# salesforce/ALPRO

Hardware: AMD Instinct MI355X
Metric: video-text pairs/sec (8f x 224^2, 40-tok) (higher is better)
Workload: dtype fp16

## Files before the change

alpro_amd/amp.py:

```python
import contextlib

import torch

from alpro_amd import config as rt


class LossScaler:

    def __init__(self, init_scale=2.0 ** 16, dynamic=True, growth=2.0, backoff=0.5, window=2000, min_scale=1.0, max_scale=2.0 ** 24, device=None):
        self.dynamic, self.growth, self.backoff, self.window = dynamic, growth, backoff, window
        self.min_scale, self.max_scale = min_scale, max_scale
        self._init = float(init_scale)
        self.state = None
        if device is not None:
            self.to(device)

    def to(self, device):
        if self.state is None or self.state.device != torch.device(device):
            prev = self.state.tolist() if self.state is not None else (getattr(self, "_pending", None) or [self._init, 0.0, 0.0, 0.0])
            self.state = torch.tensor(prev, dtype=torch.float32, device=device)
        return self

    @property
    def scale(self):
        return self.state[0:1]

    def loss_scale(self):
        return float(self.state[0].item())

    def state_dict(self):
        s = self.state.tolist() if self.state is not None else (getattr(self, "_pending", None) or [self._init, 0.0, 0.0, 0.0])
        return {"loss_scale": s[0], "unskipped": int(s[1]), "applied_steps": int(s[2]), "skipped_steps": int(s[3])}

    def load_state_dict(self, sd):
        vals = [float(sd["loss_scale"]), float(sd.get("unskipped", 0)), float(sd.get("applied_steps", 0)), float(sd.get("skipped_steps", 0))]
        if self.state is None:
            self._init = vals[0]
            self._pending = vals
        else:
            self.state.copy_(torch.tensor(vals, dtype=torch.float32))


_SCALERS = []


def needs_loss_scaling(dtype=None):
    return (dtype or rt.compute_dtype()) == torch.float16


def scaler_for(optimizer, create=True, **kw):
    inner = getattr(optimizer, "_opt", optimizer)
    sc = getattr(inner, "scaler", None)
    if sc is None and create:
        sc = LossScaler(**kw)
        inner.scaler = sc
        _SCALERS.append(sc)
        rt.set_armed_loss_scaler(sc)
    return sc


def initialize(models, optimizers=None, enabled=True, opt_level="O1", loss_scale="dynamic", **unused):
    if optimizers is not None and needs_loss_scaling():
        for opt in (optimizers if isinstance(optimizers, (list, tuple)) else [optimizers]):
            if loss_scale == "dynamic" or loss_scale is None:
                scaler_for(opt)
            else:
                scaler_for(opt, init_scale=float(loss_scale), dynamic=False)
    return models if optimizers is None else (models, optimizers)


def _grads_of(optimizer):
    from alpro_amd.optim import real_grad
    return [p.grad for g in optimizer.param_groups for p in g["params"] if real_grad(p) is not None]


def unscale_(optimizer, scaler):
    inner = getattr(optimizer, "_opt", optimizer)
    inv = torch.reciprocal(scaler.scale).reshape(())
    flat = getattr(inner, "flat", None)
    if flat is not None:
        if getattr(inner, "_inflight", None):
            inner._finish_exchange()
            inner._note_synced("sum")
        flat["g"].mul_(inv)
    else:
        grads = _grads_of(inner)
        if grads:
            torch._foreach_mul_(grads, inv)
    inner._grads_scaled = False


@contextlib.contextmanager
def scale_loss(loss, optimizers, delay_unscale=False, **unused):
    if not needs_loss_scaling():
        yield loss
        return
    opts = optimizers if isinstance(optimizers, (list, tuple)) else [optimizers]
    scaler = scaler_for(opts[0]).to(loss.device)
    for o in opts[1:]:
        getattr(o, "_opt", o).scaler = scaler
    for o in opts:
        getattr(o, "_opt", o)._grads_scaled = True
        if hasattr(getattr(o, "_opt", o), "_g_clean"):
            getattr(o, "_opt", o)._mark_dirty()
    with rt.loss_scaling(scaler):
        yield loss * scaler.scale.reshape(())
    if not delay_unscale:
        for o in opts:
            unscale_(o, scaler)
            _install_foreign_step_guard(getattr(o, "_opt", o), scaler)


def _install_foreign_step_guard(opt, scaler):
    if hasattr(opt, "flat") or getattr(opt, "_alpro_guarded", False):
        return
    real = opt.step

    def step(*a, **k):
        grads = _grads_of(opt)
        norms = torch._foreach_norm(grads) if grads else []
        finite = bool(torch.isfinite(torch.stack(norms)).all()) if norms else True
        st = scaler.state
        if not finite:
            st[0] = max(float(st[0]) * scaler.backoff, scaler.min_scale) if scaler.dynamic else st[0]
            st[1] = 0.0
            st[3] += 1.0
            return None
        out = real(*a, **k)
        st[2] += 1.0
        st[1] += 1.0
# ... 29 lines not shown
```

alpro_amd/config.py:

```python
import os

import torch

_DTYPES = {"bf16": torch.bfloat16, "bfloat16": torch.bfloat16, "f16": torch.float16, "fp16": torch.float16,
           "float16": torch.float16, "f32": torch.float32, "fp32": torch.float32, "float32": torch.float32}

_compute_dtype = _DTYPES[os.environ.get("ALPRO_COMPUTE_DTYPE", "bf16").lower()]


def compute_dtype():
    return _compute_dtype


def set_compute_dtype(dt):
    global _compute_dtype
    _compute_dtype = _DTYPES[dt.lower()] if isinstance(dt, str) else dt
    return _compute_dtype


class use_compute_dtype:

    def __init__(self, dt):
        self.dt = dt

# ... 71 lines not shown
_WGRAD_SIDE = {}


def _several_ranks():
    try:
        import torch.distributed as td
        return td.is_available() and td.is_initialized() and td.get_world_size() > 1
    except Exception:
        return False


def set_wgrad_stream(v):
    _wgrad_stream[0] = bool(v)


def wgrad_stream_enabled():
    return _wgrad_stream[0]


def wgrad_scope(enter):
    _wgrad_active[0] += 1 if enter else -1


def wgrad_side_stream(device):
    if not (_wgrad_stream[0] and _wgrad_active[0] > 0 and device.type == "cuda") or (_several_ranks() and os.environ.get("ALPRO_WGRAD_STREAM") != "force"):
        return None
    import torch
    cur = torch.cuda.current_stream(device)
    if any(s.cuda_stream == cur.cuda_stream for s in _TEXT_SIDE.values()):
        return None
    key = (device.index if device.index is not None else torch.cuda.current_device(), cur.cuda_stream)
    ent = _WGRAD_SIDE.get(key)
    if ent is None:
        ent = _WGRAD_SIDE[key] = [torch.cuda.Stream(device), False]
    ent[1] = True
    return ent[0]


def side_streams_of_current(device):
    if not (_wgrad_stream[0] and device.type == "cuda") or (_several_ranks() and os.environ.get("ALPRO_WGRAD_STREAM") != "force"):
        return []
    import torch
    key = (device.index if device.index is not None else torch.cuda.current_device(), torch.cuda.current_stream(device).cuda_stream)
    ent = _WGRAD_SIDE.get(key)
    if ent is None:
        ent = _WGRAD_SIDE[key] = [torch.cuda.Stream(device), False]
    return [ent[0].cuda_stream]


def join_wgrad():
    if not _WGRAD_SIDE:
        return
    import torch
    for (idx, handle), ent in _WGRAD_SIDE.items():
        if ent[1]:
            cur = torch.cuda.current_stream(idx)
            if cur.cuda_stream == handle:
                cur.wait_stream(ent[0])
                ent[1] = False


_text_stream = [os.environ.get("ALPRO_TEXT_STREAM", "1") != "0"]
_TEXT_SIDE = {}


def set_text_stream(v):
    _text_stream[0] = bool(v)


def text_stream_enabled():
    return _text_stream[0]


def text_side_stream(device):
    if not (_text_stream[0] and device.type == "cuda"):
        return None
    import torch
    key = (device.index if device.index is not None else torch.cuda.current_device(), torch.cuda.current_stream(device).cuda_stream)
    s = _TEXT_SIDE.get(key)
    if s is None:
        s = _TEXT_SIDE[key] = torch.cuda.Stream(device)
    return s


def is_text_side_stream(stream):
    return any(s.cuda_stream == stream.cuda_stream for s in _TEXT_SIDE.values())


def join_text_streams():
    if not _TEXT_SIDE:
        return
    import torch
    for (idx, handle), s in _TEXT_SIDE.items():
        cur = torch.cuda.current_stream(idx)
        if cur.cuda_stream == handle:
            cur.wait_stream(s)


_prompter_stream = [os.environ.get("ALPRO_PROMPTER_STREAM", "1") != "0"]
_PROMPTER_SIDE = {}


def set_prompter_stream(v):
    _prompter_stream[0] = bool(v)


def prompter_stream_enabled():
    return _prompter_stream[0]


def prompter_side_stream(device):
    if not (_prompter_stream[0] and device.type == "cuda") or (_several_ranks() and os.environ.get("ALPRO_PROMPTER_STREAM") != "force"):
        return None
    import torch
    key = (device.index if device.index is not None else torch.cuda.current_device(), torch.cuda.current_stream(device).cuda_stream)
    s = _PROMPTER_SIDE.get(key)
    if s is None:
        s = _PROMPTER_SIDE[key] = torch.cuda.Stream(device)
    return s


_defer_tadd = [os.environ.get("ALPRO_DEFER_TEMPORAL_ADD", "1") != "0"]


def defer_temporal_add():
    return _defer_tadd[0]


def set_defer_temporal_add(v):
    _defer_tadd[0] = bool(v)


def _recompute_from_env():
    v = os.environ.get("ALPRO_RECOMPUTE", "0").strip()
    if v not in ("0", "1"):
        raise ValueError("ALPRO_RECOMPUTE=%r: expected 0 (keep every ViT block activation, the default) or 1 (recompute them in backward)" % v)
    return v == "1"


_recompute = [_recompute_from_env()]


def recompute_blocks():
    return _recompute[0]


def set_recompute(flag):
    _recompute[0] = bool(flag)

# ... 113 lines not shown
```

alpro_amd/csrc/backward.hip:

```cpp
#include "common.hpp"
#include "row768.hpp"
#include <algorithm>

namespace alpro {
namespace {

template <typename Tin, typename Tout>
__device__ __forceinline__ void transpose_tile(float (&tile)[64][65], const Tin* __restrict__ in, int64_t ld_in, Tout* __restrict__ out,
                                               int64_t ld_out, int R, int C, int Rpad, float* __restrict__ colsum, int bx, int by) {
  const int r0 = by * 64, c0 = bx * 64;
  const int tx = threadIdx.x & 63, ty = threadIdx.x >> 6;
#pragma unroll 4
  for (int i = ty; i < 64; i += 4) {
    const int r = r0 + i, c = c0 + tx;
    tile[i][tx] = (r < R && c < C) ? to_f32(in[(int64_t)r * ld_in + c]) : 0.f;
  }
  __syncthreads();
  if (colsum && ty == 0 && c0 + tx < C) {
    float s = 0.f;
#pragma unroll 8
    for (int i = 0; i < 64; ++i) s += tile[i][tx];
    atomicAdd(colsum + c0 + tx, s);
  }
#pragma unroll 4
  for (int i = ty; i < 64; i += 4) {
    const int c = c0 + i, r = r0 + tx;
    if (c < C && r < Rpad) out[(int64_t)c * ld_out + r] = from_f32<Tout>(tile[tx][i]);
  }
}

template <typename Tin, typename Tout>
__global__ __launch_bounds__(256) void transpose_kernel(const Tin* __restrict__ in, int64_t ld_in, Tout* __restrict__ out, int64_t ld_out,
                                                        int R, int C, int Rpad, float* __restrict__ colsum) {
  __shared__ float tile[64][65];
  transpose_tile<Tin, Tout>(tile, in, ld_in, out, ld_out, R, C, Rpad, colsum, blockIdx.x, blockIdx.y);
}

template <typename Tout>
__global__ __launch_bounds__(256) void transpose_batch_kernel(const alpro_transpose_job_t* __restrict__ jobs, int njobs) {
  __shared__ float tile[64][65];
  int lo = 0, hi = njobs - 1;
  while (lo < hi) {
    const int mid = (lo + hi + 1) >> 1;
    if (jobs[mid].tile0 <= (int)blockIdx.x) lo = mid;
    else hi = mid - 1;
  }
  const alpro_transpose_job_t jb = jobs[lo];
  const int t = blockIdx.x - jb.tile0, tcx = (jb.C + 63) / 64;
  transpose_tile<float, Tout>(tile, jb.in, jb.ld_in, (Tout*)jb.out, jb.ld_out, jb.R, jb.C, jb.Rpad, nullptr, t % tcx, t / tcx);
}

constexpr int LN_PART_BYTES = 3 * LN_D * (int)sizeof(float);

struct EmitArgs {
// ... 4 lines not shown
  float drop_p;
  uint32_t drop_seed;
  float* colsum_pre;
  int extra_cls;
};

template <typename T, bool CP = true>
__device__ __forceinline__ void emit_row(const EmitArgs& e, int64_t r, int lane, float (&v)[12], float (&cp)[12]) {
  T* out = (T*)e.out;
  if (e.mode == ALPRO_EMIT_ROWS) {
    if (e.drop_seed) {
      const uint32_t th = drop_thresh24(e.drop_p);
      const float ks = 1.0f / (1.0f - e.drop_p);
#pragma unroll
      for (int i = 0; i < 12; ++i) v[i] = row_drop_keep(e.drop_seed, r, lane, i, th) ? v[i] * ks : 0.f;
    }
    ln_store_scaled<T>(out + r * LN_D, lane, v, e.scale ? e.scale[r / e.group] : 1.0f);
    return;
  }
  const int Tn = e.p0, N = e.p1;
  const int64_t S = 1 + (int64_t)N * Tn;
  const int64_t b = r / S, k = r - b * S;
  if (e.mode == ALPRO_EMIT_FRAME) {
    if (k == 0) {
      const float inv = 1.0f / (float)Tn;
      for (int t = 0; t < Tn; ++t) ln_store_scaled<T>(out + ((b * Tn + t) * (N + 1)) * LN_D, lane, v, (e.scale ? e.scale[b * Tn + t] : 1.0f) * inv);
    } else {
      const int64_t n = (k - 1) / Tn;
      const int t = (int)((k - 1) - n * Tn);
      ln_store_scaled<T>(out + ((b * Tn + t) * (N + 1) + 1 + n) * LN_D, lane, v, e.scale ? e.scale[b * Tn + t] : 1.0f);
    }
  } else {
    if (k == 0) return;
    const int64_t o = r - b - 1;
    if constexpr (CP) {
#pragma unroll
      for (int i = 0; i < 12; ++i) cp[i] += v[i];
    }
    ln_store_scaled<T>(out + o * LN_D, lane, v, e.scale ? e.scale[o / e.group] : 1.0f);
  }
}

#define ALPRO_LN_DATA 0
#include "layernorm_bwd_kernel.hpp"
#undef ALPRO_LN_DATA
#define ALPRO_LN_DATA 1
#include "layernorm_bwd_kernel.hpp"
#undef ALPRO_LN_DATA

__global__ __launch_bounds__(1024) void colsum_reduce_kernel(const float* __restrict__ part, int nparts, int nslots, float* __restrict__ d0,
                                                             float* __restrict__ d1, float* __restrict__ d2) {
  __shared__ float4 red[128][8];
  __shared__ float4 red2[8][8];
  const int k = blockIdx.y, c4 = threadIdx.x & 7, sl = threadIdx.x >> 3;
  float* dst = k == 0 ? d0 : (k == 1 ? d1 : d2);
  if (!dst) return;
  const int col = blockIdx.x * 32 + c4 * 4;
  float4 s = make_float4(0.f, 0.f, 0.f, 0.f);
#pragma unroll 4
  for (int p = sl; p < nparts; p += 128) {
    const float4 v = *(const float4*)(part + ((int64_t)p * nslots + k) * LN_D + col);
    s.x += v.x; s.y += v.y; s.z += v.z; s.w += v.w;
  }
  red[sl][c4] = s;
  __syncthreads();
  if (sl < 8) {
    float4 t = red[sl * 16][c4];
#pragma unroll
    for (int i = 1; i < 16; ++i) { const float4 v = red[sl * 16 + i][c4]; t.x += v.x; t.y += v.y; t.z += v.z; t.w += v.w; }
    red2[sl][c4] = t;
  }
  __syncthreads();
  if (sl == 0) {
    float4 t = red2[0][c4];
#pragma unroll
    for (int i = 1; i < 8; ++i) { const float4 v = red2[i][c4]; t.x += v.x; t.y += v.y; t.z += v.z; t.w += v.w; }
    float4* o = (float4*)(dst + col);
    const float4 c = *o;
    *o = make_float4(c.x + t.x, c.y + t.y, c.z + t.z, c.w + t.w);
  }
}

__global__ __launch_bounds__(192) void cls_rows_reduce_kernel(const float* __restrict__ cls_ws, float* __restrict__ dx, int64_t ld_dx, int T, int N) {
  const int b = blockIdx.x, c = threadIdx.x * 4;
  float4 s = make_float4(0.f, 0.f, 0.f, 0.f);
  for (int t = 0; t < T; ++t) {
    const float4 v = *(const float4*)(cls_ws + ((int64_t)b * T + t) * LN_D + c);
    s.x += v.x; s.y += v.y; s.z += v.z; s.w += v.w;
  }
  float4* o = (float4*)(dx + (int64_t)b * (1 + (int64_t)N * T) * ld_dx + c);
  const float4 cur = *o;
  *o = make_float4(cur.x + s.x, cur.y + s.y, cur.z + s.z, cur.w + s.w);
}

template <typename TE, int MODE>
__global__ __launch_bounds__(256) void vit_final_pool_bwd_kernel(const float* __restrict__ dout, const float* __restrict__ x, const float* __restrict__ gamma,
                                                                 float eps, float* __restrict__ dx, float* __restrict__ dgamma, float* __restrict__ dbeta,
                                                                 int64_t rows, int Tn, int N, const EmitArgs em, float* __restrict__ part) {
  __shared__ float red[2][4][LN_D];
  const int lane = threadIdx.x & 63, w = threadIdx.x >> 6;
  const int64_t nwaves = (int64_t)gridDim.x * 4;
  const int64_t S = 1 + (int64_t)N * Tn;
  float g[12], ag[12], ab[12], cp[12];
  ln_load(gamma, lane, g);
#pragma unroll
  for (int i = 0; i < 12; ++i) ag[i] = ab[i] = cp[i] = 0.f;
  for (int64_t r = (int64_t)blockIdx.x * 4 + w; r < rows; r += nwaves) {
    const int64_t b = r / S, k = r - b * S;
    const int64_t n = k ? (k - 1) / Tn : 0;
    const int t = k ? (int)((k - 1) - n * Tn) : 0;
    int64_t src;
    float sc = 1.0f;
    if constexpr (MODE == ALPRO_POOL_TEMPORAL) {
      src = b * (N + 1) + (k ? 1 + n : 0);
      if (k) sc = 1.0f / (float)Tn;
    } else if constexpr (MODE == ALPRO_POOL_SPATIAL) {
      src = b * (Tn + 1) + (k ? 1 + t : 0);
      if (k) sc = 1.0f / (float)N;
    } else {
      src = (b * Tn + t) * (N + 1) + (k ? 1 + n : 0);
    }
    float xv[12], d[12];
    ln_load_nt(x + r * LN_D, lane, xv);
    ln_load(dout + src * LN_D, lane, d);
    if (MODE == ALPRO_POOL_NONE && k == 0) {
      for (int f = 1; f < Tn; ++f) {
        float d2[12];
        ln_load(dout + (src + (int64_t)f * (N + 1)) * LN_D, lane, d2);
#pragma unroll
        for (int i = 0; i < 12; ++i) d[i] += d2[i];
      }
    }
    float mean, rstd;
// ... 345 lines not shown
  ALPRO_DISPATCH_DTYPE(out_dtype, T, hipLaunchKernelGGL(transpose_batch_kernel<T>, dim3((unsigned)total_tiles), dim3(256), 0, (hipStream_t)stream, jobs, njobs));
  return check_launch("alpro_transpose_batch");
}

extern "C" int alpro_layernorm_bwd_emit(const void* dy, int dy_dtype, int64_t ld_dy, const float* dy2, const float* x, int64_t ldx,
                                        const float* gamma, float eps, float* dx, int64_t ld_dx, int accumulate, float* dgamma, float* dbeta,
                                        int rows, int D, int map_mode, int map_p0, int map_p1, float drop_p, uint32_t drop_seed, void* emit_out,
                                        int emit_dtype, int emit_mode, int emit_p0, int emit_p1, const float* emit_scale, int emit_scale_group, float emit_drop_p,
                                        uint32_t emit_drop_seed, float* emit_colsum_pre, int emit_extra_cls, void* workspace, size_t workspace_bytes,
                                        void* stream) {
  ALPRO_CHECK(dy && x && gamma && dx && rows > 0, "alpro_layernorm_bwd: bad args");
  ALPRO_CHECK((dgamma != nullptr) == (dbeta != nullptr), "alpro_layernorm_bwd: dgamma and dbeta must both be given or both be NULL (got %s only); "
              "pass a throw-away buffer for the one that is not wanted", dgamma ? "dgamma" : "dbeta");
  const bool data_only = dgamma == nullptr;
  ALPRO_CHECK(!data_only || !emit_colsum_pre, "alpro_layernorm_bwd_emit: colsum_pre needs the column-sum form of the kernel -- pass a throw-away dgamma / dbeta pair with it");
  ALPRO_CHECK(!workspace || (((uintptr_t)workspace % 16) == 0 && workspace_bytes >= LN_PART_BYTES), "alpro_layernorm_bwd: the workspace must be 16-byte aligned and hold at least one workgroup's sums (%d bytes)", LN_PART_BYTES);
  ALPRO_CHECK(D == LN_D, "alpro_layernorm_bwd: D=%d unsupported", D);
  ALPRO_CHECK(map_mode >= 0 && map_mode <= ALPRO_MAP_FRAME_TOKENS, "alpro_layernorm_bwd: bad map_mode %d", map_mode);
  ALPRO_CHECK(map_mode != ALPRO_MAP_FRAME_TOKENS || accumulate, "alpro_layernorm_bwd: the FRAME_TOKENS scatter needs accumulate=1 (CLS rows are shared)");
  ALPRO_CHECK(emit_mode >= ALPRO_EMIT_NONE && emit_mode <= ALPRO_EMIT_SKIP_CLS, "alpro_layernorm_bwd_emit: bad emit_mode %d", emit_mode);
  ALPRO_CHECK(emit_mode == ALPRO_EMIT_NONE || emit_out, "alpro_layernorm_bwd_emit: an emit mode needs the output rows");
  ALPRO_CHECK(emit_mode == ALPRO_EMIT_NONE || ld_dx == LN_D, "alpro_layernorm_bwd_emit: the emit needs a dense gradient stream (ld_dx == 768)");
  ALPRO_CHECK(emit_mode == ALPRO_EMIT_NONE || emit_mode == ALPRO_EMIT_ROWS || (emit_p0 > 0 && emit_p1 > 0), "alpro_layernorm_bwd_emit: FRAME / SKIP_CLS emits need p0 = T, p1 = N");
  ALPRO_CHECK(!emit_scale || emit_scale_group > 0, "alpro_layernorm_bwd_emit: emit_scale_group must be > 0");
  ALPRO_CHECK(!emit_drop_seed || (emit_mode == ALPRO_EMIT_ROWS && emit_drop_p > 0.f && emit_drop_p < 1.f), "alpro_layernorm_bwd_emit: dropout only in ROWS mode, 0 < p < 1");
  ALPRO_CHECK(!emit_colsum_pre || emit_mode == ALPRO_EMIT_SKIP_CLS, "alpro_layernorm_bwd_emit: colsum_pre belongs to the SKIP_CLS emit");
  ALPRO_CHECK(emit_extra_cls == 0 || (emit_mode == ALPRO_EMIT_ROWS && map_mode == ALPRO_MAP_SKIP_CLS && emit_p0 > 0 && emit_p1 > 0),
              "alpro_layernorm_bwd_emit: extra CLS rows go with ROWS emit after a SKIP_CLS-mapped LayerNorm (p0 = T, p1 = N)");
  EmitArgs em;
  em.out = emit_out; em.mode = emit_mode; em.p0 = emit_p0; em.p1 = emit_p1; em.scale = emit_scale; em.group = emit_scale_group;
  em.drop_p = emit_drop_p; em.drop_seed = emit_drop_seed; em.colsum_pre = emit_colsum_pre; em.extra_cls = emit_extra_cls;
  ALPRO_CHECK(emit_mode == ALPRO_EMIT_NONE || emit_dtype == dy_dtype || dy_dtype == ALPRO_F32, "alpro_layernorm_bwd_emit: emit_dtype must be dy's dtype, or any dtype when dy is the fp32 stream");
  const bool frame = map_mode == ALPRO_MAP_FRAME_TOKENS;
  const size_t cls_bytes = frame ? (size_t)(rows / (map_p1 + 1)) * LN_D * sizeof(float) : 0;
  ALPRO_CHECK(!workspace || workspace_bytes >= cls_bytes + LN_PART_BYTES, "alpro_layernorm_bwd: the workspace must hold the CLS frame terms (%zu bytes) and at least one workgroup's sums", cls_bytes);
  const int cap = get_option(OPT_LN_GRID);
  int nblk = grid_for(rows, 4 * 8, cap > 0 ? cap : 256 * 8);
  if (workspace && !data_only) nblk = (int)std::min<size_t>((size_t)nblk, (workspace_bytes - cls_bytes) / LN_PART_BYTES);
  const dim3 grid(nblk), blk(256);
  float* part = data_only ? nullptr : (float*)workspace;
  float* cls_ws = (workspace && frame) ? (float*)workspace + (data_only ? 0 : (size_t)nblk * 3 * LN_D) : nullptr;
  hipStream_t st = (hipStream_t)stream;
#define ALPRO_LNB(T, TE) \
  do { if (data_only) ALPRO_LNB_K(layernorm_bwd_data_kernel, T, TE); else ALPRO_LNB_K(layernorm_bwd_kernel, T, TE); } while (0)
#define ALPRO_LNB_K(KERNEL, T, TE) hipLaunchKernelGGL((KERNEL<T, TE>), grid, blk, 0, st, (const T*)dy, ld_dy, dy2, x, ldx, gamma, eps, dx, ld_dx, accumulate, dgamma, dbeta, (int64_t)rows, map_mode, map_p0, map_p1, drop_p, drop_seed, em, part, cls_ws)
  if (dy_dtype == ALPRO_F32 && emit_mode != ALPRO_EMIT_NONE && emit_dtype == ALPRO_BF16) ALPRO_LNB(float, bf16_t);
  else if (dy_dtype == ALPRO_F32 && emit_mode != ALPRO_EMIT_NONE && emit_dtype == ALPRO_F16) ALPRO_LNB(float, f16_t);
  else if (dy_dtype == ALPRO_F32) ALPRO_LNB(float, float);
  else if (dy_dtype == ALPRO_BF16) ALPRO_LNB(bf16_t, bf16_t);
  else if (dy_dtype == ALPRO_F16) ALPRO_LNB(f16_t, f16_t);
  else { set_error("alpro_layernorm_bwd: bad dtype %d", dy_dtype); return ALPRO_ERR_INVALID; }
#undef ALPRO_LNB
#undef ALPRO_LNB_K
  if (part) hipLaunchKernelGGL(colsum_reduce_kernel, dim3(LN_D / 32, emit_colsum_pre ? 3 : 2), dim3(1024), 0, st, part, nblk, 3, dgamma, dbeta, emit_colsum_pre);
  if (cls_ws) hipLaunchKernelGGL(cls_rows_reduce_kernel, dim3(rows / (map_p1 + 1) / map_p0), dim3(192), 0, st, cls_ws, dx, ld_dx, map_p0, map_p1);
  return check_launch("alpro_layernorm_bwd");
}

extern "C" int alpro_layernorm_bwd(const void* dy, int dy_dtype, int64_t ld_dy, const float* dy2, const float* x, int64_t ldx,
                                   const float* gamma, float eps, float* dx, int64_t ld_dx, int accumulate, float* dgamma, float* dbeta,
                                   int rows, int D, int map_mode, int map_p0, int map_p1, float drop_p, uint32_t drop_seed, void* workspace,
                                   size_t workspace_bytes, void* stream) {
  return alpro_layernorm_bwd_emit(dy, dy_dtype, ld_dy, dy2, x, ldx, gamma, eps, dx, ld_dx, accumulate, dgamma, dbeta, rows, D, map_mode, map_p0, map_p1,
                                  drop_p, drop_seed, nullptr, dy_dtype, ALPRO_EMIT_NONE, 0, 0, nullptr, 1, 0.f, 0u, nullptr, 0, workspace, workspace_bytes, stream);
}

extern "C" int alpro_vit_final_pool_mode_bwd(const float* dout, const float* x, const float* gamma, float eps, float* dx, float* dgamma, float* dbeta,
                                             int mode, int64_t rows, int B, int T, int N, int D, void* emit_out, int emit_dtype, const float* emit_scale,
                                             int emit_scale_group, void* workspace, size_t workspace_bytes, void* stream) {
  constexpr size_t part_bytes = 2 * LN_D * sizeof(float);
  ALPRO_CHECK(dout && x && gamma && dx && dgamma && dbeta && B > 0 && T > 0 && N > 0, "alpro_vit_final_pool_mode_bwd: bad args");
  ALPRO_CHECK(mode >= ALPRO_POOL_TEMPORAL && mode <= ALPRO_POOL_NONE, "alpro_vit_final_pool_mode_bwd: bad mode %d (ALPRO_POOL_TEMPORAL / _SPATIAL / _NONE)", mode);
  ALPRO_CHECK(D == LN_D, "alpro_vit_final_pool_mode_bwd: D=%d unsupported (hidden size is 768 on this path)", D);
  ALPRO_CHECK(rows == (int64_t)B * (1 + (int64_t)N * T), "alpro_vit_final_pool_mode_bwd: rows=%lld is not B * (1 + N * T) = %d * (1 + %d * %d)", (long long)rows, B, N, T);
  ALPRO_CHECK(!workspace || (((uintptr_t)workspace % 16) == 0 && workspace_bytes >= part_bytes), "alpro_vit_final_pool_mode_bwd: the workspace must be 16-byte aligned and hold at least one workgroup's sums (%zu bytes)", part_bytes);
  ALPRO_CHECK(!emit_out || emit_dtype == ALPRO_F32 || emit_dtype == ALPRO_BF16 || emit_dtype == ALPRO_F16, "alpro_vit_final_pool_mode_bwd: bad emit_dtype %d", emit_dtype);
  ALPRO_CHECK(!emit_scale || emit_scale_group > 0, "alpro_vit_final_pool_mode_bwd: emit_scale_group must be > 0");
  EmitArgs em;
  em.out = emit_out; em.mode = emit_out ? ALPRO_EMIT_ROWS : ALPRO_EMIT_NONE; em.p0 = T; em.p1 = N; em.scale = emit_scale; em.group = emit_scale_group;
  em.drop_p = 0.f; em.drop_seed = 0u; em.colsum_pre = nullptr; em.extra_cls = 0;
  const int cap = get_option(OPT_LN_GRID);
  int nblk = grid_for(rows, 4 * 8, cap > 0 ? cap : 256 * 8);
  if (workspace) nblk = (int)std::min<size_t>((size_t)nblk, workspace_bytes / part_bytes);
  const dim3 grid(nblk), blk(256);
  float* part = (float*)workspace;
  hipStream_t st = (hipStream_t)stream;
#define ALPRO_FPB(TE, M) hipLaunchKernelGGL((vit_final_pool_bwd_kernel<TE, M>), grid, blk, 0, st, dout, x, gamma, eps, dx, dgamma, dbeta, rows, T, N, em, part)
#define ALPRO_FPB_MODES(TE) \
  do { if (mode == ALPRO_POOL_TEMPORAL) ALPRO_FPB(TE, ALPRO_POOL_TEMPORAL); else if (mode == ALPRO_POOL_SPATIAL) ALPRO_FPB(TE, ALPRO_POOL_SPATIAL); else ALPRO_FPB(TE, ALPRO_POOL_NONE); } while (0)
  if (emit_out && emit_dtype == ALPRO_BF16) ALPRO_FPB_MODES(bf16_t);
  else if (emit_out && emit_dtype == ALPRO_F16) ALPRO_FPB_MODES(f16_t);
  else ALPRO_FPB_MODES(float);
#undef ALPRO_FPB_MODES
#undef ALPRO_FPB
  if (part) hipLaunchKernelGGL(colsum_reduce_kernel, dim3(LN_D / 32, 2), dim3(1024), 0, st, part, nblk, 2, dgamma, dbeta, (float*)nullptr);
  return check_launch("alpro_vit_final_pool_mode_bwd");
}

extern "C" int alpro_gather_cast(const float* src, int64_t ld, void* out, int dtype, int rows, int D, int map_mode, int map_p0, int map_p1,
                                 const float* row_scale, int row_scale_group, float cls_scale, float drop_p, uint32_t drop_seed, float* colsum,
                                 float* colsum_pre, void* workspace, size_t workspace_bytes, void* stream) {
  ALPRO_CHECK(src && out && rows > 0, "alpro_gather_cast: bad args");
  ALPRO_CHECK(!workspace || (((uintptr_t)workspace % 16) == 0 && workspace_bytes >= 2 * LN_D * sizeof(float)), "alpro_gather_cast: the workspace must be 16-byte aligned and hold at least one workgroup's sums");
  ALPRO_CHECK(D == LN_D, "alpro_gather_cast: D=%d unsupported", D);
  ALPRO_CHECK(map_mode >= 0 && map_mode <= ALPRO_MAP_PATCH_EMBED, "alpro_gather_cast: bad map_mode %d", map_mode);
  ALPRO_CHECK(!row_scale || row_scale_group > 0, "alpro_gather_cast: row_scale_group must be > 0");
  if (colsum || colsum_pre) {
    float* part = (float*)workspace;
    int nblk = grid_for(rows, 32, 512);
    if (part) nblk = (int)std::min<size_t>((size_t)nblk, workspace_bytes / (2 * LN_D * sizeof(float)));
    ALPRO_DISPATCH_DTYPE(dtype, T, hipLaunchKernelGGL((gather_cast_kernel<T, 16>), dim3(nblk), dim3(1024), 0, (hipStream_t)stream, src, ld, (T*)out, (int64_t)rows, map_mode, map_p0, map_p1, row_scale, row_scale_group, cls_scale, drop_p, drop_seed, colsum, colsum_pre, part));
    if (part) hipLaunchKernelGGL(colsum_reduce_kernel, dim3(LN_D / 32, 2), dim3(1024), 0, (hipStream_t)stream, part, nblk, 2, colsum, colsum_pre, (float*)nullptr);
  } else {
    ALPRO_DISPATCH_DTYPE(dtype, T, hipLaunchKernelGGL((gather_cast_kernel<T, 4>), dim3(grid_for(rows, 8, 256 * 32)), dim3(256), 0, (hipStream_t)stream, src, ld, (T*)out, (int64_t)rows, map_mode, map_p0, map_p1, row_scale, row_scale_group, cls_scale, drop_p, drop_seed, colsum, colsum_pre, (float*)nullptr));
  }
  return check_launch("alpro_gather_cast");
}

extern "C" int alpro_colsum_tn(const void* A, int64_t lda, int dtype, int M, int N, int K, float* colsum, void* workspace, size_t workspace_bytes,
                               void* stream) {
  ALPRO_CHECK(A && colsum && M > 0 && N > 0 && K > 0, "alpro_colsum_tn: bad args");
  ALPRO_CHECK(dtype == ALPRO_BF16 || dtype == ALPRO_F16, "alpro_colsum_tn: 16-bit rows only (it restates the 16-bit weight-gradient GEMM's bias gradient)");
  ALPRO_CHECK(lda >= N, "alpro_colsum_tn: lda must cover N");
  const int ranges = alpro_gemm_tn_ranges(M, N, K, cu_budget((hipStream_t)stream));
  const int total_steps = (M + 31) / 32, per = (total_steps + ranges - 1) / ranges, tk_cnt = (K + 255) / 256;
  const int sets = ranges * tk_cnt, npad = (N + 31) / 32 * 32;
  ALPRO_CHECK(workspace && ((uintptr_t)workspace % 16) == 0 && workspace_bytes >= (size_t)sets * npad * sizeof(float),
              "alpro_colsum_tn: the workspace must be 16-byte aligned and hold %d partial sets of %d floats (%zu bytes)", sets, npad, (size_t)sets * npad * sizeof(float));
  float* part = (float*)workspace;
  const dim3 grid((npad / 32 + 3) / 4, sets);
  hipStream_t st = (hipStream_t)stream;
  if (dtype == ALPRO_BF16) hipLaunchKernelGGL(colsum_tn_kernel<bf16_t>, grid, dim3(256), 0, st, (const bf16_t*)A, lda, M, N, per, tk_cnt, total_steps, part, npad);
  else hipLaunchKernelGGL(colsum_tn_kernel<f16_t>, grid, dim3(256), 0, st, (const f16_t*)A, lda, M, N, per, tk_cnt, total_steps, part, npad);
  hipLaunchKernelGGL(colsum_tn_reduce_kernel, dim3((N + 255) / 256), dim3(256), 0, st, part, sets, npad, colsum, N);
  return check_launch("alpro_colsum_tn");
}

extern "C" int alpro_tproj_small(const alpro_tproj_job_t* jobs_device, int njobs, int D, int mode, void* stream) {
  ALPRO_CHECK(jobs_device && njobs > 0 && (mode == 0 || mode == 1), "alpro_tproj_small: bad args");
  ALPRO_CHECK(D == LN_D, "alpro_tproj_small: D=%d unsupported", D);
  if (mode == 0) hipLaunchKernelGGL(tproj_small_kernel<0>, dim3(D / 4, njobs), dim3(256), 0, (hipStream_t)stream, jobs_device, D);
  else hipLaunchKernelGGL(tproj_small_kernel<1>, dim3(D / 64, njobs), dim3(256), 0, (hipStream_t)stream, jobs_device, D);
  return check_launch("alpro_tproj_small");
}

extern "C" int alpro_gelu_bwd(const void* dh, const void* u, void* du, int dtype, int64_t n, void* stream) {
  ALPRO_CHECK(dh && u && du && n > 0, "alpro_gelu_bwd: bad args");
  ALPRO_CHECK(n % 8 == 0, "alpro_gelu_bwd: n must be a multiple of 8");
  ALPRO_DISPATCH_DTYPE(dtype, T, hipLaunchKernelGGL(gelu_bwd_kernel<T>, dim3(grid_for(n / Chunk<T>::N, 256, 256 * 16)), dim3(256), 0, (hipStream_t)stream, (const T*)dh, (const T*)u, (T*)du, n));
  return check_launch("alpro_gelu_bwd");
}

extern "C" int alpro_cls_mean_bwd(const float* dx_out, int64_t ld_batch, float* dside, int B, int T, int D, void* stream) {
  ALPRO_CHECK(dx_out && dside && B > 0 && T > 0 && D > 0, "alpro_cls_mean_bwd: bad args");
  hipLaunchKernelGGL(cls_mean_bwd_kernel, dim3(B), dim3(256), 0, (hipStream_t)stream, dx_out, ld_batch, dside, B, T, D);
  return check_launch("alpro_cls_mean_bwd");
}

extern "C" int alpro_scatter_add_rows_ordered(const float* src, const int64_t* idx, float* dst, int rows, int D, int64_t dst_rows, int64_t skip_idx, uint32_t* keys_ws,
                                              void* stream) {
  ALPRO_CHECK(src && idx && dst && keys_ws && rows > 0, "alpro_scatter_add_rows_ordered: bad args");
  ALPRO_CHECK(D == LN_D, "alpro_scatter_add_rows_ordered: D=%d unsupported", D);
  ALPRO_CHECK(rows <= SCATTER_SORT_MAX && dst_rows > 0 && dst_rows < (1 << 19), "alpro_scatter_add_rows_ordered: at most %d source rows and fewer than 2^19 table rows (got %d, %lld)",
              SCATTER_SORT_MAX, rows, (long long)dst_rows);
  hipLaunchKernelGGL(scatter_sort_keys_kernel, dim3(1), dim3(1024), 0, (hipStream_t)stream, idx, rows, dst_rows, keys_ws);
// ... 15 lines not shown
```

alpro_amd/csrc/gemm_tn.hip:

```cpp
#include "common.hpp"

namespace alpro {
namespace {

constexpr int TM = 32;
constexpr int NSTAGE = 4;
constexpr int TW = 256;
constexpr int ROW_BYTES = TW * 2;
constexpr int IMG_BYTES = TM * ROW_BYTES;
constexpr int NT3 = 512;

__device__ u32x4 g_zero_page[4];

typedef short s16x4 __attribute__((ext_vector_type(4)));

__device__ __forceinline__ u32x2 tr4(const char* img, int m0, int colblk16, int lane) {
  const int p = lane & 15;
  const int row = m0 + (p >> 2);
  const int chunk = (colblk16 << 1) | ((p >> 1) & 1);
  const char* a = img + row * ROW_BYTES + ((chunk ^ ((row & 3) << 2)) << 4) + ((p & 1) << 3);
  const s16x4 r = __builtin_amdgcn_ds_read_tr16_b64_v4i16((__attribute__((address_space(3))) s16x4*)a);
  return __builtin_bit_cast(u32x2, r);
}
__device__ __forceinline__ u32x4 frag8(const char* img, int ks, int col0, int lane) {
  const int g = lane >> 5;
  const int blk = (col0 >> 4) + ((lane >> 4) & 1);
  const u32x2 a = tr4(img, ks * 16 + 4 * g, blk, lane);
  const u32x2 b = tr4(img, ks * 16 + 8 + 4 * g, blk, lane);
  const uint32_t ax = a.x, ay = a.y, bx = b.x, by = b.y;
  return mk4(ax, ay, bx, by);
}

template <typename T, int PP = 0>
__global__ __launch_bounds__(NT3, 1) void gemm_tn_kernel(const T* __restrict__ A, int64_t lda, const T* __restrict__ B, int64_t ldb,
                                                         float* __restrict__ C, int64_t ldc, int M, int N, int K, int per,
                                                         int tiles, int units, int tn_cnt, float* __restrict__ colsum, float* __restrict__ part,
                                                         float* __restrict__ part_cs, int ablate ) {
  extern __shared__ __attribute__((aligned(16))) char smem[];
  const int tid = threadIdx.x, lane = tid & 63, wave = __builtin_amdgcn_readfirstlane(tid >> 6);
  const int wr = wave >> 2, wc = wave & 3;
  const int upx = (units + 7) >> 3;
  const int unit = (blockIdx.x & 7) * upx + (blockIdx.x >> 3);
  if (unit >= units) return;
  const int range = unit / tiles, tile = unit - range * tiles;
  const int total_steps = (M + TM - 1) / TM;
  const int s0 = range * per, s1 = min(s0 + per, total_steps);
  const int n0 = (tile % tn_cnt) * TW, k0 = (tile / tn_cnt) * TW;
  if (s0 >= s1) return;

  const char* zero = (const char*)g_zero_page;
  const int rows_end = min(s1 * TM, M);
  const char* curA[2];
  const char* curB[2];
  int mrow[2];
  int64_t strA[2], strB[2];
#pragma unroll
  for (int i = 0; i < 2; ++i) {
    const int row = (wave + 8 * i) * 2 + (lane >> 5);
    const int col = ((lane & 31) ^ ((row & 3) << 2)) * 8;
    const int64_t m = (int64_t)s0 * TM + row;
// ... 131 lines not shown
        copy(2 * (1 - ks) + 1, buf);
        advance(1 - ks);
        asm volatile("s_waitcnt vmcnt(6)" ::: "memory");
        pbar();
        __builtin_amdgcn_s_setprio(1);
#pragma unroll
        for (int i = 0; i < 4; ++i)
#pragma unroll
          for (int jj = 0; jj < 2; ++jj) mma_chunk<T>(acc[i][jj], fa[i], fb[jj]);
        __builtin_amdgcn_s_setprio(0);
        if (cs_now) add_cols(fa);
        pbar();
      }
    }
    if (wr == 0) pbar();
  }
  if (do_cs) {
    const float t = cs + __shfl_xor(cs, 32, 64);
    const int n = n0 + wr * 128 + wc * 32 + (lane & 31);
    if (lane < 32 && part_cs) part_cs[((int64_t)range * tk_cnt + tk) * (tn_cnt * TW) + n] = t;
    else if (lane < 32 && n < N) unsafeAtomicAdd(colsum + n, t);
  }
  asm volatile("s_waitcnt vmcnt(0)" ::: "memory");
  if (part) {
    float* dst = part + (int64_t)unit * (TW * TW) + wave * 8192 + lane * 4;
#pragma unroll
    for (int i = 0; i < 4; ++i)
#pragma unroll
      for (int j = 0; j < 2; ++j)
#pragma unroll
        for (int q = 0; q < 4; ++q) {
          f32x4 v = {acc[i][j][4 * q], acc[i][j][4 * q + 1], acc[i][j][4 * q + 2], acc[i][j][4 * q + 3]};
          __builtin_nontemporal_store(v, (f32x4*)(dst + ((i * 2 + j) * 4 + q) * 256));
        }
    return;
  }
#pragma unroll
  for (int j = 0; j < 2; ++j) {
    const int k = k0 + wc * 64 + j * 32 + (lane & 31);
    if (k < K) {
#pragma unroll
      for (int i = 0; i < 4; ++i)
#pragma unroll
        for (int r = 0; r < 16; ++r) {
          const int n = n0 + wr * 128 + i * 32 + acc_row(r, lane);
          if (n < N) unsafeAtomicAdd(C + (int64_t)n * ldc + k, acc[i][j][r]);
        }
    }
  }
}

__global__ __launch_bounds__(256) void tn_reduce_kernel(const float* __restrict__ part, const float* __restrict__ part_cs, float* __restrict__ C,
                                                        int64_t ldc, float* __restrict__ colsum, int N, int K, int tiles, int ranges, int tn_cnt) {
  const int tile_blocks = part ? tiles * 64 : 0;
  if ((int)blockIdx.x >= tile_blocks) {
    __shared__ float red[8][32];
    const int c = threadIdx.x & 31, p = threadIdx.x >> 5;
    const int n = (blockIdx.x - tile_blocks) * 32 + c;
    const int sets = ranges * (tiles / tn_cnt);
    float t = 0.f;
    for (int r = p; r < sets; r += 8) t += part_cs[(int64_t)r * (tn_cnt * TW) + n];
    red[p][c] = t;
    __syncthreads();
    if (p == 0 && n < N) colsum[n] += ((red[0][c] + red[1][c]) + (red[2][c] + red[3][c])) + ((red[4][c] + red[5][c]) + (red[6][c] + red[7][c]));
    return;
  }
  const int tile = blockIdx.x >> 6, f = ((blockIdx.x & 63) << 8) + threadIdx.x;
  const int lane = f & 63, q = (f >> 6) & 3, j = (f >> 8) & 1, i = (f >> 9) & 3, wave = f >> 11;
  const int n = (tile % tn_cnt) * TW + (wave >> 2) * 128 + i * 32 + 8 * q + 4 * (lane >> 5);
  const int k = (tile / tn_cnt) * TW + (wave & 3) * 64 + j * 32 + (lane & 31);
  const float* src = part + (int64_t)tile * (TW * TW) + f * 4;
  const int64_t stride = (int64_t)tiles * (TW * TW);
  f32x4 t = {0.f, 0.f, 0.f, 0.f};
  int r = 0;
  for (; r + 4 <= ranges; r += 4) {
    const f32x4 a = __builtin_nontemporal_load((const f32x4*)(src + (r + 0) * stride)), b = __builtin_nontemporal_load((const f32x4*)(src + (r + 1) * stride));
    const f32x4 c = __builtin_nontemporal_load((const f32x4*)(src + (r + 2) * stride)), d = __builtin_nontemporal_load((const f32x4*)(src + (r + 3) * stride));
    t = (((t + a) + b) + c) + d;
  }
  for (; r < ranges; ++r) t = t + __builtin_nontemporal_load((const f32x4*)(src + r * stride));
  if (k < K) {
#pragma unroll
    for (int c = 0; c < 4; ++c)
      if (n + c < N) C[(int64_t)(n + c) * ldc + k] += t[c];
  }
}

template <typename T>
__global__ __launch_bounds__(256) void colsum_kernel(const T* __restrict__ A, int64_t lda, float* __restrict__ out, int M, int N) {
  constexpr int E = Chunk<T>::N;
  __shared__ float red[4][64 * E];
  const int lane = threadIdx.x & 63, w = threadIdx.x >> 6;
  const int c = blockIdx.x * 64 + lane;
  const bool cv = c * E < N;
  const int m0 = blockIdx.y * 256, m1 = min(m0 + 256, M);
  float s[E];
#pragma unroll
  for (int e = 0; e < E; ++e) s[e] = 0.f;
  if (cv) {
    const T* base = A + c * E;
    int m = m0 + w;
    for (; m + 28 < m1; m += 32) {
      u32x4 v[8];
#pragma unroll
      for (int u = 0; u < 8; ++u) v[u] = *(const u32x4*)(base + (int64_t)(m + 4 * u) * lda);
#pragma unroll
      for (int u = 0; u < 8; ++u) {
        float f[E];
        unpack_chunk<T>(v[u], f);
#pragma unroll
        for (int e = 0; e < E; ++e) s[e] += f[e];
      }
    }
    for (; m < m1; m += 4) {
      float f[E];
      unpack_chunk<T>(*(const u32x4*)(base + (int64_t)m * lda), f);
#pragma unroll
      for (int e = 0; e < E; ++e) s[e] += f[e];
    }
  }
#pragma unroll
  for (int e = 0; e < E; ++e) red[w][lane * E + e] = s[e];
  __syncthreads();
  for (int i = threadIdx.x; i < 64 * E; i += 256) {
    const int col = blockIdx.x * 64 * E + i;
    if (col < N) unsafeAtomicAdd(out + col, red[0][i] + red[1][i] + red[2][i] + red[3][i]);
  }
}

}
}

using namespace alpro;

namespace {
struct TnPlan {
  int tn, tiles, total_steps, ranges, per, units;
  size_t part_floats, cs_floats;
// ... 25 lines not shown
  return p;
}
}

extern "C" size_t alpro_gemm_tn_workspace_bytes(int M, int N, int K) {
  if (M <= 0 || N <= 0 || K <= 0) return 0;
  struct Memo { int M, N, K, forced; size_t bytes; };
  static Memo memo[64];
  static int n_memo = 0, lock = 0;
  const int forced = get_option(OPT_TN_SPLITS);
  while (__atomic_exchange_n(&lock, 1, __ATOMIC_ACQUIRE)) {}
  for (int i = 0; i < n_memo; ++i)
    if (memo[i].M == M && memo[i].N == N && memo[i].K == K && memo[i].forced == forced) {
      const size_t b = memo[i].bytes;
      __atomic_store_n(&lock, 0, __ATOMIC_RELEASE);
      return b;
    }
  __atomic_store_n(&lock, 0, __ATOMIC_RELEASE);
  size_t best = 0;
  for (int cus = 64; cus <= 256; cus += 8) {
    const TnPlan p = tn_plan(M, N, K, true, cus);
    const size_t b = (p.part_floats + p.cs_floats) * sizeof(float);
    best = b > best ? b : best;
  }
  while (__atomic_exchange_n(&lock, 1, __ATOMIC_ACQUIRE)) {}
  if (n_memo < 64) memo[n_memo++] = Memo{M, N, K, forced, best};
  __atomic_store_n(&lock, 0, __ATOMIC_RELEASE);
  return best;
}

extern "C" int alpro_gemm_tn_ranges(int M, int N, int K, int compute_units) {
  if (M <= 0 || N <= 0 || K <= 0) return 0;
  const int cus = (compute_units >= 64 && compute_units < 256) ? compute_units / 8 * 8 : 256;
  return tn_plan(M, N, K, true, cus).ranges;
}

extern "C" int alpro_gemm_tn_acc_ws(const void* A, int64_t lda, const void* B, int64_t ldb, float* C, int64_t ldc, int dtype, int M, int N,
                                    int K, float* colsum, void* workspace, size_t workspace_bytes, void* stream) {
  ALPRO_CHECK(A && B && C && M > 0 && N > 0 && K > 0, "alpro_gemm_tn_acc: bad args");
  ALPRO_CHECK(dtype == ALPRO_BF16 || dtype == ALPRO_F16, "alpro_gemm_tn_acc: 16-bit operands only (fp32 mode uses alpro_transpose + alpro_gemm)");
  ALPRO_CHECK(lda % 8 == 0 && ldb % 8 == 0 && lda >= (N + 7) / 8 * 8 && ldb >= (K + 7) / 8 * 8,
              "alpro_gemm_tn_acc: lda/ldb must be multiples of 8 covering N/K rounded up to 8 (16-byte chunks are read whole)");
  ALPRO_CHECK(((uintptr_t)A % 16) == 0 && ((uintptr_t)B % 16) == 0, "alpro_gemm_tn_acc: operands must be 16-byte aligned");
  const bool ws = workspace != nullptr;
  const TnPlan p = tn_plan(M, N, K, ws, cu_budget((hipStream_t)stream));
  float* part = nullptr;
  float* part_cs = nullptr;
  if (ws) {
    ALPRO_CHECK(((uintptr_t)workspace % 16) == 0 && workspace_bytes >= (p.part_floats + p.cs_floats) * sizeof(float),
                "alpro_gemm_tn_acc_ws: workspace must be 16-byte aligned and hold alpro_gemm_tn_workspace_bytes(M, N, K) bytes");
    part = p.ranges > 1 ? (float*)workspace : nullptr;
    part_cs = colsum ? (float*)workspace + p.part_floats : nullptr;
  }
  const bool pp = get_option(OPT_TN_KIND) == 2;
  const unsigned grid = (unsigned)((p.units + 7) / 8 * 8);
  const size_t lds = (size_t)NSTAGE * 2 * IMG_BYTES;
  hipStream_t st = (hipStream_t)stream;
  if (dtype == ALPRO_BF16) {
    static DeviceOnce once;
    once.run([&] {
      (void)hipFuncSetAttribute((const void*)gemm_tn_kernel<bf16_t, 0>, hipFuncAttributeMaxDynamicSharedMemorySize, (int)lds);
      (void)hipFuncSetAttribute((const void*)gemm_tn_kernel<bf16_t, 1>, hipFuncAttributeMaxDynamicSharedMemorySize, (int)lds);
    });
    if (pp) hipLaunchKernelGGL((gemm_tn_kernel<bf16_t, 1>), dim3(grid), dim3(NT3), lds, st, (const bf16_t*)A, lda, (const bf16_t*)B, ldb, C, ldc, M, N, K, p.per, p.tiles, p.units, p.tn, colsum, part, part_cs, 0);
    else hipLaunchKernelGGL((gemm_tn_kernel<bf16_t, 0>), dim3(grid), dim3(NT3), lds, st, (const bf16_t*)A, lda, (const bf16_t*)B, ldb, C, ldc, M, N, K, p.per, p.tiles, p.units, p.tn, colsum, part, part_cs, 0);
  } else {
    static DeviceOnce once;
    once.run([&] {
      (void)hipFuncSetAttribute((const void*)gemm_tn_kernel<f16_t, 0>, hipFuncAttributeMaxDynamicSharedMemorySize, (int)lds);
      (void)hipFuncSetAttribute((const void*)gemm_tn_kernel<f16_t, 1>, hipFuncAttributeMaxDynamicSharedMemorySize, (int)lds);
    });
    if (pp) hipLaunchKernelGGL((gemm_tn_kernel<f16_t, 1>), dim3(grid), dim3(NT3), lds, st, (const f16_t*)A, lda, (const f16_t*)B, ldb, C, ldc, M, N, K, p.per, p.tiles, p.units, p.tn, colsum, part, part_cs, 0);
    else hipLaunchKernelGGL((gemm_tn_kernel<f16_t, 0>), dim3(grid), dim3(NT3), lds, st, (const f16_t*)A, lda, (const f16_t*)B, ldb, C, ldc, M, N, K, p.per, p.tiles, p.units, p.tn, colsum, part, part_cs, 0);
  }
  if (part || part_cs)
    hipLaunchKernelGGL(tn_reduce_kernel, dim3((part ? p.tiles * 64 : 0) + (part_cs ? p.tn * (TW / 32) : 0)), dim3(256), 0, st, part, part_cs, C, ldc, colsum, N, K, p.tiles, p.ranges, p.tn);
  return check_launch("alpro_gemm_tn_acc");
}

extern "C" int alpro_gemm_tn_acc(const void* A, int64_t lda, const void* B, int64_t ldb, float* C, int64_t ldc, int dtype, int M, int N,
                                 int K, float* colsum, void* stream) {
  return alpro_gemm_tn_acc_ws(A, lda, B, ldb, C, ldc, dtype, M, N, K, colsum, nullptr, 0, stream);
}

extern "C" int alpro_colsum_acc(const void* A, int64_t lda, float* out, int dtype, int M, int N, void* stream) {
  ALPRO_CHECK(A && out && M > 0 && N > 0, "alpro_colsum_acc: bad args");
  const int esz = dtype == ALPRO_F32 ? 4 : 2;
  ALPRO_CHECK((N * esz) % 16 == 0 && (lda * esz) % 16 == 0, "alpro_colsum_acc: rows must be 16-byte multiples");
  ALPRO_DISPATCH_DTYPE(dtype, T, hipLaunchKernelGGL(colsum_kernel<T>, dim3((N + 64 * Chunk<T>::N - 1) / (64 * Chunk<T>::N), (M + 255) / 256), dim3(256), 0, (hipStream_t)stream, (const T*)A, lda, out, M, N));
  return check_launch("alpro_colsum_acc");
}
```

alpro_amd/dist.py:

```python
import os
import sys

import torch
import torch.distributed as td


def is_initialized():
    return td.is_available() and td.is_initialized()


_FORCE = [os.environ.get("ALPRO_FORCE_COLLECTIVES", "0") == "1"]


def collectives_active():
    return is_initialized() and (td.get_world_size() > 1 or _FORCE[0])


def rccl_cu_reserve():
    return max(0, min(64, int(os.environ.get("ALPRO_RCCL_CU_RESERVE", "16"))))


def _single_node():
    world = int(os.environ.get("WORLD_SIZE", "1"))
    for var in ("LOCAL_WORLD_SIZE", "OMPI_COMM_WORLD_LOCAL_SIZE", "MV2_COMM_WORLD_LOCAL_SIZE"):
# ... 44 lines not shown

def set_allgather_grad_mode(mode):
    assert mode in ("average", "sum"), mode
    _GATHER_GRAD[0] = mode


def allgather_grad_mode():
    return _GATHER_GRAD[0]


class _AllGather(torch.autograd.Function):

    @staticmethod
    def forward(ctx, x):
        ctx.n = x.shape[0]
        out = torch.empty((size() * x.shape[0],) + tuple(x.shape[1:]), dtype=x.dtype, device=x.device)
        td.all_gather_into_tensor(out, x.contiguous())
        return out

    @staticmethod
    def backward(ctx, g):
        g = g.contiguous()
        out = torch.empty((ctx.n,) + tuple(g.shape[1:]), dtype=g.dtype, device=g.device)
        if td.get_backend() == "gloo":
            g = g.clone()
            td.all_reduce(g)
            out.copy_(g[rank() * ctx.n:(rank() + 1) * ctx.n])
        else:
            td.reduce_scatter_tensor(out, g)
        if _GATHER_GRAD[0] == "average":
            out.div_(size())
        return out


def allgather(x, name=None):
    if not collectives_active():
        return x
    return _AllGather.apply(x)


_GRAD_FINAL_HOOKS = []


def register_grads_final_hook(fn):
    import weakref
    ref = weakref.WeakMethod(fn) if hasattr(fn, "__self__") else (lambda f=fn: f)
    _GRAD_FINAL_HOOKS.append(ref)


def grads_final(params=None, all_but=None):
    if not collectives_active() or not _GRAD_FINAL_HOOKS:
        return
    from alpro_amd import config as rt
    rt.join_wgrad()
    rt.join_text_streams()
    live = []
    for ref in _GRAD_FINAL_HOOKS:
        fn = ref()
        if fn is not None:
            fn(params=params, all_but=all_but)
            live.append(ref)
    _GRAD_FINAL_HOOKS[:] = live


def allreduce_grads_(params, bucket_bytes=64 << 20, average=True):
    if not collectives_active():
        return 0
    params = list(params)
    real = lambda p: p.grad is not None and (p.grad.dim() == 0 or p.grad.numel() <= 1 or any(p.grad.stride()))
    if params:
        has = torch.tensor([1 if real(p) else 0 for p in params], dtype=torch.int32, device=params[0].device)
        td.all_reduce(has, op=td.ReduceOp.MAX)
        for p, h in zip(params, has.tolist()):
            if h and not real(p):
                p.grad = torch.zeros_like(p)
    grads = [p.grad for p in params if real(p)]
    sent = 0
    bucket, nbytes = [], 0

    def flush():
        nonlocal bucket, nbytes, sent
        if not bucket:
            return
        flat = torch.cat([g.reshape(-1) for g in bucket])
        td.all_reduce(flat)
        if average:
            flat.div_(size())
        off = 0
        for g in bucket:
            g.copy_(flat[off:off + g.numel()].view_as(g))
            off += g.numel()
        sent += flat.numel() * flat.element_size()
        bucket, nbytes = [], 0

    for g in grads:
        bucket.append(g)
        nbytes += g.numel() * g.element_size()
        if nbytes >= bucket_bytes:
            flush()
    flush()
    return sent


def broadcast_parameters(module_or_state, root_rank=0):
    if not collectives_active():
        return
# ... 10 lines not shown
```

alpro_amd/hip.py:

```python
import ctypes
import os

import torch

_HERE = os.path.dirname(os.path.abspath(__file__))
LIB_PATH = os.environ.get("ALPRO_HIP_LIB") or os.path.join(_HERE, "lib", "libalpro_hip.so")

F32, BF16, F16 = 0, 1, 2
ACT_NONE, ACT_GELU, ACT_RELU, ACT_GELU_BWD, ACT_GELU_SAVE_GRAD, ACT_MUL_SAVED, ACT_RELU_MASK = 0, 1, 2, 3, 4, 5, 6
POOL_MODES = {"mean": 0, "max": 1, "lse": 2}
MAP_IDENTITY, MAP_SKIP_CLS, MAP_FRAME_TOKENS, MAP_PATCH_EMBED = 0, 1, 2, 3
ADD_IDENTITY, ADD_PRE_SPATIAL, ADD_PRE_MLP, ADD_PRE_TEMPORAL = 0, 1, 2, 3
EMIT_NONE, EMIT_ROWS, EMIT_FRAME, EMIT_SKIP_CLS = 0, 1, 2, 3
AUG_OPS = {"Identity": 0, "HorizontalFlip": 1, "Brightness": 2, "Contrast": 3, "Sharpness": 4, "Color": 5, "Solarize": 6, "Posterize": 7,
           "TranslateX": 8, "TranslateY": 9, "ShearX": 10, "ShearY": 11, "Rotate": 12}
POOL_TEMPORAL, POOL_SPATIAL, POOL_NONE = 0, 1, 2

_TORCH_DTYPE = {F32: torch.float32, BF16: torch.bfloat16, F16: torch.float16}
_CODE = {v: k for k, v in _TORCH_DTYPE.items()}

EXPORTS = ["alpro_hip_last_error", "alpro_hip_abi_version", "alpro_hip_set_option", "alpro_hip_set_stream_option", "alpro_gemm", "alpro_gemm_c2_tiled_rows", "alpro_layernorm_fwd",
           "alpro_attn_temporal_fwd", "alpro_attn_fwd", "alpro_patchify", "alpro_cls_mean_residual",
           "alpro_vit_final_pool", "alpro_bert_embed_fwd", "alpro_cast_from_f32", "alpro_attn_bwd", "alpro_attn_temporal_bwd",
           "alpro_layernorm_bwd", "alpro_transpose", "alpro_transpose_batch", "alpro_gelu_bwd", "alpro_cls_mean_bwd", "alpro_scatter_add_rows", "alpro_gather_cast", "alpro_sumsq", "alpro_adamw_step", "alpro_gemm_tn_acc", "alpro_gemm_tn_acc_ws", "alpro_gemm_tn_workspace_bytes", "alpro_gemm_tn_ranges", "alpro_colsum_acc", "alpro_colsum_tn", "alpro_softmax_xent", "alpro_vtc_loss_fwd", "alpro_vtc_loss_bwd", "alpro_prepare_clips", "alpro_loss_scale_update", "alpro_add_layernorm_fwd", "alpro_layernorm_bwd_emit", "alpro_gemm_batch", "alpro_tproj_small", "alpro_attn_cls_fwd", "alpro_gemm_rows_f32", "alpro_gather_seq_fwd", "alpro_gather_seq_bwd", "alpro_scatter_add_rows_ordered",
           "alpro_hip_sched_workspace_bytes", "alpro_hip_set_sched_workspace", "alpro_hip_release_stream", "alpro_gemm_qkv_tattn", "alpro_add_layernorm_pre_mlp2", "alpro_adamw_step_lp",
           "alpro_gemm_rows_f32_relu_mask", "alpro_clip_pool", "alpro_adamw_step_groups", "alpro_attn_temporal_fwd_drop", "alpro_attn_temporal_bwd_drop",
           "alpro_vit_final_pool_mode", "alpro_vit_final_pool_mode_bwd", "alpro_augment_stage", "alpro_augment_stats", "alpro_resized_crop",
           "alpro_sim_topk", "alpro_sim_topk_workspace_bytes", "alpro_attn_probs", "alpro_attn_temporal_probs", "alpro_attn_probs_grad", "alpro_unpatchify"]


class GemmDesc(ctypes.Structure):
    _fields_ = [("A", ctypes.c_void_p), ("W", ctypes.c_void_p), ("C", ctypes.c_void_p),
                ("lda", ctypes.c_int64), ("ldw", ctypes.c_int64), ("ldc", ctypes.c_int64),
                ("M", ctypes.c_int), ("N", ctypes.c_int), ("K", ctypes.c_int),
                ("dtype", ctypes.c_int), ("c_dtype", ctypes.c_int), ("alpha", ctypes.c_float),
                ("bias", ctypes.c_void_p), ("act", ctypes.c_int),
                ("row_scale", ctypes.c_void_p), ("row_scale_group", ctypes.c_int),
                ("residual", ctypes.c_void_p), ("ldr", ctypes.c_int64),
                ("map_mode", ctypes.c_int), ("map_p0", ctypes.c_int), ("map_p1", ctypes.c_int),
                ("side", ctypes.c_void_p), ("ld_side", ctypes.c_int64),
                ("C2", ctypes.c_void_p), ("ldc2", ctypes.c_int64),
                ("drop_p", ctypes.c_float), ("drop_seed", ctypes.c_uint32), ("bias2", ctypes.c_void_p), ("m_off", ctypes.c_int64),
                ("c2_tiled", ctypes.c_int32), ("reserved0", ctypes.c_int32)]


class TprojJob(ctypes.Structure):
    _fields_ = [("wfc", ctypes.c_void_p), ("bp", ctypes.c_void_p), ("b1", ctypes.c_void_p), ("db1", ctypes.c_void_p), ("g_fc", ctypes.c_void_p),
                ("g_bp", ctypes.c_void_p)]


class TransposeJob(ctypes.Structure):
    _fields_ = [("in_", ctypes.c_void_p), ("out", ctypes.c_void_p), ("ld_in", ctypes.c_int64), ("ld_out", ctypes.c_int64),
                ("R", ctypes.c_int32), ("C", ctypes.c_int32), ("Rpad", ctypes.c_int32), ("tile0", ctypes.c_int32)]


ADAMW_MAX_SEGMENTS = 32
RESAMPLE_MAX_TAPS = 257


class AdamWSegment(ctypes.Structure):
    _fields_ = [("end", ctypes.c_int64), ("lr", ctypes.c_float), ("beta1", ctypes.c_float), ("beta2", ctypes.c_float), ("eps", ctypes.c_float),
                ("weight_decay", ctypes.c_float), ("step_size", ctypes.c_float), ("correct_bias", ctypes.c_int32), ("reserved0", ctypes.c_int32)]


class AdamWSegments(ctypes.Structure):
    _fields_ = [("count", ctypes.c_int32), ("reserved0", ctypes.c_int32), ("seg", AdamWSegment * ADAMW_MAX_SEGMENTS)]


ABI_VERSION = 22
_lib = None


def load():
    global _lib
    if _lib is not None:
        return _lib
    hq = os.environ.get("GPU_MAX_HW_QUEUES")
    if hq and hq.isdigit() and int(hq) > 4 and any(os.environ.get(k, "1") != "0" for k in ("ALPRO_WGRAD_STREAM", "ALPRO_TEXT_STREAM", "ALPRO_PROMPTER_STREAM")):
        import warnings
        warnings.warn("alpro_amd: GPU_MAX_HW_QUEUES=%s -- with more than 4 hardware queues the training step's side streams (ALPRO_WGRAD_STREAM / "
                      "ALPRO_TEXT_STREAM / ALPRO_PROMPTER_STREAM) measured 11 %% SLOWER than with the runtime's default of 4 (profiles/r6_hw_queues.txt): "
                      "a fifth queue shares a dispatch pipe with the launch stream's" % hq)
    if not os.path.exists(LIB_PATH):
        raise RuntimeError("libalpro_hip.so not found at %s -- run `python -m alpro_amd.build` "
                           "(there is no CPU fallback for the ALPRO hot path)" % LIB_PATH)
    lib = ctypes.CDLL(LIB_PATH)
    lib.alpro_hip_last_error.restype = ctypes.c_char_p
    for name in EXPORTS:
        getattr(lib, name)
    vp, i32, i64, f32 = ctypes.c_void_p, ctypes.c_int, ctypes.c_int64, ctypes.c_float
    lib.alpro_gemm.argtypes = [ctypes.POINTER(GemmDesc), vp]
    lib.alpro_gemm_batch.argtypes = [ctypes.POINTER(GemmDesc), vp, ctypes.c_int, vp]
    lib.alpro_tproj_small.argtypes = [vp, ctypes.c_int, ctypes.c_int, ctypes.c_int, vp]
    lib.alpro_layernorm_fwd.argtypes = [vp, i64, vp, vp, f32, vp, i32, i64, vp, vp, vp, i32, i32, i32, i32, i32, vp]
    lib.alpro_add_layernorm_fwd.argtypes = [vp, vp, i32, vp, i32, vp, vp, vp, f32, vp, vp, i64, i32, i32, i32, vp]
    lib.alpro_attn_temporal_fwd.argtypes = [vp, vp, i32, i64, i32, i32, f32, vp, vp]
    u32 = ctypes.c_uint32
    lib.alpro_attn_bwd.argtypes = [vp, vp, vp, vp, vp, i32, i32, i32, i32, f32, vp, f32, u32, vp]
    lib.alpro_attn_temporal_bwd.argtypes = [vp, vp, vp, vp, vp, i32, i64, i32, i32, f32, vp]
    lib.alpro_attn_temporal_fwd_drop.argtypes = [vp, vp, i32, i64, i32, i32, f32, vp, f32, u32, vp]
    lib.alpro_attn_temporal_bwd_drop.argtypes = [vp, vp, vp, vp, vp, i32, i64, i32, i32, f32, f32, u32, vp]
    lib.alpro_layernorm_bwd.argtypes = [vp, i32, i64, vp, vp, i64, vp, f32, vp, i64, i32, vp, vp, i32, i32, i32, i32, i32, f32, u32, vp, ctypes.c_size_t, vp]
    lib.alpro_layernorm_bwd_emit.argtypes = [vp, i32, i64, vp, vp, i64, vp, f32, vp, i64, i32, vp, vp, i32, i32, i32, i32, i32, f32, u32,
                                             vp, i32, i32, i32, i32, vp, i32, f32, u32, vp, i32, vp, ctypes.c_size_t, vp]
    lib.alpro_transpose.argtypes = [vp, i32, i64, vp, i32, i64, i32, i32, i32, vp, vp]
    lib.alpro_gelu_bwd.argtypes = [vp, vp, vp, i32, i64, vp]
    lib.alpro_sumsq.argtypes = [vp, i64, vp, vp, ctypes.c_size_t, vp]
    lib.alpro_softmax_xent.argtypes = [vp, i64, vp, i32, vp, vp, i32, i64, vp, i32, i32, i32, vp]
    lib.alpro_gemm_tn_acc.argtypes = [vp, i64, vp, i64, vp, i64, i32, i32, i32, i32, vp, vp]
    lib.alpro_gemm_tn_acc_ws.argtypes = [vp, i64, vp, i64, vp, i64, i32, i32, i32, i32, vp, vp, ctypes.c_size_t, vp]
    lib.alpro_gemm_tn_workspace_bytes.argtypes = [i32, i32, i32]
    lib.alpro_gemm_tn_workspace_bytes.restype = ctypes.c_size_t
    lib.alpro_gemm_tn_ranges.argtypes = [i32, i32, i32, i32]
    lib.alpro_colsum_acc.argtypes = [vp, i64, vp, i32, i32, i32, vp]
    lib.alpro_colsum_tn.argtypes = [vp, i64, i32, i32, i32, i32, vp, vp, ctypes.c_size_t, vp]
    lib.alpro_transpose_batch.argtypes = [vp, i32, i32, i32, vp]
    lib.alpro_adamw_step.argtypes = [vp, vp, vp, vp, i64, f32, f32, f32, f32, f32, f32, vp, f32, f32, vp, i32, i32, i32, vp]
    lib.alpro_adamw_step_lp.argtypes = [vp, vp, vp, vp, i64, f32, f32, f32, f32, f32, f32, vp, f32, f32, vp, i32, i32, i32, vp, i32, vp]
    lib.alpro_adamw_step_groups.argtypes = [vp, vp, vp, vp, i64, ctypes.POINTER(AdamWSegments), vp, f32, f32, vp, i32, i32, vp, i32, vp]
    lib.alpro_loss_scale_update.argtypes = [vp, vp, f32, f32, i32, f32, f32, vp]
    lib.alpro_gather_cast.argtypes = [vp, i64, vp, i32, i32, i32, i32, i32, i32, vp, i32, f32, f32, u32, vp, vp, vp, ctypes.c_size_t, vp]
    lib.alpro_cls_mean_bwd.argtypes = [vp, i64, vp, i32, i32, i32, vp]
    lib.alpro_scatter_add_rows.argtypes = [vp, vp, vp, i32, i32, i32, i64, vp]
    lib.alpro_attn_fwd.argtypes = [vp, vp, i32, i32, i32, i32, f32, vp, vp, f32, u32, vp, i32, vp, vp]
    lib.alpro_attn_cls_fwd.argtypes = [vp, i32, vp, vp, vp, i32, i32, i32, i32, f32, f32, u32, vp]
    lib.alpro_gemm_rows_f32.argtypes = [vp, i64, vp, i64, vp, i64, i32, i32, i32, vp, i32, vp, vp, i64, vp, vp, f32, vp]
    lib.alpro_gemm_rows_f32_relu_mask.argtypes = [vp, i64, vp, i64, vp, i64, i32, i32, i32, vp, i64, vp]
    lib.alpro_clip_pool.argtypes = [vp, i64, vp, i64, vp, i32, i32, i32, i32, vp]
    lib.alpro_gemm_c2_tiled_rows.argtypes = [i64, i64, i64, i32]
    lib.alpro_gemm_c2_tiled_rows.restype = i64
    lib.alpro_patchify.argtypes = [vp, vp, i32, i32, i32, i32, i32, vp]
    lib.alpro_cls_mean_residual.argtypes = [vp, i64, vp, vp, i64, i32, i32, i32, vp]
    lib.alpro_vit_final_pool.argtypes = [vp, vp, vp, f32, vp, vp, i32, i32, i32, i32, i32, vp]
    lib.alpro_vit_final_pool_mode.argtypes = [vp, vp, vp, f32, vp, vp, i32, i32, i64, i32, i32, i32, i32, vp]
    lib.alpro_vit_final_pool_mode_bwd.argtypes = [vp, vp, vp, f32, vp, vp, vp, i32, i64, i32, i32, i32, i32, vp, i32, vp, i32, vp, ctypes.c_size_t, vp]
    lib.alpro_add_layernorm_pre_mlp2.argtypes = [vp, vp, vp, vp, i32, vp, vp, vp, f32, vp, i64, i32, i32, i32, vp]
    lib.alpro_bert_embed_fwd.argtypes = [vp, vp, vp, vp, vp, vp, f32, vp, vp, i32, vp, vp, i32, i32, i32, f32, u32, vp]
    lib.alpro_cast_from_f32.argtypes = [vp, vp, i32, i64, vp]
    lib.alpro_hip_set_option.argtypes = [ctypes.c_char_p, i32]
    lib.alpro_hip_set_stream_option.argtypes = [vp, ctypes.c_char_p, i32]
    lib.alpro_hip_sched_workspace_bytes.restype = ctypes.c_size_t
    lib.alpro_hip_set_sched_workspace.argtypes = [vp, vp, ctypes.c_size_t]
    lib.alpro_hip_release_stream.argtypes = [vp]
    lib.alpro_gemm_qkv_tattn.argtypes = [vp, i64, vp, i64, vp, vp, i64, i32, i32, i32, i32, i32, f32, vp, i64, vp, vp]
    lib.alpro_scatter_add_rows_ordered.argtypes = [vp, vp, vp, i32, i32, i64, i64, vp, vp]
    lib.alpro_gather_seq_fwd.argtypes = [vp, vp, vp, vp, vp, vp, i32, i32, i32, i32, i32, vp]
    lib.alpro_gather_seq_bwd.argtypes = [vp, vp, i32, vp, vp, vp, vp, i32, i32, i32, i32, i32, i32, vp]
    lib.alpro_prepare_clips.argtypes = [vp, i32, vp, f32, ctypes.POINTER(f32), ctypes.POINTER(f32), vp, vp, vp, i32, i32, i32, i32, vp]
    lib.alpro_augment_stage.argtypes = [vp, vp, vp, vp, vp, vp, i32, i32, i32, i32, i32, i32, vp]
    lib.alpro_augment_stats.argtypes = [vp, vp, vp, vp, vp, vp, i32, i32, i32, i32, i32, i32, vp]
    lib.alpro_resized_crop.argtypes = [vp, i64, vp, vp, vp, vp, i32, i32, i32, i32, vp]
    lib.alpro_vtc_loss_fwd.argtypes = [vp, vp, vp, vp, vp, i32, i32, i32, i32, vp, vp, vp, vp, vp]
    lib.alpro_vtc_loss_bwd.argtypes = [vp, vp, vp, vp, vp, i32, i32, i32, i32, vp, vp, vp, vp, vp, vp, vp, vp, vp, vp, vp, vp]
    lib.alpro_sim_topk_workspace_bytes.argtypes = [i32, i32, i32, i32]
    lib.alpro_sim_topk_workspace_bytes.restype = ctypes.c_size_t
    lib.alpro_sim_topk.argtypes = [vp, i32, vp, i32, i32, i32, f32, i32, vp, vp, vp, ctypes.c_size_t, vp]
    lib.alpro_attn_probs.argtypes = [vp, vp, vp, vp, i32, i32, i32, i32, f32, i32, i32, i32, i32, vp]
    lib.alpro_attn_temporal_probs.argtypes = [vp, vp, vp, i32, i64, i32, i32, f32, vp]
    lib.alpro_attn_probs_grad.argtypes = [vp, vp, vp, vp, vp, vp, i32, i32, i32, i32, f32, f32, i32, i32, i32, i32, vp]
    lib.alpro_unpatchify.argtypes = [vp, i32, vp, i32, i32, i32, i32, vp]
    if lib.alpro_hip_abi_version() != ABI_VERSION:
        raise RuntimeError("libalpro_hip.so ABI version mismatch")
    _lib = lib
# ... 258 lines not shown
    else:
        _check(lib.alpro_attn_temporal_fwd_drop(_ptr(qkv), _ptr(out), _CODE[qkv.dtype], rows, T, H, scale, _ptr(lse), drop_p, drop_seed, _stream()),
               "alpro_attn_temporal_fwd_drop")
    return (out, lse) if want_lse else out


def attn_temporal_bwd(qkv, out, dout, lse, T, H, scale, drop_p=0.0, drop_seed=0):
    lib = load()
    _dev(qkv); _dev(out, qkv.dtype); _dev(dout, qkv.dtype); _dev(lse, torch.float32)
    dqkv = torch.empty_like(qkv)
    if drop_p == 0.0 and drop_seed == 0:
        _check(lib.alpro_attn_temporal_bwd(_ptr(qkv), _ptr(out), _ptr(dout), _ptr(lse), _ptr(dqkv), _CODE[qkv.dtype], qkv.shape[0], T, H, scale,
                                           _stream()), "alpro_attn_temporal_bwd")
    else:
        _check(lib.alpro_attn_temporal_bwd_drop(_ptr(qkv), _ptr(out), _ptr(dout), _ptr(lse), _ptr(dqkv), _CODE[qkv.dtype], qkv.shape[0], T, H, scale,
                                                drop_p, drop_seed, _stream()), "alpro_attn_temporal_bwd_drop")
    return dqkv


def attn_bwd(qkv, out, dout, lse, batch, L, H, scale, key_bias=None, drop_p=0.0, drop_seed=0):
    lib = load()
    _dev(qkv); _dev(out, qkv.dtype); _dev(dout, qkv.dtype); _dev(lse, torch.float32)
    dqkv = torch.empty_like(qkv)
    kb = _dev(key_bias, torch.float32) if key_bias is not None else None
    _check(lib.alpro_attn_bwd(_ptr(qkv), _ptr(out), _ptr(dout), _ptr(lse), _ptr(dqkv), _CODE[qkv.dtype], batch, L, H, scale, _ptr(kb), drop_p, drop_seed, _stream()),
           "alpro_attn_bwd")
    return dqkv


_LN_THROWAWAY = {}


def ln_throwaway_pair(device):
    t = _LN_THROWAWAY.get(str(device))
    if t is None:
        t = _LN_THROWAWAY[str(device)] = torch.zeros((2, 768), dtype=torch.float32, device=device)
    return t[0], t[1]


def layernorm_bwd(dy, x, gamma, eps, dx, dgamma=None, dbeta=None, rows=None, dy2=None, accumulate=True, map_mode=MAP_IDENTITY, map_p0=0, map_p1=0,
                  drop_p=0.0, drop_seed=0, emit=None):
    lib = load()
    _dev(dy); _dev(x, torch.float32); _dev(dx, torch.float32)
    if (dgamma is None) != (dbeta is None) or (dgamma is None and emit is not None and emit.get("colsum_pre") is not None):
        tg, tb = ln_throwaway_pair(dy.device)
        dgamma, dbeta = (tg if dgamma is None else dgamma), (tb if dbeta is None else dbeta)
    if dgamma is not None:
        _dev(dgamma, torch.float32); _dev(dbeta, torch.float32)
    D = x.shape[-1]
    rows = rows if rows is not None else dy.numel() // D
    common = (_ptr(dy), _CODE[dy.dtype], D, _ptr(_dev(dy2, torch.float32)) if dy2 is not None else None, _ptr(x), D,
              _ptr(_dev(gamma, torch.float32)), eps, _ptr(dx), D, 1 if accumulate else 0, _ptr(dgamma), _ptr(dbeta), rows, D,
              map_mode, map_p0, map_p1, drop_p, drop_seed)
    ws, wsb = _reduce_ws(dy.device)
    if emit is None:
        _check(lib.alpro_layernorm_bwd(*common, ws, wsb, _stream()), "alpro_layernorm_bwd")
        return dx
    out = torch.empty((emit["rows"], D), dtype=emit.get("dtype", dy.dtype), device=dy.device)
    sc, cp = emit.get("scale"), emit.get("colsum_pre")
    _check(lib.alpro_layernorm_bwd_emit(*common, _ptr(out), _CODE[out.dtype], emit["mode"], emit.get("T", 0), emit.get("N", 0),
                                        _ptr(_dev(sc, torch.float32)) if sc is not None else None, emit.get("group", 1), emit.get("drop_p", 0.0),
                                        emit.get("drop_seed", 0), _ptr(_dev(cp, torch.float32)) if cp is not None else None, emit.get("extra_cls", 0),
                                        ws, wsb, _stream()), "alpro_layernorm_bwd_emit")
    return dx, out


def transpose(x, out_dtype=None, pad_to=64, colsum=None):
    lib = load()
    _dev(x)
    R, C = x.shape
    out_dtype = out_dtype or x.dtype
    Rpad = (R + pad_to - 1) // pad_to * pad_to
    out = torch.empty((C, Rpad), dtype=out_dtype, device=x.device)
    if colsum is not None and _DETERMINISTIC[0]:
        _dev(colsum, torch.float32)[:C].add_(x.sum(0, dtype=torch.float32))
        colsum = None
    _check(lib.alpro_transpose(_ptr(x), _CODE[x.dtype], x.stride(0), _ptr(out), _CODE[out_dtype], Rpad, R, C, Rpad,
                               _ptr(_dev(colsum, torch.float32)) if colsum is not None else None, _stream()), "alpro_transpose")
    return out


def gather_cast(src, dtype, rows=None, map_mode=MAP_IDENTITY, map_p0=0, map_p1=0, row_scale=None, row_scale_group=1, cls_scale=1.0,
                drop_p=0.0, drop_seed=0, colsum=None, colsum_pre=None):
    lib = load()
    _dev(src, torch.float32)
    D = src.shape[-1]
    rows = rows if rows is not None else src.numel() // D
    out = torch.empty((rows, D), dtype=dtype, device=src.device)
    ws, wsb = _reduce_ws(src.device) if (colsum is not None or colsum_pre is not None) else (None, 0)
    _check(lib.alpro_gather_cast(_ptr(src), D, _ptr(out), _CODE[dtype], rows, D, map_mode, map_p0, map_p1,
                                 _ptr(_dev(row_scale, torch.float32)) if row_scale is not None else None, row_scale_group, cls_scale, drop_p, drop_seed,
                                 _ptr(_dev(colsum, torch.float32)) if colsum is not None else None,
                                 _ptr(_dev(colsum_pre, torch.float32)) if colsum_pre is not None else None, ws, wsb, _stream()),
           "alpro_gather_cast")
    return out


def gelu_bwd(dh, u):
    lib = load()
    _dev(dh); _dev(u, dh.dtype)
    du = torch.empty_like(dh)
    _check(lib.alpro_gelu_bwd(_ptr(dh), _ptr(u), _ptr(du), _CODE[dh.dtype], dh.numel(), _stream()), "alpro_gelu_bwd")
    return du


def cls_mean_bwd(dx_out, B, T):
    lib = load()
    _dev(dx_out, torch.float32)
    D = dx_out.shape[-1]
    dside = torch.empty((B * T, D), dtype=torch.float32, device=dx_out.device)
    _check(lib.alpro_cls_mean_bwd(_ptr(dx_out), dx_out.stride(0), _ptr(dside), B, T, D, _stream()), "alpro_cls_mean_bwd")
    return dside


_SCATTER_KEYS = {}


def scatter_add_rows(src, idx, dst, idx_mod=0, skip_idx=-1):
    lib = load()
    _dev(src, torch.float32); _dev(dst, torch.float32)
    if idx is not None and _DETERMINISTIC[0]:
        idx = _dev(idx, torch.int64).view(-1)
        if src.shape[0] <= 8192 and dst.shape[0] < (1 << 19) and src.is_contiguous() and dst.is_contiguous():
            ws = _SCATTER_KEYS.get(src.device)
            if ws is None:
                ws = _SCATTER_KEYS[src.device] = torch.empty(8192, dtype=torch.int32, device=src.device)
            _check(lib.alpro_scatter_add_rows_ordered(_ptr(src), _ptr(idx), _ptr(dst), src.shape[0], src.shape[1], dst.shape[0], int(skip_idx), _ptr(ws), _stream()),
                   "alpro_scatter_add_rows_ordered")
            return dst
        rows = src if skip_idx < 0 else src * (idx != skip_idx).unsqueeze(1).to(src.dtype)
        dst.index_put_((idx,), rows, accumulate=True)
        return dst
    _check(lib.alpro_scatter_add_rows(_ptr(src), _ptr(_dev(idx, torch.int64)) if idx is not None else None, _ptr(dst), src.shape[0], idx_mod,
                                      src.shape[1], int(skip_idx), _stream()), "alpro_scatter_add_rows")
    return dst


def attn(qkv, batch, L, H, scale, key_bias=None, want_lse=False, drop_p=0.0, drop_seed=0, cls_q=None, cls_group=1, cls_out=None):
    lib = load()
    _dev(qkv)
    assert qkv.shape[0] == batch * L
    out = torch.empty((batch * L, H * 64), dtype=qkv.dtype, device=qkv.device)
    lse = torch.empty((batch, H, L), dtype=torch.float32, device=qkv.device) if want_lse else None
    kb = _dev(key_bias, torch.float32) if key_bias is not None else None
    if cls_q is None:
        cls_out = None
    else:
        _dev(cls_q, torch.float32)
        if cls_q.shape != (batch // cls_group, 3 * H * 64) or batch % cls_group or not cls_q.is_contiguous():
            raise RuntimeError("attn: cls_q %s does not match batch=%d H=%d cls_group=%d" % (tuple(cls_q.shape), batch, H, cls_group))
        if cls_out is None:
            cls_out = torch.empty((batch, H * 64), dtype=torch.float32, device=qkv.device)
        assert cls_out.shape == (batch, H * 64) and cls_out.is_contiguous()
        _dev(cls_out, torch.float32)
    _check(lib.alpro_attn_fwd(_ptr(qkv), _ptr(out), _CODE[qkv.dtype], batch, L, H, scale, _ptr(kb), _ptr(lse), drop_p, drop_seed,
                              _ptr(cls_q), cls_group, _ptr(cls_out), _stream()), "alpro_attn_fwd")
    res = (out,) + ((lse,) if want_lse else ()) + ((cls_out,) if cls_q is not None else ())
    return res if len(res) > 1 else out


def _window(r, L):
    if r is None:
        return 0, L
    lo, hi = int(r[0]), int(r[1])
    return lo, hi - lo


def attn_probs(qkv, lse, batch, L, H, scale, key_bias=None, q_range=None, k_range=None):
    for name, t in (("qkv", qkv), ("lse", lse)) + ((("key_bias", key_bias),) if key_bias is not None else ()):
        if not isinstance(t, torch.Tensor) or not t.is_cuda:
            raise RuntimeError("attn_probs: %s must be a device tensor (got %s): the hot path has no CPU fallback" % (name, getattr(t, "device", type(t))))
    lib = load()
    batch, L, H = int(batch), int(L), int(H)
# ... 226 lines not shown
    _check(lib.alpro_cls_mean_residual(_ptr(_dev(x_in, torch.float32)), x_in.stride(0), _ptr(_dev(side, torch.float32)), _ptr(x_out), x_out.stride(0),
                                       B, T, D, _stream()), "alpro_cls_mean_residual")
    return x_out


def vit_final_pool(x, gamma, beta, eps, B, T, N, dtype):
    lib = load()
    _dev(x, torch.float32)
    D = x.shape[-1]
    out32 = torch.empty((B, N + 1, D), dtype=torch.float32, device=x.device)
    out_t = torch.empty((B, N + 1, D), dtype=dtype, device=x.device) if dtype != torch.float32 else None
    _check(lib.alpro_vit_final_pool(_ptr(x), _ptr(gamma), _ptr(beta), eps, _ptr(out32), _ptr(out_t), _CODE[dtype], B, T, N, D, _stream()),
           "alpro_vit_final_pool")
    return out32, (out_t if out_t is not None else out32)


def _pool_out_shape(mode, B, T, N, D):
    if mode not in (POOL_TEMPORAL, POOL_SPATIAL, POOL_NONE):
        raise RuntimeError("final pool: bad mode %r (POOL_TEMPORAL / POOL_SPATIAL / POOL_NONE)" % (mode,))
    return {POOL_TEMPORAL: (B, 1 + N, D), POOL_SPATIAL: (B, 1 + T, D), POOL_NONE: (B, T, 1 + N, D)}[mode]


def vit_final_pool_mode(x, gamma, beta, eps, B, T, N, dtype, mode):
    lib = load()
    D = x.shape[-1]
    shape = _pool_out_shape(mode, B, T, N, D)
    _dev(x, torch.float32)
    if gamma.numel() != D or beta.numel() != D:
        raise RuntimeError("vit_final_pool_mode: gamma / beta hold %d / %d elements, not %d" % (gamma.numel(), beta.numel(), D))
    out32 = torch.empty(shape, dtype=torch.float32, device=x.device)
    out_t = torch.empty(shape, dtype=dtype, device=x.device) if dtype != torch.float32 else None
    _check(lib.alpro_vit_final_pool_mode(_ptr(x), _ptr(_dev(gamma, torch.float32)), _ptr(_dev(beta, torch.float32)), eps, _ptr(out32), _ptr(out_t),
                                         _CODE[dtype], mode, x.numel() // D, B, T, N, D, _stream()), "alpro_vit_final_pool_mode")
    return out32, (out_t if out_t is not None else out32)


def vit_final_pool_mode_bwd(dout, x, gamma, eps, dgamma, dbeta, B, T, N, mode, emit=None):
    lib = load()
    _dev(dout, torch.float32); _dev(x, torch.float32); _dev(dgamma, torch.float32); _dev(dbeta, torch.float32)
    D = x.shape[-1]
    rows = x.numel() // D
    if tuple(dout.shape) != _pool_out_shape(mode, B, T, N, D):
        raise RuntimeError("vit_final_pool_mode_bwd: dout is %s, mode %d at B=%d T=%d N=%d needs %s" % (tuple(dout.shape), mode, B, T, N, _pool_out_shape(mode, B, T, N, D)))
    if gamma.numel() != D or dgamma.numel() != D or dbeta.numel() != D:
        raise RuntimeError("vit_final_pool_mode_bwd: gamma / dgamma / dbeta hold %d / %d / %d elements, not %d" % (gamma.numel(), dgamma.numel(), dbeta.numel(), D))
    dx = torch.empty_like(x)
    out = sc = None
    group = 1
    if emit is not None:
        out = torch.empty((rows, D), dtype=emit["dtype"], device=x.device)
        sc, group = emit.get("scale"), emit.get("group", 1)
        if sc is not None and (_dev(sc, torch.float32).numel() * group < rows or group <= 0):
            raise RuntimeError("vit_final_pool_mode_bwd: %d row scales for groups of %d rows do not cover %d rows" % (sc.numel(), group, rows))
    ws, wsb = _reduce_ws(x.device)
    _check(lib.alpro_vit_final_pool_mode_bwd(_ptr(dout), _ptr(x), _ptr(_dev(gamma, torch.float32)), eps, _ptr(dx), _ptr(dgamma), _ptr(dbeta), mode, rows, B, T, N, D,
                                             _ptr(out), _CODE[out.dtype] if out is not None else F32, _ptr(sc), group, ws, wsb, _stream()),
           "alpro_vit_final_pool_mode_bwd")
    return dx if emit is None else (dx, out)


def bert_embed(ids, word, pos, type_emb, gamma, beta, eps, dtype, stats=False, drop_p=0.0, drop_seed=0):
    lib = load()
    _dev(ids, torch.int64)
    B, L = ids.shape
    D = word.shape[1]
    rows = B * L
    y32 = torch.empty((rows, D), dtype=torch.float32, device=ids.device)
    y_t = torch.empty((rows, D), dtype=dtype, device=ids.device) if dtype != torch.float32 else None
    mean = torch.empty(rows, dtype=torch.float32, device=ids.device) if stats else None
    rstd = torch.empty(rows, dtype=torch.float32, device=ids.device) if stats else None
    _check(lib.alpro_bert_embed_fwd(_ptr(ids), _ptr(_dev(word, torch.float32)), _ptr(_dev(pos, torch.float32)), _ptr(_dev(type_emb, torch.float32)),
                                    _ptr(gamma), _ptr(beta), eps, _ptr(y32), _ptr(y_t), _CODE[dtype], _ptr(mean), _ptr(rstd), rows, L, D,
                                    drop_p, drop_seed, _stream()), "alpro_bert_embed_fwd")
    if stats:
        return y32, (y_t if y_t is not None else y32), mean, rstd
    return y32, (y_t if y_t is not None else y32)


def cast(src, dtype, out=None):
    lib = load()
    _dev(src, torch.float32)
    if dtype == torch.float32:
        return src
    dst = out if out is not None else torch.empty(src.shape, dtype=dtype, device=src.device)
    assert dst.dtype == dtype and dst.numel() == src.numel() and dst.is_contiguous()
    _check(lib.alpro_cast_from_f32(_ptr(src), _ptr(dst), _CODE[dtype], src.numel(), _stream()), "alpro_cast_from_f32")
    return dst


def sumsq(x, out):
    lib = load()
    _dev(x, torch.float32); _dev(out, torch.float32)
    ws, wsb = _reduce_ws(x.device)
    _check(lib.alpro_sumsq(_ptr(x), x.numel(), _ptr(out), ws, min(wsb, 1 << 16), _stream()), "alpro_sumsq")
    return out


def adamw_step(p, g, m, v, lr, beta1, beta2, eps, weight_decay, step_size, gnorm_sq=None, max_norm=0.0, grad_scale=1.0, dyn_state=None,
               grads_scaled=True, correct_bias=True, zero_grad=False, lp=None):
    lib = load()
    for t in (p, g, m, v):
        _dev(t, torch.float32)
    if dyn_state is not None:
        _dev(dyn_state, torch.float32)
        assert dyn_state.numel() >= 4 and gnorm_sq is not None
    if lp is not None:
        _dev(lp)
        if lp.dtype not in (torch.float16, torch.bfloat16) or lp.numel() != p.numel() or not lp.is_contiguous():
            raise RuntimeError("adamw_step: lp must be a contiguous 16-bit tensor with p's number of elements")
    _check(lib.alpro_adamw_step_lp(_ptr(p), _ptr(g), _ptr(m), _ptr(v), p.numel(), lr, beta1, beta2, eps, weight_decay, step_size,
# ... 17 lines not shown
    tab.count = len(segments)
    for dst, s in zip(tab.seg, segments):
        dst.end, dst.lr, dst.beta1, dst.beta2, dst.eps = int(s["end"]), s["lr"], s["beta1"], s["beta2"], s["eps"]
        dst.weight_decay, dst.step_size, dst.correct_bias = s["weight_decay"], s["step_size"], int(bool(s["correct_bias"]))
    _check(lib.alpro_adamw_step_groups(_ptr(p), _ptr(g), _ptr(m), _ptr(v), p.numel(), ctypes.byref(tab), _ptr(gnorm_sq), max_norm, grad_scale,
                                       _ptr(dyn_state), int(bool(grads_scaled)), int(bool(zero_grad)), _ptr(lp), _CODE[lp.dtype] if lp is not None else 0,
                                       _stream()),
           "alpro_adamw_step_groups")


def loss_scale_update(dyn_state, gnorm_sq, growth=2.0, backoff=0.5, window=2000, min_scale=1.0, max_scale=2.0 ** 24):
    _dev(dyn_state, torch.float32); _dev(gnorm_sq, torch.float32)
    _check(load().alpro_loss_scale_update(_ptr(dyn_state), _ptr(gnorm_sq), growth, backoff, int(window), min_scale, max_scale, _stream()),
           "alpro_loss_scale_update")


_TN_WORKSPACE = {}


def _tn_workspace(device, nbytes):
    key = (device.index, torch.cuda.current_stream(device).cuda_stream)
    ws = _TN_WORKSPACE.get(key)
    if ws is None or ws.numel() < nbytes:
        ws = _TN_WORKSPACE[key] = torch.empty(max(nbytes, 64 << 20), dtype=torch.uint8, device=device)
    return ws


_DETERMINISTIC_WGRAD = [os.environ.get("ALPRO_ATOMIC_WGRAD", "0") != "1"]
_DETERMINISTIC = [os.environ.get("ALPRO_DETERMINISTIC", "1") != "0"]


def set_deterministic_wgrad(on=True):
    _DETERMINISTIC_WGRAD[0] = bool(on)


def set_deterministic(on=True):
    _DETERMINISTIC[0] = bool(on)


def deterministic():
    return _DETERMINISTIC[0]


_REDUCE_WS_BYTES = 8192 * 3 * 768 * 4 + 4096 * 768 * 4


def _reduce_ws(device):
    if not _DETERMINISTIC[0]:
        return None, 0
    ws = _tn_workspace(device, _REDUCE_WS_BYTES)
    return _ptr(ws), _REDUCE_WS_BYTES


def gemm_tn_acc(a, b, c, colsum=None, atomic=None):
    lib = load()
    _dev(a); _dev(b, a.dtype); _dev(c, torch.float32)
    assert a.shape[0] == b.shape[0] and tuple(c.shape) == (a.shape[1], b.shape[1])
    if colsum is not None:
        _dev(colsum, torch.float32)
        assert colsum.numel() >= a.shape[1]
    M, N, K = a.shape[0], a.shape[1], b.shape[1]
    if atomic is None:
        atomic = not _DETERMINISTIC_WGRAD[0] and M > 65536 and ((N + 255) // 256) * ((K + 255) // 256) > 9
    if atomic:
        _check(lib.alpro_gemm_tn_acc(_ptr(a), a.stride(0), _ptr(b), b.stride(0), _ptr(c), c.stride(0), _CODE[a.dtype], M, N, K, _ptr(colsum), _stream()),
               "alpro_gemm_tn_acc")
        return c
    ws = _tn_workspace(a.device, lib.alpro_gemm_tn_workspace_bytes(M, N, K))
    _check(lib.alpro_gemm_tn_acc_ws(_ptr(a), a.stride(0), _ptr(b), b.stride(0), _ptr(c), c.stride(0), _CODE[a.dtype], M, N, K, _ptr(colsum),
                                    _ptr(ws), ws.numel(), _stream()), "alpro_gemm_tn_acc_ws")
    return c


def colsum_tn(a, K, colsum):
    lib = load()
    _dev(a); _dev(colsum, torch.float32)
    M, N = a.shape
    assert colsum.numel() >= N
    ws = _tn_workspace(a.device, lib.alpro_gemm_tn_workspace_bytes(M, N, K))
    _check(lib.alpro_colsum_tn(_ptr(a), a.stride(0), _CODE[a.dtype], M, N, K, _ptr(colsum), _ptr(ws), ws.numel(), _stream()), "alpro_colsum_tn")
    return colsum


def transpose_jobs(pairs):
    jobs = (TransposeJob * len(pairs))()
    t0 = 0
    for j, (src, out) in zip(jobs, pairs):
        _dev(src, torch.float32); _dev(out)
        assert src.dim() == 2 and out.dim() == 2 and src.stride(1) == 1 and out.stride(1) == 1 and out.shape[0] == src.shape[1] and out.shape[1] >= src.shape[0]
        j.in_, j.out, j.ld_in, j.ld_out = src.data_ptr(), out.data_ptr(), src.stride(0), out.stride(0)
        j.R, j.C, j.Rpad, j.tile0 = src.shape[0], src.shape[1], out.shape[1], t0
        t0 += ((src.shape[1] + 63) // 64) * ((out.shape[1] + 63) // 64)
    table = torch.frombuffer(bytearray(bytes(jobs)), dtype=torch.uint8).to(pairs[0][0].device)
    return table, len(pairs), t0


def transpose_batch(table, njobs, total_tiles, out_dtype):
    _check(load().alpro_transpose_batch(_ptr(table), njobs, total_tiles, _CODE[out_dtype], _stream()), "alpro_transpose_batch")


def colsum_acc(a, out):
    lib = load()
    _dev(a); _dev(out, torch.float32)
    _check(lib.alpro_colsum_acc(_ptr(a), a.stride(0), _ptr(out), _CODE[a.dtype], a.shape[0], a.shape[1], _stream()), "alpro_colsum_acc")
    return out


def softmax_xent(logits, labels, grad_dtype=None, grad_scale=None, ignore_index=-100, pad_to=64):
    lib = load()
    _dev(logits, torch.float32); _dev(labels, torch.int64)
    M, V = logits.shape
    loss_rows = torch.empty(M, dtype=torch.float32, device=logits.device)
    dl, Vp = None, (V + pad_to - 1) // pad_to * pad_to
    if grad_dtype is not None:
        dl = torch.empty((M, Vp), dtype=grad_dtype, device=logits.device)
        _dev(grad_scale, torch.float32)
    _check(lib.alpro_softmax_xent(_ptr(logits), logits.stride(0), _ptr(labels), ignore_index, _ptr(loss_rows), _ptr(dl),
                                  _CODE[grad_dtype] if grad_dtype is not None else 0, Vp, _ptr(grad_scale), M, V, Vp, _stream()),
           "alpro_softmax_xent")
    return (loss_rows, dl) if dl is not None else loss_rows


def vtc_loss_fwd(v, t, gv, gt, temp, col0):
    lib = load()
    for x in (v, t, gv, gt):
        _dev(x, torch.float32)
        assert x.is_contiguous()
    _dev(temp, torch.float32)
    B, E = v.shape
    G = gv.shape[0]
    sim_v2t = torch.empty((B, G), dtype=torch.float32, device=v.device)
# ... 146 lines not shown
```

alpro_amd/modeling/timesformer/vit.py:

```python
import math
from functools import partial

import torch
import torch.nn as nn

from alpro_amd import config as rt
from alpro_amd import hip
from alpro_amd.modeling import train as tr
from alpro_amd.modeling.weights import OperandCache, param_version

VIT_EPS = 1e-6


def trunc_normal_(tensor, mean=0., std=1., a=-2., b=2.):
    return nn.init.trunc_normal_(tensor, mean=mean, std=std, a=a, b=b)


def to_2tuple(x):
    return tuple(x) if isinstance(x, (tuple, list)) else (x, x)


class DropPath(nn.Module):

    def __init__(self, drop_prob=None):
# ... 428 lines not shown
                     map_mode=hip.MAP_FRAME_TOKENS, map_p0=T, map_p1=N, side=cls_rows)
            hip.cls_mean_residual(xt, cls_rows, x2, B, T)
            h2 = hip.layernorm(x2, self.norm2.weight, self.norm2.bias, VIT_EPS, dt)
        u, u_tiled = tr.gelu_save_buffer(B * S, mlp.fc1.out_features, D, dt, dev) if save else (None, False)
        f1 = hip.gemm(h2, self._w("fc1", mlp.fc1, dt), bias=mlp.fc1.bias, act=hip.ACT_GELU_SAVE_GRAD if save else hip.ACT_GELU, pre_act=u, c2_tiled=u_tiled)
        out = hip.gemm(f1, self._w("fc2", mlp.fc2, dt), out=None if (save or cls_only) else xf, bias=mlp.fc2.bias, out_dtype=f32,
                       residual=x2.view(-1, D), **rs_m)
        if cls_only:
            return out
        out = out.view(B, S, D) if save else x
        if cp:
            ev_out = torch.cuda.current_stream().record_event() if side is not None else None
            x2_c = x2[:, 0] if save else (side.buf("x2_c", (B, D), dev) if side is not None else torch.empty_like(x_cls_in))
            self._cls_chain(x_cls_in, o_c, B, T, drop_s, drop_m, x2_c, out[:, 0], side, ev_mid, ev_out)
        if not save:
            return out
        return out, dict(x=x, dims=(B, T, N, S, D, H), dt=dt, drop_t=drop_t, drop_s=drop_s, drop_m=drop_m, attn_drop=seeds, merged=merged, u_tiled=u_tiled,
                         h=h, qkv_t=qkv_t, a_t=a_t, lse_t=lse_t, pr=pr, xt=xt, hs=hs, qkv_s=qkv_s, a_s=a_s, lse_s=lse_s, x2=x2, h2=h2, u=u, f1=f1)

    SLIM_KEYS = ("x", "drop_t", "drop_s", "drop_m", "attn_drop", "dims", "dt", "merged", "u_tiled")

    @staticmethod
    def slim_saved(sv):
        return {k: sv[k] for k in Block.SLIM_KEYS}

    def replay(self, slim, W, cls_precise=None):
        B, T = slim["dims"][0], slim["dims"][1]
        out, sv = self._forward(slim["x"], B, T, save=True, drop_masks=(slim["drop_t"], slim["drop_s"], slim["drop_m"]), replay=slim, cls_precise=cls_precise)
        _ClsSide.join(out.device)
        return sv

    def _wt(self, name, lin, dt):
        return tr.transposed_operand(self._ops, name + "^T", lin.weight, dt)

    def _merged_tproj_backward(self, sv, dx, B, T, N, D, dt, G=None):
        ta, fc = self.temporal_attn, self.temporal_fc
        wp, bp, wf = ta.proj.weight.detach(), ta.proj.bias.detach(), fc.weight.detach()
        mg = self._merged_tproj(dt)
        dev = dx.device
        if G is None:
            G = hip.gather_cast(dx, dt, rows=B * N * T, map_mode=hip.MAP_SKIP_CLS, map_p0=N * T, row_scale=sv["drop_t"], row_scale_group=T,
                                colsum_pre=tr.bias_grad(fc.bias))
        t_fc, t_p, t_bp = tr.trainable(fc.weight), tr.trainable(ta.proj.weight), tr.trainable(ta.proj.bias)
        if not (t_fc or t_p or t_bp):
            return tr.dgrad(G, mg["wT"])
        ws = sv.get("ws")
        if ws is None:
            ws = torch.zeros(D * D + D, dtype=torch.float32, device=dev)
        dWe, db1 = ws[:D * D].view(D, D), ws[D * D:]
        cs = db1 if (t_fc or t_bp) else None
        if dt != torch.float32 and not (t_fc or t_p):
            hip.colsum_tn(G, sv["a_t"].shape[1], db1)
        elif dt != torch.float32:
            hip.gemm_tn_acc(G, sv["a_t"], dWe, colsum=cs)
        elif t_fc or t_p:
            hip.gemm(hip.transpose(G, colsum=cs), hip.transpose(sv["a_t"]), out=dWe, out_dtype=torch.float32)
        else:
            db1.add_(G.sum(0, dtype=torch.float32))
        da = tr.dgrad(G, mg["wT"])
        if sv.get("defer_product_rule"):
            return da
        g_fc, g_p = tr.grad_target(fc.weight), tr.grad_target(ta.proj.weight)
        if dt != torch.float32:
            if g_fc is not None:
                hip.gemm(hip.cast(dWe, dt), self._w("t_proj", ta.proj, dt), out=g_fc, out_dtype=torch.float32, residual=g_fc)
            if g_p is not None:
                hip.gemm(self._wt("t_fc", fc, dt)[:, :D], hip.transpose(dWe, out_dtype=dt), out=g_p, out_dtype=torch.float32, residual=g_p)
        else:
            if g_fc is not None:
                hip.gemm(dWe, wp.contiguous(), out=g_fc, out_dtype=torch.float32, residual=g_fc)
            if g_p is not None:
                hip.gemm(hip.transpose(wf.contiguous()), hip.transpose(dWe), out=g_p, out_dtype=torch.float32, residual=g_p)
        if g_fc is not None:
            g_fc.addr_(db1, bp)
        if t_bp:
            tr.bias_grad(ta.proj.bias).add_(torch.mv(wf.t(), db1))
        return da

    def backward(self, sv, dx, dz=None, emit_for=None):
        B, T, N, S, D, H = sv["dims"]
        dt = sv["dt"]
        ta, sa = self.temporal_attn, self.attn
        ap_t, seed_t, ap_s, seed_s = sv["attn_drop"]
        if dz is None:
            dz = hip.gather_cast(dx, dt, row_scale=sv["drop_m"], row_scale_group=S)
        tr.wgrad(dz, sv["f1"], self.mlp.fc2.weight, self.mlp.fc2.bias)
        du = tr.dgrad(dz, self._wt("fc2", self.mlp.fc2, dt), gelu_grad=sv["u"], gelu_tiled=sv["u_tiled"])
        del dz
        tr.wgrad(du, sv["h2"], self.mlp.fc1.weight, self.mlp.fc1.bias)
        dh2 = tr.dgrad(du, self._wt("fc1", self.mlp.fc1, dt))
        g, b_ = tr.grad_target(self.norm2.weight), tr.grad_target(self.norm2.bias)
        _, dpo = hip.layernorm_bwd(dh2, sv["x2"], self.norm2.weight, VIT_EPS, dx, g, b_,
                                   emit=dict(mode=hip.EMIT_FRAME, rows=B * T * (N + 1), dtype=dt, T=T, N=N, scale=sv["drop_s"]))
        tr.wgrad(dpo, sv["a_s"], sa.proj.weight, sa.proj.bias)
        da = tr.dgrad(dpo, self._wt("s_proj", sa.proj, dt))
        del dpo
        dqkv = hip.attn_bwd(sv["qkv_s"], sv["a_s"], da, sv["lse_s"], B * T, N + 1, H, sa.scale, drop_p=ap_s, drop_seed=seed_s)
        tr.wgrad(dqkv, sv["hs"], sa.qkv.weight, sa.qkv.bias)
        dhs = tr.dgrad(dqkv, self._wt("s_qkv", sa.qkv, dt))
        g, b_ = tr.grad_target(self.norm1.weight), tr.grad_target(self.norm1.bias)
        G = None
        if sv["merged"]:
            _, G = hip.layernorm_bwd(dhs, sv["xt"], self.norm1.weight, VIT_EPS, dx, g, b_, rows=B * T * (N + 1), map_mode=hip.MAP_FRAME_TOKENS,
                                     map_p0=T, map_p1=N, emit=dict(mode=hip.EMIT_SKIP_CLS, rows=B * N * T, dtype=dt, T=T, N=N, scale=sv["drop_t"], group=T,
                                                                   colsum_pre=tr.bias_grad(self.temporal_fc.bias)))
        else:
            hip.layernorm_bwd(dhs, sv["xt"], self.norm1.weight, VIT_EPS, dx, g, b_, rows=B * T * (N + 1),
# ... 100 lines not shown
                hip.cast(st["we32"].view(-1), dt, out=st["we_dt"].view(-1))
            hip.transpose_batch(*st["t_we"], dt)
            hip.tproj_small(*st["t_b1"], D, 0)
        st["key"] = key
        self.state = st
        from alpro_amd.modeling import weights
        weights.note_operand_rebuild()
        return st

    def workspace(self, dt, device):
        nb, D = len(self.blocks), self.blocks[0].temporal_fc.weight.shape[0]
        b = self.bwd
        if b is None or b["ws"].device != device or b["dt"] != dt:
            ws = torch.empty((nb, D * D + D), dtype=torch.float32, device=device)
            b = self.bwd = dict(dt=dt, ws=ws, ws_dt=torch.empty((nb, D * D + D), dtype=dt, device=device) if dt != torch.float32 else None,
                                dweT=torch.empty((nb, D, D), dtype=dt, device=device))
            self._bwd_tables = {}
        b["ws"].zero_()
        return b["ws"]

    def all_trainable(self, idx):
        blk = self.blocks[idx]
        return all(tr.trainable(p) for p in (blk.temporal_fc.weight, blk.temporal_attn.proj.weight, blk.temporal_attn.proj.bias))

    def product_rule(self, lo, hi, dt, idx=None):
        assert dt != torch.float32 and self.bwd is not None
        idx = tuple(range(lo, hi)) if idx is None else tuple(idx)
        if not idx:
            return
        b, blocks = self.bwd, [self.blocks[i] for i in idx]
        D = blocks[0].temporal_fc.weight.shape[0]
        ops = []
        for i, blk in zip(idx, blocks):
            ta, fc = blk.temporal_attn, blk.temporal_fc
            g_fc, g_p = tr.grad_buffer(fc.weight, zero=True)[0], tr.grad_buffer(ta.proj.weight, zero=True)[0]
            g_bp = tr.bias_grad(ta.proj.bias)
            ops.append(dict(i=i, wp_dt=blk._w("t_proj", ta.proj, dt), wfT_dt=blk._wt("t_fc", fc, dt), g_fc=g_fc, g_p=g_p, g_bp=g_bp,
                            wf=fc.weight.detach(), bp=ta.proj.bias.detach()))
        sig = tuple((o["wp_dt"].data_ptr(), o["wfT_dt"].data_ptr(), o["g_fc"].data_ptr(), o["g_p"].data_ptr(), o["g_bp"].data_ptr(), o["wf"].data_ptr())
                    for o in ops)
        tb = self._bwd_tables.get(idx)
        if tb is None or tb["sig"] != sig:
            ga, gbb = hip.GemmBatch(), hip.GemmBatch()
            for o in ops:
                dwe_dt = b["ws_dt"][o["i"], :D * D].view(D, D)
                ga.add(dwe_dt, o["wp_dt"], out=o["g_fc"], out_dtype=torch.float32, residual=o["g_fc"])
                gbb.add(o["wfT_dt"][:, :D], b["dweT"][o["i"]], out=o["g_p"], out_dtype=torch.float32, residual=o["g_p"])
            tb = dict(sig=sig, ga=ga, gb=gbb, keep=ops,
                      t_dwe=hip.transpose_jobs([(b["ws"][o["i"], :D * D].view(D, D), b["dweT"][o["i"]]) for o in ops]),
                      t_small=hip.tproj_jobs([dict(wfc=o["wf"], bp=o["bp"], db1=b["ws"][o["i"], D * D:], g_fc=o["g_fc"], g_bp=o["g_bp"]) for o in ops],
                                             b["ws"].device))
            self._bwd_tables[idx] = tb
        lo, hi = idx[0], idx[-1] + 1
        hip.cast(b["ws"][lo:hi].reshape(-1), dt, out=b["ws_dt"][lo:hi].reshape(-1))
        hip.transpose_batch(*tb["t_dwe"], dt)
        tb["ga"].launch()
        tb["gb"].launch()
        hip.tproj_small(*tb["t_small"], D, 1)


class PatchEmbed(nn.Module):

    def __init__(self, img_size=224, patch_size=16, in_chans=3, embed_dim=768):
        super().__init__()
        img_size, patch_size = to_2tuple(img_size), to_2tuple(patch_size)
        assert patch_size == (16, 16), "alpro_patchify is specialised for 16x16 patches (ViT-B/16)"
        self.img_size, self.patch_size = img_size, patch_size
        self.num_patches = (img_size[1] // patch_size[1]) * (img_size[0] // patch_size[0])
        self.proj = nn.Conv2d(in_chans, embed_dim, kernel_size=patch_size, stride=patch_size)


class VisionTransformer(nn.Module):
    def __init__(self, img_size=224, patch_size=16, in_chans=3, num_classes=1000, embed_dim=768, depth=12, num_heads=12,
                 mlp_ratio=4., qkv_bias=False, qk_scale=None, drop_rate=0., attn_drop_rate=0., drop_path_rate=0.1,
                 hybrid_backbone=None, norm_layer=nn.LayerNorm, num_frames=8, attention_type='divided_space_time', dropout=0.,
                 cross_attention_config=None, use_grad_checkpointing=False):
        super().__init__()
        assert drop_rate == 0., "drop_rate must be 0 (pos / time / proj / MLP dropout is not implemented; attn_drop_rate is)"
        self.attention_type = attention_type
        self.depth = depth
        self.num_classes = num_classes
        self.num_features = self.embed_dim = embed_dim
        self.patch_embed = PatchEmbed(img_size=img_size, patch_size=patch_size, in_chans=in_chans, embed_dim=embed_dim)
        num_patches = self.patch_embed.num_patches
        self.cls_token = nn.Parameter(torch.zeros(1, 1, embed_dim))
        self.pos_embed = nn.Parameter(torch.zeros(1, num_patches + 1, embed_dim))
        self.time_embed = nn.Parameter(torch.zeros(1, num_frames, embed_dim))
        dpr = [x.item() for x in torch.linspace(0, drop_path_rate, self.depth)]
        self.blocks = nn.ModuleList([
            Block(layer_num=i, use_grad_checkpointing=use_grad_checkpointing, dim=embed_dim, num_heads=num_heads,
                  mlp_ratio=mlp_ratio, qkv_bias=qkv_bias, qk_scale=qk_scale, drop=drop_rate, attn_drop=attn_drop_rate,
                  drop_path=dpr[i], norm_layer=norm_layer, attention_type=self.attention_type) for i in range(self.depth)])
        self.norm = norm_layer(embed_dim)
        self.head = nn.Linear(embed_dim, num_classes) if num_classes > 0 else nn.Identity()
        trunc_normal_(self.pos_embed, std=.02)
        trunc_normal_(self.cls_token, std=.02)
        self.apply(self._init_weights)
        for i, blk in enumerate(self.blocks):
            if i > 0:
                nn.init.constant_(blk.temporal_fc.weight, 0)
                nn.init.constant_(blk.temporal_fc.bias, 0)
        self._ops = OperandCache()
        self._attach_bank()

    def _attach_bank(self):
        self._tproj_bank = _MergedTProjBank(self.blocks)
# ... 253 lines not shown
            out32, _ = hip.vit_final_pool_mode(tok, m.norm.weight, m.norm.bias, VIT_EPS, B, T, N, torch.float32, self.mode)
        return out32

    def backward(self, dout):
        m = self.enc.model
        B, T, N = self.dims
        D = m.embed_dim
        nb, nfro = len(m.blocks), self.nfro
        g, b_ = tr.grad_target(m.norm.weight), tr.grad_target(m.norm.bias)
        S_ = 1 + N * T
        last = self.saved[-1] if self.saved else None
        emit_dt = last["dt"] if last is not None else rt.compute_dtype()
        if self.mode == hip.POOL_TEMPORAL:
            dy = torch.empty((B, 1 + N * T, D), dtype=torch.float32, device=dout.device)
            dy[:, 0] = dout[:, 0]
            torch.mul(dout[:, 1:].unsqueeze(2).expand(B, N, T, D), 1.0 / T, out=dy[:, 1:].view(B, N, T, D))
            dtok = torch.empty_like(dy)
            r = hip.layernorm_bwd(dy.view(-1, D), self.tok, m.norm.weight, VIT_EPS, dtok, g, b_, accumulate=False,
                                  emit=dict(mode=hip.EMIT_ROWS, rows=B * S_, dtype=emit_dt, scale=last["drop_m"], group=S_) if last is not None else None)
            dz = r[1] if last is not None else None
            del dy, r
        else:
            if g is None or b_ is None:
                tg, tb = hip.ln_throwaway_pair(dout.device)
                g, b_ = (tg if g is None else g), (tb if b_ is None else b_)
            r = hip.vit_final_pool_mode_bwd(dout, self.tok, m.norm.weight, VIT_EPS, g, b_, B, T, N, self.mode,
                                            emit=dict(dtype=emit_dt, scale=last["drop_m"], group=S_) if last is not None else None)
            dtok, dz = r if last is not None else (r, None)
        if last is None:
            return self._embed_backward(dtok)
        bank = m.blocks[0]._bank()
        dt_run = last["dt"]
        banked = bank is not None and dt_run != torch.float32 and all(sv["merged"] for sv in self.saved)
        ws = bank.workspace(dt_run, dout.device) if banked else torch.zeros((nb, D * D + D), dtype=torch.float32, device=dout.device)
        from alpro_amd import dist
        overlap = dist.collectives_active() and not getattr(self, "others_pending", False)
        if overlap:
            dist.grads_final(all_but=list(self.enc.parameters()))
        group_hi, group_rule = nb, []
        marks = {}
        for j in range(nb - 1, nfro - 1, -1):
            blk, sv = m.blocks[j], self.saved[j - nfro]
            if self.recompute:
                ev = marks.pop(j + 2, None)
                if ev is not None:
                    ev.synchronize()
                sv = blk.replay(sv, self.Wg, cls_precise=self.cp)
                self.saved[j - nfro] = None
            sv["ws"] = ws[j]
            sv["defer_product_rule"] = banked and bank.all_trainable(j)
            if sv["defer_product_rule"]:
                group_rule.insert(0, j)
            dtok, dz = blk.backward(sv, dtok, dz=dz, emit_for=self.saved[j - 1 - nfro] if j > nfro else None)
            done = nb - j
            if done % 4 == 0 or j == nfro:
                if banked:
                    bank.product_rule(j, group_hi, dt_run, idx=group_rule)
                if overlap and j > nfro:
                    dist.grads_final(params=[p for b in m.blocks[j:group_hi] for p in b.parameters()] + (list(m.norm.parameters()) if group_hi == nb else []))
                group_hi, group_rule = j, []
            sv.clear()
            if self.recompute:
                marks[j] = rt.wgrad_side_event(dtok.device)
        return self._embed_backward(dtok)

    def _embed_backward(self, dtok):
        B, T, N = self.dims
        dx = None
        if not self.embed_frozen:
            dx = self.enc.model._embed_backward(self.rows, dtok, B, T, N, self.Wg, pixel_grad=self.x_grad is not None)
        self.saved = self.rows = self.tok = None
        if dx is None:
            return None
        return dx.to(self.x_grad[1]).transpose(1, 2)
```

alpro_amd/modeling/train.py:

```python
import weakref

import torch

from alpro_amd import hip
from alpro_amd.modeling.weights import param_version


def trainable(p):
    return p is not None and p.requires_grad


def grad_target(p, zero=True):
    return grad_buffer(p, zero=zero)[0] if trainable(p) else None


def frozen_prefix(stages, input_needs_grad=False):
    if input_needs_grad:
        return 0
    n = 0
    for params in stages:
        if any(trainable(p) for p in params):
            break
        n += 1
    return n


def grad_buffer(p, zero=False):
    if p.grad is not None and (p.grad.numel() <= 1 or any(p.grad.stride())):
        return p.grad, True
    p.grad = torch.zeros_like(p, memory_format=torch.contiguous_format) if zero else torch.empty_like(p, memory_format=torch.contiguous_format)
    return p.grad, False


def add_grad(p, g):
    if not trainable(p):
        return
    if p.grad is None or (p.grad.numel() > 1 and not any(p.grad.stride())):
        p.grad = g.detach().clone().reshape(p.shape).contiguous()
    else:
        p.grad.add_(g.reshape(p.shape))


def fused_param_view(params):
    ps = [p.detach() for p in params]
    if any(not p.is_contiguous() for p in ps):
        return None
    base = ps[0]
    off = base.data_ptr()
    for p in ps:
        if p.untyped_storage().data_ptr() != base.untyped_storage().data_ptr() or p.data_ptr() != off or p.shape[1:] != base.shape[1:]:
            return None
        off += p.numel() * 4
    rows = sum(p.shape[0] for p in ps)
    return torch.as_strided(base, (rows, base.numel() // base.shape[0]), (base.numel() // base.shape[0], 1))


_WT_REGISTRY = {}
_WT_TABLE = {}


def transposed_operand(cache, key, weight, dt):
    plist = (weight,) if torch.is_tensor(weight) else tuple(weight)
    ver = tuple(param_version(p) for p in plist)
    hit = cache._store.get(key)
    if hit is not None and hit[0] == ver and hit[1].dtype == dt:
        return hit[1]
    with torch.no_grad():
        src = fused_param_view(plist) if len(plist) > 1 else plist[0].detach().reshape(plist[0].shape[0], -1)
        if src is None:
            src = torch.cat([p.detach().reshape(p.shape[0], -1) for p in plist], 0)
        src = src.contiguous()
        out = hip.transpose(src, out_dtype=dt, pad_to=64)
    cache._store[key] = (ver, out)
    stable = src.data_ptr() == plist[0].data_ptr() and all(v[0] >= 0 for v in ver)
    if stable and src.dtype == torch.float32 and src.is_cuda:
        _WT_REGISTRY[(id(cache), key)] = dict(cache=weakref.ref(cache), key=key, params=[weakref.ref(p) for p in plist], src=src, out=out)
    else:
        _WT_REGISTRY.pop((id(cache), key), None)
    return out


def refresh_transposed_operands():
    live = []
    for k, e in list(_WT_REGISTRY.items()):
        cache, ps = e["cache"](), [r() for r in e["params"]]
        hit = cache._store.get(e["key"]) if cache is not None else None
        if hit is None or hit[1] is not e["out"] or any(p is None for p in ps) or ps[0].data_ptr() != e["src"].data_ptr():
            del _WT_REGISTRY[k]
            continue
        live.append((e, cache, ps))
    if not live:
        return 0
    t = _WT_TABLE
    by_dtype = {}
    for item in live:
        by_dtype.setdefault(item[0]["out"].dtype, []).append(item)
    n = 0
    for dt, items in by_dtype.items():
        sig = tuple((e["src"].data_ptr(), e["out"].data_ptr()) for e, _, _ in items)
        slot = t.setdefault(dt, {})
        if slot.get("sig") != sig:
            slot["table"], slot["njobs"], slot["tiles"] = hip.transpose_jobs([(e["src"], e["out"]) for e, _, _ in items])
            slot["sig"] = sig
        hip.transpose_batch(slot["table"], slot["njobs"], slot["tiles"], dt)
        for e, cache, ps in items:
            cache._store[e["key"]] = (tuple(param_version(p) for p in ps), e["out"])
        n += len(items)
    return n


def bias_grad(bias):
    return grad_target(bias)


def fused_grad_view(params):
    gs = [p.grad for p in params]
    if any(g is None or not g.is_contiguous() for g in gs):
        return None
    base = gs[0]
    off = base.data_ptr()
    for g in gs:
        if g.untyped_storage().data_ptr() != base.untyped_storage().data_ptr() or g.data_ptr() != off or g.shape[1:] != base.shape[1:]:
            return None
        off += g.numel() * 4
    rows = sum(g.shape[0] for g in gs)
    return torch.as_strided(base, (rows,) + tuple(base.shape[1:]), base.stride())


def wgrad(dy_t, x_t, weight, bias, bias_done=False):
    if bias_done or not trainable(bias):
        bias = None
    want_w = trainable(weight)
    if not want_w and bias is None:
        return
    gb = grad_buffer(bias, zero=True)[0] if bias is not None else None
    if want_w:
        gw = grad_buffer(weight, zero=True)[0]
        gw2 = gw.view(gw.shape[0], -1)
    if dy_t.dtype != torch.float32:
        if not want_w:
            hip.colsum_tn(dy_t, x_t.shape[1], gb)
            return
        from alpro_amd import config as rt
        side = rt.wgrad_side_stream(dy_t.device)
        if side is None:
            hip.gemm_tn_acc(dy_t, x_t, gw2, colsum=gb)
            return
        side.wait_stream(torch.cuda.current_stream(dy_t.device))
        with torch.cuda.stream(side):
            hip.gemm_tn_acc(dy_t, x_t, gw2, colsum=gb)
        dy_t.record_stream(side)
        x_t.record_stream(side)
        return
    if not want_w:
        gb[:dy_t.shape[1]].add_(dy_t.sum(0, dtype=torch.float32))
        return
    dyT = hip.transpose(dy_t, colsum=gb)
    hip.gemm(dyT, hip.transpose(x_t), out=gw2, out_dtype=torch.float32, residual=gw2)


def gelu_save_buffer(M, N, K, dt, device):
    rows = hip.gemm_c2_tiled_rows(M, N, K, dt)
    return torch.empty((rows or M, N), dtype=dt, device=device), rows > 0


def dgrad(dy_t, wT, out_dtype=None, row_scale=None, row_scale_group=1, gelu_grad=None, gelu_tiled=False):
    n = dy_t.shape[1]
    w = wT if wT.shape[1] == n else wT[:, :n]
    if not w.is_contiguous() or n % (64 if dy_t.dtype != torch.float32 else 32) != 0:
        pad = wT.shape[1] - n
        dy_t = torch.nn.functional.pad(dy_t, (0, pad))
        w = wT
    return hip.gemm(dy_t, w, out_dtype=out_dtype or dy_t.dtype, row_scale=row_scale, row_scale_group=row_scale_group,
                    act=hip.ACT_MUL_SAVED if gelu_grad is not None else hip.ACT_NONE, pre_act=gelu_grad, c2_tiled=gelu_tiled)


_LIVE_ANCHORS = weakref.WeakSet()


BACKWARD_EPOCH = [0]


class Anchor(torch.autograd.Function):

    @staticmethod
    def forward(ctx, run, n_act, *inputs):
        ctx.run = run
        ctx.n_act = n_act
        ctx.n_in = len(inputs)
        from alpro_amd import config as rt
        ctx.dt = rt.compute_dtype()
        ctx.set_materialize_grads(False)
        _LIVE_ANCHORS.add(ctx)
        with torch.no_grad():
            outs = run.forward(*inputs[:n_act])
        ctx.single = torch.is_tensor(outs)
        return outs

    @staticmethod
    def backward(ctx, *grads):
        ctx.run.others_pending = any(c is not ctx for c in _LIVE_ANCHORS)
        BACKWARD_EPOCH[0] += 1
        from alpro_amd import config as rt
        rt.check_backward_precision(getattr(ctx.run, "dt", None) or ctx.dt)
        rt.wgrad_scope(True)
        try:
            with torch.no_grad():
                g = ctx.run.backward(*[None if x is None else x.contiguous() for x in grads])
        finally:
            rt.wgrad_scope(False)
            rt.join_wgrad()
            _LIVE_ANCHORS.discard(ctx)
        if grads and any(x is not None and x.is_cuda for x in grads):
            cur = torch.cuda.current_stream()
            if rt.is_text_side_stream(cur):
                ev = cur.record_event()
                torch.autograd.Variable._execution_engine.queue_callback(lambda: torch.cuda.current_stream().wait_event(ev))
        g = (g,) if (torch.is_tensor(g) or g is None) else tuple(g)
        g = g + (None,) * (ctx.n_act - len(g))
        ctx.run = None
        return (None, None) + tuple(g) + (None,) * (ctx.n_in - ctx.n_act)


def run_anchored(run, activations, params):
    params = [p for p in params if p.requires_grad]
    need = torch.is_grad_enabled() and (any(torch.is_tensor(a) and a.requires_grad for a in activations) or len(params) > 0)
    if not need:
        with torch.no_grad():
            return run.forward(*activations)
    return Anchor.apply(run, len(activations), *activations, *params)
```

alpro_amd/modeling/xbert.py:

```python
import math
import os
from types import SimpleNamespace

import torch
import torch.nn as nn

from alpro_amd import config as rt
from alpro_amd import hip
from alpro_amd.modeling import train as tr
from alpro_amd.modeling.weights import OperandCache


def _cfg_get(cfg, name, default=None):
    if isinstance(cfg, dict):
        return cfg.get(name, default)
    return getattr(cfg, name, default)


class BertEmbeddings(nn.Module):
    def __init__(self, config):
        super().__init__()
        self.word_embeddings = nn.Embedding(config.vocab_size, config.hidden_size, padding_idx=config.pad_token_id)
        self.position_embeddings = nn.Embedding(config.max_position_embeddings, config.hidden_size)
        self.token_type_embeddings = nn.Embedding(config.type_vocab_size, config.hidden_size)
# ... 159 lines not shown
        if save and attn_grads is not None:
            sv["attn_grads"], sv["pass_index"] = attn_grads, pass_index
        return o32, o_t, sv

    def backward(self, sv, do32, do_t):
        B, L, H, scale = sv["dims"]
        dt = sv["dt"]
        sa, so = self.attention.self, self.attention.output
        eps = self.config.layer_norm_eps
        dev = sv["s1"].device
        M, D = sv["s1"].shape

        def ln_bwd(ln, x, dy_t, dy32, drop_seed):
            if dy_t is None:
                dy_t, dy32 = dy32, None
            dx = torch.empty((M, D), dtype=torch.float32, device=dev)
            g, b_ = tr.grad_target(ln.weight), tr.grad_target(ln.bias)
            _, dx_t = hip.layernorm_bwd(dy_t, x, ln.weight, eps, dx, g, b_, dy2=dy32, accumulate=False,
                                        emit=dict(mode=hip.EMIT_ROWS, rows=M, dtype=dt, drop_p=hp if drop_seed else 0.0, drop_seed=drop_seed))
            return dx, dx_t

        hp, seed1, seed2, ap, seed_a = sv["drop"]
        ds2, ds2_t = ln_bwd(self.output.LayerNorm, sv["s2"], do_t, do32, seed2)
        tr.wgrad(ds2_t, sv["it"], self.output.dense.weight, self.output.dense.bias)
        du = tr.dgrad(ds2_t, tr.transposed_operand(self._ops, "o_w^T", self.output.dense.weight, dt), gelu_grad=sv["u"], gelu_tiled=sv["u_tiled"])
        tr.wgrad(du, sv["a_t"], self.intermediate.dense.weight, self.intermediate.dense.bias)
        da_t = tr.dgrad(du, tr.transposed_operand(self._ops, "i_w^T", self.intermediate.dense.weight, dt))
        ds1, ds1_t = ln_bwd(so.LayerNorm, sv["s1"], da_t, ds2, seed1)
        tr.wgrad(ds1_t, sv["ctx"], so.dense.weight, so.dense.bias)
        dctx = tr.dgrad(ds1_t, tr.transposed_operand(self._ops, "ao_w^T", so.dense.weight, dt))
        rows = sv.get("rows")
        if rows is not None:
            full = torch.zeros((sv["M_full"], D), dtype=dctx.dtype, device=dev)
            full.index_copy_(0, rows, dctx)
            dctx = full
            full32 = torch.zeros((sv["M_full"], D), dtype=torch.float32, device=dev)
            full32.index_copy_(0, rows, ds1)
            ds1 = full32
        collector = sv.get("attn_grads")
        if collector is not None:
            collector.add(sv["pass_index"], sv["qkv"], dctx, sv["lse"], sv["dims"], sv["kb"])
        if sa.save_attention:
            sa.save_attn_gradients(hip.attn_probs_grad(sv["qkv"], dctx, sv["lse"], B, L, H, scale, sv["kb"], want=("grad",)))
        dqkv = hip.attn_bwd(sv["qkv"], sv["ctx_full"], dctx, sv["lse"], B, L, H, scale, sv["kb"], drop_p=ap, drop_seed=seed_a)
        Hd = sa.all_head_size
        lins = (sa.query, sa.key, sa.value)
        gw = gb = None
        if dqkv.dtype != torch.float32 and all(tr.trainable(q) for lin in lins for q in (lin.weight, lin.bias)):
            for lin in lins:
                tr.grad_buffer(lin.weight, zero=True)
                tr.grad_buffer(lin.bias, zero=True)
            gw, gb = tr.fused_grad_view([l.weight for l in lins]), tr.fused_grad_view([l.bias for l in lins])
        if gw is not None and gb is not None:
            hip.gemm_tn_acc(dqkv, sv["h_t"], gw, colsum=gb)
        else:
            for i, lin in enumerate(lins):
                tr.wgrad(dqkv[:, i * Hd:(i + 1) * Hd], sv["h_t"], lin.weight, lin.bias)
        wT = (None, tr.transposed_operand(self._ops, "qkv_w^T", (sa.query.weight, sa.key.weight, sa.value.weight), dt))
        dh_t = tr.dgrad(dqkv, wT[1])
        return ds1, dh_t


class _AttnTap:

    def __init__(self, window=None):
        self.q_range, self.k_range = window if window is not None else (None, None)
        self.maps = []

    def add(self, qkv, lse, B, L, H, scale, key_bias):
        self.maps.append(hip.attn_probs(qkv, lse, B, L, H, scale, key_bias, q_range=self.q_range, k_range=self.k_range))


class AttnGradients:

    def __init__(self, layers=None, window=None, want=("cam",), grad_scale=1.0):
        self.layers = None if layers is None else tuple(int(l) for l in layers)
        self.q_range, self.k_range = window if window is not None else (None, None)
        self.want = (want,) if isinstance(want, str) else tuple(want)
        if not self.want or len(set(self.want)) != len(self.want) or any(w not in ("grad", "cam") for w in self.want):
            raise ValueError("AttnGradients: want=%r (one or both of 'grad', 'cam')" % (want,))
        if self.layers is not None and not self.layers:
            raise ValueError("AttnGradients: no layer chosen")
        self.grad_scale = float(grad_scale)
        if not self.grad_scale > 0 or not math.isfinite(self.grad_scale):
            raise ValueError("AttnGradients: grad_scale=%r (a positive finite number)" % (grad_scale,))
        self._pick, self._pending = (), None
        self._grads, self._cams = {}, {}

    def begin(self, n):
        idx = range(n) if self.layers is None else self.layers
        for i in idx:
            if not -n <= i < n:
                raise ValueError("AttnGradients: layer %d outside the %d layers of the pass" % (i, n))
        self._pick = tuple(sorted(set(i % n for i in idx)))
        self._pending = set(self._pick)
        self._grads, self._cams = {}, {}

    def wants(self, i):
        return i in self._pick

    def first(self):
        return self._pick[0]

    def add(self, i, qkv, dctx, lse, dims, key_bias):
        if i not in self._pending:
            return
        B, L, H, scale = dims
# ... 241 lines not shown
            B, L = ti.numel(), text_pool.shape[1] + video_pool.shape[1]
            self.pool_dims = (text_pool.shape[0], video_pool.shape[0], text_pool.shape[1], video_pool.shape[1])
            h32, h_t = hip.gather_seq(text_pool.contiguous().float(), video_pool.contiguous().float(), ti, vi, dt)
            if h_t is None:
                h_t = h32
        elif encoder_embeds is None:
            B, L = self.ids.shape
            self.ids = self.ids.contiguous()
            word = emb.word_embeddings.weight
            ep = float(cfg.hidden_dropout_prob) if emb.training else 0.0
            self.emb_drop = (ep, rt.next_dropout_seed() if ep > 0 else 0)
            h32, h_t = hip.bert_embed(self.ids, word, emb.position_embeddings.weight, emb.token_type_embeddings.weight,
                                      emb.LayerNorm.weight, emb.LayerNorm.bias, cfg.layer_norm_eps, dt,
                                      drop_p=self.emb_drop[0], drop_seed=self.emb_drop[1])
        else:
            B, L, Hd = encoder_embeds.shape
            h32 = encoder_embeds.reshape(B * L, Hd).contiguous().float()
            h_t = hip.cast(h32, dt)
        mask = self.mask if self.mask is not None else torch.ones((B, L), device=h32.device)
        kb = m.key_bias(mask)
        self.dims = (B, L)
        self.from_ids = encoder_embeds is None and self.parts is None
        self.saved = []
        lo, hi = m.encoder.layer_range(self.mode)
        stages = ([list(emb.parameters())] if self.from_ids else []) + [list(m.encoder.layer[i].parameters()) for i in range(lo, hi)]
        k = tr.frozen_prefix(stages, any(torch.is_tensor(a) and a.requires_grad for a in (encoder_embeds, video_pool)))
        first = lo + max(k - (1 if self.from_ids else 0), 0)
        watched = [i for i in range(lo, first) if m.encoder.layer[i].attention.self.save_attention]
        if self.grads is not None:
            watched.append(lo + self.grads.first())
        first = min([first] + watched)
        self.range = (first, hi)
        self.prefix = k > 0
        for i in range(lo, hi):
            rows = self.out_rows if i == hi - 1 else None
            if self.hidden is not None:
                self.hidden.append(_hidden_copy(h32, B, L))
            if i < first:
                h32, h_t = m.encoder.layer[i](h32, h_t, kb, B, L, rows=rows, tap=self.tap)
                continue
            h32, h_t, sv = m.encoder.layer[i].forward_train(h32, h_t, kb, B, L, rows=rows, tap=self.tap, attn_grads=self.grads, pass_index=i - lo)
            self.saved.append(sv)
        if self.hidden is not None:
            self.hidden.append(_hidden_copy(h32, B, L, self.out_rows))
        return h32.view(B, L, -1) if self.out_rows is None else h32

    def backward(self, dout):
        m, cfg = self.m, self.m.config
        B, L = self.dims
        lo, hi = self.range
        d32, d_t = (dout.reshape(B * L, -1) if self.out_rows is None else dout.reshape(self.out_rows.numel(), -1)).contiguous(), None
        for i in range(hi - 1, lo - 1, -1):
            d32, d_t = m.encoder.layer[i].backward(self.saved.pop(), d32, d_t)
        if self.prefix:
            return None
        if self.parts is not None:
            if d_t is not None and d_t.dtype == torch.float32:
                d32, d_t = d32 + d_t, None
            return hip.gather_seq_bwd(d32.contiguous(), None if d_t is None else d_t.contiguous(), self.parts[0], self.parts[1], *self.pool_dims)
        if not self.from_ids:
            return (d32 + d_t.float()).view(B, L, -1)
        emb = m.embeddings
        D = d32.shape[1]
        tw, tp, tt = (tr.trainable(e.weight) for e in (emb.word_embeddings, emb.position_embeddings, emb.token_type_embeddings))
        g, b_ = tr.grad_target(emb.LayerNorm.weight), tr.grad_target(emb.LayerNorm.bias)
        if not (tw or tp or tt or g is not None or b_ is not None):
            return None
        pre = (emb.word_embeddings.weight.detach()[self.ids.view(-1)] + emb.token_type_embeddings.weight.detach()[0]
               + emb.position_embeddings.weight.detach()[:L].repeat(B, 1)).contiguous()
        de = torch.empty_like(pre)
        hip.layernorm_bwd(d_t, pre, emb.LayerNorm.weight, cfg.layer_norm_eps, de, g, b_, dy2=d32, accumulate=False,
                          drop_p=self.emb_drop[0], drop_seed=self.emb_drop[1])
        if tw:
            gw = tr.grad_buffer(emb.word_embeddings.weight, zero=True)[0] if emb.word_embeddings.weight.grad is None else emb.word_embeddings.weight.grad
            pad = emb.word_embeddings.padding_idx
            hip.scatter_add_rows(de, self.ids.view(-1), gw, skip_idx=-1 if pad is None else int(pad))
        if tp:
            gp = tr.grad_buffer(emb.position_embeddings.weight, zero=True)[0] if emb.position_embeddings.weight.grad is None else emb.position_embeddings.weight.grad
            hip.scatter_add_rows(de, None, gp, idx_mod=L)
        if tt:
            gt = tr.grad_buffer(emb.token_type_embeddings.weight, zero=True)[0] if emb.token_type_embeddings.weight.grad is None else emb.token_type_embeddings.weight.grad
            gt[0].add_(de.sum(0))
        return None


class BertPredictionHeadTransform(nn.Module):
    def __init__(self, config):
        super().__init__()
        self.dense = nn.Linear(config.hidden_size, config.hidden_size)
        self.LayerNorm = nn.LayerNorm(config.hidden_size, eps=config.layer_norm_eps)


class BertLMPredictionHead(nn.Module):
    def __init__(self, config):
        super().__init__()
        self.config = config
        self.transform = BertPredictionHeadTransform(config)
        self.decoder = nn.Linear(config.hidden_size, config.vocab_size, bias=False)
        self.bias = nn.Parameter(torch.zeros(config.vocab_size))
        self.decoder.bias = self.bias
        self._ops = OperandCache()

    def forward(self, hidden_states):
        if torch.is_grad_enabled() and (hidden_states.requires_grad or any(p.requires_grad for p in self.parameters())):
            return tr.run_anchored(_LMHeadRun(self), [hidden_states], list(self.parameters()))
        dt = rt.compute_dtype()
# ... 125 lines not shown
```

alpro_amd/optim.py:

```python
import math

import torch

from alpro_amd import dist, hip
from alpro_amd import config as rt
from alpro_amd.modeling.weights import bump_param_epoch, register_flat_lp


_ZERO = {}


def placeholder_grad(p):
    if p.numel() <= 1:
        return torch.zeros_like(p)
    key = (p.device, p.dtype)
    z = _ZERO.get(key)
    if z is None:
        z = _ZERO[key] = torch.zeros(1, dtype=p.dtype, device=p.device)
    return z.expand(p.shape)


def is_placeholder_grad(g):
    return g is not None and g.dim() > 0 and g.numel() > 1 and not any(g.stride())

# ... 296 lines not shown
    def _finish_exchange(self):
        n = self.flat["n"]
        rec = self.record_exchange
        on_gpu = rec and self.flat["g"].is_cuda
        if rec:
            import time
            t0 = time.perf_counter()
            if on_gpu:
                e0, e1 = torch.cuda.Event(enable_timing=True), torch.cuda.Event(enable_timing=True)
                e0.record()
        late = [0, 0]
        pos = 0
        for s, e in self._merge(self._reduced) + [(n, n)]:
            for c in range(pos, s, self.bucket_elems):
                self._launch(c, min(s, c + self.bucket_elems))
                late[0] += 1
                late[1] += min(s, c + self.bucket_elems) - c
            pos = max(pos, e)
        for h, w, g in self._inflight:
            h.wait()
            if w is not None:
                g.copy_(w)
        self._inflight, self._reduced = [], []
        if rec:
            if on_gpu:
                e1.record()
            wire = 4 if self.wire_dtype in (None, torch.float32) else torch.empty(0, dtype=self.wire_dtype).element_size()
            self.exchange_log.append(dict(ranges_on_wire_early=self._early[0], bytes_on_wire_early=self._early[1] * wire, ranges_at_synchronize=late[0],
                                          bytes_at_synchronize=late[1] * wire, cu_budget=self._budget_seen if self._cus_reserved else None,
                                          events=(e0, e1) if on_gpu else None, host_ms=(time.perf_counter() - t0) * 1e3))
        self._early = [0, 0]
        self._reserve_cus(False)

    def exchange_stats(self, last=None):
        log = self.exchange_log[-last:] if last else self.exchange_log
        if not log:
            return None
        ms = []
        for r in log:
            if r["events"] is not None:
                r["events"][1].synchronize()
                ms.append(r["events"][0].elapsed_time(r["events"][1]))
            else:
                ms.append(r["host_ms"])
        k = float(len(log))
        budgets = sorted({r["cu_budget"] for r in log if r["cu_budget"] is not None})
        return dict(exchanges=len(log), comm_exposed_ms=round(sum(ms) / k, 3), comm_exposed_ms_max=round(max(ms), 3),
                    ranges_on_wire_early=round(sum(r["ranges_on_wire_early"] for r in log) / k, 2), bytes_on_wire_early=int(sum(r["bytes_on_wire_early"] for r in log) / k),
                    ranges_at_synchronize=round(sum(r["ranges_at_synchronize"] for r in log) / k, 2), bytes_at_synchronize=int(sum(r["bytes_at_synchronize"] for r in log) / k),
                    cu_budget_while_in_flight=budgets[0] if len(budgets) == 1 else (budgets or None), overlap_backward=bool(self.overlap_backward),
                    timer="device events on the compute stream" if log[0]["events"] is not None else "host clock (CPU tensors)")

    def synchronize(self, average=False):
        if not self.allreduce or not dist.collectives_active():
            self._note_synced("avg" if average else None)
            return 0
        if self._sync_is_current() and not self._inflight:
            if average and self._pre_synced == "sum":
                if self.flat is not None:
                    self.flat["g"].div_(dist.size())
                else:
                    for p in self.params:
                        if real_grad(p) is not None:
                            p.grad.div_(dist.size())
                self._note_synced("avg")
            return 0
        if self._pre_synced == "sum":
            raise RuntimeError("FlatAdamW.synchronize: gradients were accumulated on top of an already exchanged SUM; with several backward "
                               "passes per step call synchronize(average=True) after each of them (hvd.DistributedOptimizer.synchronize does) "
                               "or only once before step()")
        if self.flat is None:
            dist.allreduce_grads_(self.params, average=average)
            self._note_synced("avg" if average else "sum")
            return 0
        g, n = self.flat["g"], self.flat["n"]
        self._finish_exchange()
        if average:
            g.div_(dist.size())
        self._note_synced("avg" if average else "sum")
        return n * 4

    def backward(self, loss):
        self._g_clean = False
        self._writes += 1
        return self._backward(loss)

    def _backward(self, loss):
        from alpro_amd import amp
        if not amp.needs_loss_scaling():
            return loss.backward()
        sc = amp.scaler_for(self).to(loss.device)
        self._grads_scaled = True
        with rt.loss_scaling(sc):
            (loss * sc.scale.reshape(())).backward()

    def step(self, closure=None):
        if self._pre_synced is not None and not (self._sync_is_current() and not self._inflight) and self.allreduce and dist.collectives_active():
            self.synchronize(average=self._pre_synced == "avg")
        pre = self._pre_synced
        self._note_synced(None)
        if self.flat is None and not self._build():
            return None
        f, grp = self.flat, self.param_groups[0]
        late = [p for p in self.params if real_grad(p) is not None and (p.grad.data_ptr() < f["g"].data_ptr() or p.grad.data_ptr() >= f["g"].data_ptr() + f["n"] * 4)]
        if late:
            raise RuntimeError("%d parameters started receiving gradients after the flat buffers were built" % len(late))
        if pre is None:
            self.synchronize()
            self._note_synced(None)
        world = dist.size() if (self.allreduce and pre != "avg") else 1
        if self.scaler is not None and getattr(self, "_scaler_steps_synced", None) is not self.scaler:
            self.scaler.to(f["g"].device).state[2] = float(self.step_count)
            self._scaler_steps_synced = self.scaler
        self.step_count += 1
        lr, (b1, b2) = grp["lr"], grp["betas"]
        step_size = lr
        if grp["correct_bias"]:
            step_size = lr * math.sqrt(1.0 - b2 ** self.step_count) / (1.0 - b1 ** self.step_count)
        grouped = len(self.param_groups) > 1
        norm = None
        sc = self.scaler
        if sc is not None:
            sc.to(f["g"].device)
        if (self.max_grad_norm is not None and self.max_grad_norm > 0) or sc is not None:
            norm = f["norm"]
            norm.zero_()
            hip.sumsq(f["g"], norm)
            self.last_grad_norm = norm
        dt = rt.compute_dtype()
        lp = None
        if dt != torch.float32:
            if f.get("lp") is None or f["lp"].dtype != dt:
                f["lp"] = torch.empty(f["n"], dtype=dt, device=f["p"].device)
                hip.cast(f["p"], dt, out=f["lp"])
            lp = f["lp"]
        held = [(a, e, f["p"][a:e].clone(), f["m"][a:e].clone(), f["v"][a:e].clone())
                for a, e in self._merge([self._span[id(p)] for p in f["live"] if not p.requires_grad])]
        if grouped:
            hip.adamw_step_groups(f["p"], f["g"], f["m"], f["v"], self._segments(self.step_count), norm, float(self.max_grad_norm or 0.0), 1.0 / world,
                                  dyn_state=sc.state if sc is not None else None, grads_scaled=self._grads_scaled, zero_grad=self.fused_zero_grad, lp=lp)
        else:
            hip.adamw_step(f["p"], f["g"], f["m"], f["v"], lr, b1, b2, grp["eps"], grp["weight_decay"], step_size, norm,
                           float(self.max_grad_norm or 0.0), 1.0 / world, dyn_state=sc.state if sc is not None else None,
                           grads_scaled=self._grads_scaled, correct_bias=grp["correct_bias"], zero_grad=self.fused_zero_grad, lp=lp)
        for a, e, hp, hm, hv in held:
            f["p"][a:e].copy_(hp)
            f["m"][a:e].copy_(hm)
            f["v"][a:e].copy_(hv)
            if lp is not None:
# ... 60 lines not shown
```

include/alpro_hip.h:

```cpp
#ifndef ALPRO_HIP_H
#define ALPRO_HIP_H

#include <stddef.h>
#include <stdint.h>

#ifdef __cplusplus
extern "C" {
#endif

#define ALPRO_HIP_ABI_VERSION 22

enum { ALPRO_OK = 0, ALPRO_ERR_INVALID = 1, ALPRO_ERR_LAUNCH = 2 };
enum { ALPRO_F32 = 0, ALPRO_BF16 = 1, ALPRO_F16 = 2 };
enum { ALPRO_ACT_NONE = 0, ALPRO_ACT_GELU = 1, ALPRO_ACT_RELU = 2, ALPRO_ACT_GELU_BWD = 3,
       ALPRO_ACT_GELU_SAVE_GRAD = 4, ALPRO_ACT_MUL_SAVED = 5,
       ALPRO_ACT_RELU_MASK = 6 };

enum { ALPRO_MAP_IDENTITY = 0, ALPRO_MAP_SKIP_CLS = 1, ALPRO_MAP_FRAME_TOKENS = 2, ALPRO_MAP_PATCH_EMBED = 3 };

const char* alpro_hip_last_error(void);
int alpro_hip_abi_version(void);
int alpro_hip_set_option(const char* name, int value);
int alpro_hip_set_stream_option(void* stream, const char* name, int value);
size_t alpro_hip_sched_workspace_bytes(void);
// ... 134 lines not shown
                   void* stream);
int alpro_attn_temporal_bwd(const void* qkv, const void* out, const void* dout, const float* lse, void* dqkv, int dtype,
                            int64_t rows, int T, int H, float scale, void* stream);
int alpro_attn_temporal_bwd_drop(const void* qkv, const void* out, const void* dout, const float* lse, void* dqkv, int dtype,
                                 int64_t rows, int T, int H, float scale, float drop_p, uint32_t drop_seed, void* stream);

int alpro_layernorm_bwd(const void* dy, int dy_dtype, int64_t ld_dy, const float* dy2, const float* x, int64_t ldx,
                        const float* gamma, float eps, float* dx, int64_t ld_dx, int accumulate, float* dgamma,
                        float* dbeta, int rows, int D, int map_mode, int map_p0, int map_p1, float drop_p,
                        uint32_t drop_seed, void* workspace, size_t workspace_bytes, void* stream);

enum { ALPRO_EMIT_NONE = 0, ALPRO_EMIT_ROWS = 1, ALPRO_EMIT_FRAME = 2, ALPRO_EMIT_SKIP_CLS = 3 };
int alpro_layernorm_bwd_emit(const void* dy, int dy_dtype, int64_t ld_dy, const float* dy2, const float* x, int64_t ldx,
                             const float* gamma, float eps, float* dx, int64_t ld_dx, int accumulate, float* dgamma, float* dbeta,
                             int rows, int D, int map_mode, int map_p0, int map_p1, float drop_p, uint32_t drop_seed, void* emit_out,
                             int emit_dtype , int emit_mode, int emit_p0, int emit_p1, const float* emit_scale, int emit_scale_group, float emit_drop_p,
                             uint32_t emit_drop_seed, float* emit_colsum_pre, int emit_extra_cls, void* workspace, size_t workspace_bytes,
                             void* stream);

int alpro_transpose(const void* in, int in_dtype, int64_t ld_in, void* out, int out_dtype, int64_t ld_out, int R, int C,
                    int Rpad, float* colsum, void* stream);

typedef struct alpro_transpose_job {
  const float* in;
  void* out;
  int64_t ld_in, ld_out;
  int32_t R, C, Rpad, tile0;
} alpro_transpose_job_t;
int alpro_transpose_batch(const alpro_transpose_job_t* jobs, int njobs, int total_tiles, int out_dtype, void* stream);

int alpro_gather_cast(const float* src, int64_t ld, void* out, int dtype, int rows, int D, int map_mode, int map_p0,
                      int map_p1, const float* row_scale, int row_scale_group, float cls_scale, float drop_p,
                      uint32_t drop_seed, float* colsum, float* colsum_pre, void* workspace, size_t workspace_bytes, void* stream);

int alpro_gelu_bwd(const void* dh, const void* u, void* du, int dtype, int64_t n, void* stream);

int alpro_cls_mean_bwd(const float* dx_out, int64_t ld_batch, float* dside, int B, int T, int D, void* stream);

int alpro_scatter_add_rows(const float* src, const int64_t* idx, float* dst, int rows, int idx_mod, int D, int64_t skip_idx, void* stream);
int alpro_scatter_add_rows_ordered(const float* src, const int64_t* idx, float* dst, int rows, int D, int64_t dst_rows, int64_t skip_idx, uint32_t* keys_ws,
                                   void* stream);

int alpro_gemm_tn_acc(const void* A, int64_t lda, const void* B, int64_t ldb, float* C, int64_t ldc, int dtype, int M,
                      int N, int K, float* colsum, void* stream);

size_t alpro_gemm_tn_workspace_bytes(int M, int N, int K);
int alpro_gemm_tn_ranges(int M, int N, int K, int compute_units);
int alpro_gemm_tn_acc_ws(const void* A, int64_t lda, const void* B, int64_t ldb, float* C, int64_t ldc, int dtype, int M,
                         int N, int K, float* colsum, void* workspace, size_t workspace_bytes, void* stream);

int alpro_colsum_acc(const void* A, int64_t lda, float* out, int dtype, int M, int N, void* stream);
int alpro_colsum_tn(const void* A, int64_t lda, int dtype, int M, int N, int K, float* colsum, void* workspace, size_t workspace_bytes, void* stream);

int alpro_softmax_xent(const float* logits, int64_t ld, const int64_t* labels, int ignore_index, float* loss_rows,
                       void* dlogits, int dtype, int64_t ldd, const float* grad_scale, int M, int V, int Vpad,
                       void* stream);

int alpro_vtc_loss_fwd(const float* v, const float* t, const float* gv, const float* gt, const float* temp, int B, int G, int E, int col0,
                       float* sim_v2t, float* sim_t2v, float* lse, float* loss, void* stream);
int alpro_vtc_loss_bwd(const float* v, const float* t, const float* gv, const float* gt, const float* temp, int B, int G, int E, int col0,
                       const float* sim_v2t, const float* sim_t2v, const float* lse, const float* dloss, float* ds_v2t, float* ds_t2v,
                       float* dv, float* dt, float* dgv, float* dgt, float* dtemp, void* stream);


int alpro_sumsq(const float* x, int64_t n, float* out, void* workspace, size_t workspace_bytes, void* stream);

int alpro_adamw_step(float* p, float* g, float* m, float* v, int64_t n, float lr, float beta1, float beta2,
                     float eps, float weight_decay, float step_size, const float* gnorm_sq, float max_norm,
                     float grad_scale, const float* dyn_state, int grads_scaled, int correct_bias,
                     int zero_grad , void* stream);
int alpro_adamw_step_lp(float* p, float* g, float* m, float* v, int64_t n, float lr, float beta1, float beta2, float eps, float weight_decay,
                        float step_size, const float* gnorm_sq, float max_norm, float grad_scale, const float* dyn_state, int grads_scaled,
                        int correct_bias, int zero_grad, void* lp, int lp_dtype, void* stream);

#define ALPRO_ADAMW_MAX_SEGMENTS 32
typedef struct alpro_adamw_segment_t {
  int64_t end;
  float lr, beta1, beta2, eps, weight_decay, step_size;
  int32_t correct_bias, reserved0;
} alpro_adamw_segment_t;
typedef struct alpro_adamw_segments_t {
  int32_t count, reserved0;
  alpro_adamw_segment_t seg[ALPRO_ADAMW_MAX_SEGMENTS];
} alpro_adamw_segments_t;
int alpro_adamw_step_groups(float* p, float* g, float* m, float* v, int64_t n, const alpro_adamw_segments_t* segments, const float* gnorm_sq,
                            float max_norm, float grad_scale, const float* dyn_state, int grads_scaled, int zero_grad, void* lp, int lp_dtype,
                            void* stream);

int alpro_loss_scale_update(float* dyn_state, const float* gnorm_sq, float growth, float backoff, int window, float min_scale,
                            float max_scale, void* stream);

#define ALPRO_TOPK_MAX_K 128
size_t alpro_sim_topk_workspace_bytes(int nq, int ng, int k, int chunk);
int alpro_sim_topk(const float* q, int nq, const float* g, int ng, int d, int k, float scale, int chunk, float* out_val, int32_t* out_idx,
                   void* workspace, size_t workspace_bytes, void* stream);

int alpro_attn_probs(const void* qkv, const float* lse, const float* key_bias, float* out, int dtype, int batch, int L, int H, float scale,
                     int q0, int nq, int k0, int nk, void* stream);

int alpro_attn_temporal_probs(const void* qkv, const float* lse, float* out, int dtype, int64_t rows, int T, int H, float scale, void* stream);

int alpro_attn_probs_grad(const void* qkv, const void* dctx, const float* lse, const float* key_bias, float* grad_out, float* cam_out, int dtype,
                          int batch, int L, int H, float scale, float grad_scale, int q0, int nq, int k0, int nk, void* stream);

#ifdef __cplusplus
}
// ... 3 lines not shown
```

Baseline: 437.1.

## Defer and batch split-K and colsum second-stage reductions into grouped launches

```diff
diff --git a/alpro_amd/amp.py b/alpro_amd/amp.py
--- a/alpro_amd/amp.py
+++ b/alpro_amd/amp.py
@@ -76,6 +76,8 @@
 
 def unscale_(optimizer, scaler):
     inner = getattr(optimizer, "_opt", optimizer)
+    from alpro_amd import hip
+    hip.flush_reduce(all_streams=True)
     inv = torch.reciprocal(scaler.scale).reshape(())
     flat = getattr(inner, "flat", None)
     if flat is not None:
diff --git a/alpro_amd/config.py b/alpro_amd/config.py
--- a/alpro_amd/config.py
+++ b/alpro_amd/config.py
@@ -147,10 +147,12 @@
     if not _WGRAD_SIDE:
         return
     import torch
+    from alpro_amd import hip
     for (idx, handle), ent in _WGRAD_SIDE.items():
         if ent[1]:
             cur = torch.cuda.current_stream(idx)
             if cur.cuda_stream == handle:
+                hip.flush_reduce_of(idx, ent[0])
                 cur.wait_stream(ent[0])
                 ent[1] = False
 
@@ -186,10 +188,35 @@
     if not _TEXT_SIDE:
         return
     import torch
+    from alpro_amd import hip
     for (idx, handle), s in _TEXT_SIDE.items():
         cur = torch.cuda.current_stream(idx)
         if cur.cuda_stream == handle:
+            hip.flush_reduce_of(idx, s)
             cur.wait_stream(s)
+
+
+_defer_reduce = [os.environ.get("ALPRO_DEFER_REDUCE", "1") != "0"]
+
+
+def defer_reduce():
+    return _defer_reduce[0]
+
+
+def set_defer_reduce(v):
+    _defer_reduce[0] = bool(v)
+
+
+def flush_deferred_reduce(device):
+    from alpro_amd import hip
+    if device.type != "cuda" or not hip.reduce_pending():
+        return
+    idx = device.index if device.index is not None else torch.cuda.current_device()
+    cur = torch.cuda.current_stream(device)
+    hip.flush_reduce_of(idx, cur)
+    ent = _WGRAD_SIDE.get((idx, cur.cuda_stream))
+    if ent is not None:
+        hip.flush_reduce_of(idx, ent[0])
 
 
 _prompter_stream = [os.environ.get("ALPRO_PROMPTER_STREAM", "1") != "0"]
diff --git a/alpro_amd/csrc/backward.hip b/alpro_amd/csrc/backward.hip
--- a/alpro_amd/csrc/backward.hip
+++ b/alpro_amd/csrc/backward.hip
@@ -1,5 +1,6 @@
 #include "common.hpp"
 #include "row768.hpp"
+#include "reduce_jobs.hpp"
 #include <algorithm>
 
 namespace alpro {
@@ -110,33 +111,19 @@
                                                              float* __restrict__ d1, float* __restrict__ d2) {
   __shared__ float4 red[128][8];
   __shared__ float4 red2[8][8];
-  const int k = blockIdx.y, c4 = threadIdx.x & 7, sl = threadIdx.x >> 3;
-  float* dst = k == 0 ? d0 : (k == 1 ? d1 : d2);
-  if (!dst) return;
-  const int col = blockIdx.x * 32 + c4 * 4;
-  float4 s = make_float4(0.f, 0.f, 0.f, 0.f);
-#pragma unroll 4
-  for (int p = sl; p < nparts; p += 128) {
-    const float4 v = *(const float4*)(part + ((int64_t)p * nslots + k) * LN_D + col);
-    s.x += v.x; s.y += v.y; s.z += v.z; s.w += v.w;
-  }
-  red[sl][c4] = s;
-  __syncthreads();
-  if (sl < 8) {
-    float4 t = red[sl * 16][c4];
-#pragma unroll
-    for (int i = 1; i < 16; ++i) { const float4 v = red[sl * 16 + i][c4]; t.x += v.x; t.y += v.y; t.z += v.z; t.w += v.w; }
-    red2[sl][c4] = t;
-  }
-  __syncthreads();
-  if (sl == 0) {
-    float4 t = red2[0][c4];
-#pragma unroll
-    for (int i = 1; i < 8; ++i) { const float4 v = red2[i][c4]; t.x += v.x; t.y += v.y; t.z += v.z; t.w += v.w; }
-    float4* o = (float4*)(dst + col);
-    const float4 c = *o;
-    *o = make_float4(c.x + t.x, c.y + t.y, c.z + t.z, c.w + t.w);
-  }
+  const int k = blockIdx.y;
+  colsum_reduce_block((int)blockIdx.x, k, red, red2, part, nparts, nslots, k == 0 ? d0 : (k == 1 ? d1 : d2));
+}
+
+static_assert(LN_D == RJ_D, "reduce_jobs.hpp restates the row width");
+bool colsum_second_stage(const float* part, int nparts, int nslots, float* d0, float* d1, float* d2, hipStream_t st) {
+  alpro_reduce_job_t job = {};
+  job.kind = ALPRO_REDUCE_COLSUM;
+  job.part = part; job.dst[0] = d0; job.dst[1] = d1; job.dst[2] = d2; job.nparts = nparts; job.nslots = nslots;
+  const int deferred = defer_reduce_job(job);
+  if (deferred < 0) return false;
+  if (!deferred) hipLaunchKernelGGL(colsum_reduce_kernel, dim3(LN_D / 32, d2 ? 3 : 2), dim3(1024), 0, st, part, nparts, nslots, d0, d1, d2);
+  return true;
 }
 
 __global__ __launch_bounds__(192) void cls_rows_reduce_kernel(const float* __restrict__ cls_ws, float* __restrict__ dx, int64_t ld_dx, int T, int N) {
@@ -588,7 +575,7 @@
   else { set_error("alpro_layernorm_bwd: bad dtype %d", dy_dtype); return ALPRO_ERR_INVALID; }
 #undef ALPRO_LNB
 #undef ALPRO_LNB_K
-  if (part) hipLaunchKernelGGL(colsum_reduce_kernel, dim3(LN_D / 32, emit_colsum_pre ? 3 : 2), dim3(1024), 0, st, part, nblk, 3, dgamma, dbeta, emit_colsum_pre);
+  if (part && !colsum_second_stage(part, nblk, 3, dgamma, dbeta, emit_colsum_pre, st)) return ALPRO_ERR_INVALID;
   if (cls_ws) hipLaunchKernelGGL(cls_rows_reduce_kernel, dim3(rows / (map_p1 + 1) / map_p0), dim3(192), 0, st, cls_ws, dx, ld_dx, map_p0, map_p1);
   return check_launch("alpro_layernorm_bwd");
 }
@@ -629,7 +616,7 @@
   else ALPRO_FPB_MODES(float);
 #undef ALPRO_FPB_MODES
 #undef ALPRO_FPB
-  if (part) hipLaunchKernelGGL(colsum_reduce_kernel, dim3(LN_D / 32, 2), dim3(1024), 0, st, part, nblk, 2, dgamma, dbeta, (float*)nullptr);
+  if (part && !colsum_second_stage(part, nblk, 2, dgamma, dbeta, nullptr, st)) return ALPRO_ERR_INVALID;
   return check_launch("alpro_vit_final_pool_mode_bwd");
 }
 
@@ -646,7 +633,7 @@
     int nblk = grid_for(rows, 32, 512);
     if (part) nblk = (int)std::min<size_t>((size_t)nblk, workspace_bytes / (2 * LN_D * sizeof(float)));
     ALPRO_DISPATCH_DTYPE(dtype, T, hipLaunchKernelGGL((gather_cast_kernel<T, 16>), dim3(nblk), dim3(1024), 0, (hipStream_t)stream, src, ld, (T*)out, (int64_t)rows, map_mode, map_p0, map_p1, row_scale, row_scale_group, cls_scale, drop_p, drop_seed, colsum, colsum_pre, part));
-    if (part) hipLaunchKernelGGL(colsum_reduce_kernel, dim3(LN_D / 32, 2), dim3(1024), 0, (hipStream_t)stream, part, nblk, 2, colsum, colsum_pre, (float*)nullptr);
+    if (part && !colsum_second_stage(part, nblk, 2, colsum, colsum_pre, nullptr, (hipStream_t)stream)) return ALPRO_ERR_INVALID;
   } else {
     ALPRO_DISPATCH_DTYPE(dtype, T, hipLaunchKernelGGL((gather_cast_kernel<T, 4>), dim3(grid_for(rows, 8, 256 * 32)), dim3(256), 0, (hipStream_t)stream, src, ld, (T*)out, (int64_t)rows, map_mode, map_p0, map_p1, row_scale, row_scale_group, cls_scale, drop_p, drop_seed, colsum, colsum_pre, (float*)nullptr));
   }
diff --git a/alpro_amd/csrc/gemm_tn.hip b/alpro_amd/csrc/gemm_tn.hip
--- a/alpro_amd/csrc/gemm_tn.hip
+++ b/alpro_amd/csrc/gemm_tn.hip
@@ -1,4 +1,5 @@
 #include "common.hpp"
+#include "reduce_jobs.hpp"
 
 namespace alpro {
 namespace {
@@ -6,6 +7,7 @@
 constexpr int TM = 32;
 constexpr int NSTAGE = 4;
 constexpr int TW = 256;
+static_assert(TW == RJ_TW, "reduce_jobs.hpp restates the tile width");
 constexpr int ROW_BYTES = TW * 2;
 constexpr int IMG_BYTES = TM * ROW_BYTES;
 constexpr int NT3 = 512;
@@ -243,38 +245,8 @@
 
 __global__ __launch_bounds__(256) void tn_reduce_kernel(const float* __restrict__ part, const float* __restrict__ part_cs, float* __restrict__ C,
                                                         int64_t ldc, float* __restrict__ colsum, int N, int K, int tiles, int ranges, int tn_cnt) {
-  const int tile_blocks = part ? tiles * 64 : 0;
-  if ((int)blockIdx.x >= tile_blocks) {
-    __shared__ float red[8][32];
-    const int c = threadIdx.x & 31, p = threadIdx.x >> 5;
-    const int n = (blockIdx.x - tile_blocks) * 32 + c;
-    const int sets = ranges * (tiles / tn_cnt);
-    float t = 0.f;
-    for (int r = p; r < sets; r += 8) t += part_cs[(int64_t)r * (tn_cnt * TW) + n];
-    red[p][c] = t;
-    __syncthreads();
-    if (p == 0 && n < N) colsum[n] += ((red[0][c] + red[1][c]) + (red[2][c] + red[3][c])) + ((red[4][c] + red[5][c]) + (red[6][c] + red[7][c]));
-    return;
-  }
-  const int tile = blockIdx.x >> 6, f = ((blockIdx.x & 63) << 8) + threadIdx.x;
-  const int lane = f & 63, q = (f >> 6) & 3, j = (f >> 8) & 1, i = (f >> 9) & 3, wave = f >> 11;
-  const int n = (tile % tn_cnt) * TW + (wave >> 2) * 128 + i * 32 + 8 * q + 4 * (lane >> 5);
-  const int k = (tile / tn_cnt) * TW + (wave & 3) * 64 + j * 32 + (lane & 31);
-  const float* src = part + (int64_t)tile * (TW * TW) + f * 4;
-  const int64_t stride = (int64_t)tiles * (TW * TW);
-  f32x4 t = {0.f, 0.f, 0.f, 0.f};
-  int r = 0;
-  for (; r + 4 <= ranges; r += 4) {
-    const f32x4 a = __builtin_nontemporal_load((const f32x4*)(src + (r + 0) * stride)), b = __builtin_nontemporal_load((const f32x4*)(src + (r + 1) * stride));
-    const f32x4 c = __builtin_nontemporal_load((const f32x4*)(src + (r + 2) * stride)), d = __builtin_nontemporal_load((const f32x4*)(src + (r + 3) * stride));
-    t = (((t + a) + b) + c) + d;
-  }
-  for (; r < ranges; ++r) t = t + __builtin_nontemporal_load((const f32x4*)(src + r * stride));
-  if (k < K) {
-#pragma unroll
-    for (int c = 0; c < 4; ++c)
-      if (n + c < N) C[(int64_t)(n + c) * ldc + k] += t[c];
-  }
+  __shared__ float red[8][32];
+  tn_reduce_block((int)blockIdx.x, red, part, part_cs, C, ldc, colsum, N, K, tiles, ranges, tn_cnt);
 }
 
 template <typename T>
@@ -406,10 +378,11 @@
     part = p.ranges > 1 ? (float*)workspace : nullptr;
     part_cs = colsum ? (float*)workspace + p.part_floats : nullptr;
   }
+  hipStream_t st = (hipStream_t)stream;
+  if (!part && flush_deferred_overlapping(C, C + ((int64_t)(N - 1) * ldc + K), st) != ALPRO_OK) return ALPRO_ERR_INVALID;
   const bool pp = get_option(OPT_TN_KIND) == 2;
   const unsigned grid = (unsigned)((p.units + 7) / 8 * 8);
   const size_t lds = (size_t)NSTAGE * 2 * IMG_BYTES;
-  hipStream_t st = (hipStream_t)stream;
   if (dtype == ALPRO_BF16) {
     static DeviceOnce once;
     once.run([&] {
@@ -427,8 +400,16 @@
     if (pp) hipLaunchKernelGGL((gemm_tn_kernel<f16_t, 1>), dim3(grid), dim3(NT3), lds, st, (const f16_t*)A, lda, (const f16_t*)B, ldb, C, ldc, M, N, K, p.per, p.tiles, p.units, p.tn, colsum, part, part_cs, 0);
     else hipLaunchKernelGGL((gemm_tn_kernel<f16_t, 0>), dim3(grid), dim3(NT3), lds, st, (const f16_t*)A, lda, (const f16_t*)B, ldb, C, ldc, M, N, K, p.per, p.tiles, p.units, p.tn, colsum, part, part_cs, 0);
   }
-  if (part || part_cs)
-    hipLaunchKernelGGL(tn_reduce_kernel, dim3((part ? p.tiles * 64 : 0) + (part_cs ? p.tn * (TW / 32) : 0)), dim3(256), 0, st, part, part_cs, C, ldc, colsum, N, K, p.tiles, p.ranges, p.tn);
+  if (part || part_cs) {
+    alpro_reduce_job_t job = {};
+    job.kind = ALPRO_REDUCE_TN;
+    job.part = part; job.part_cs = part_cs; job.dst[0] = C; job.dst[1] = part_cs ? colsum : nullptr; job.ldc = ldc;
+    job.N = N; job.K = K; job.tiles = p.tiles; job.ranges = p.ranges; job.tn_cnt = p.tn;
+    const int deferred = defer_reduce_job(job);
+    if (deferred < 0) return ALPRO_ERR_INVALID;
+    if (!deferred)
+      hipLaunchKernelGGL(tn_reduce_kernel, dim3((part ? p.tiles * 64 : 0) + (part_cs ? p.tn * (TW / 32) : 0)), dim3(256), 0, st, part, part_cs, C, ldc, colsum, N, K, p.tiles, p.ranges, p.tn);
+  }
   return check_launch("alpro_gemm_tn_acc");
 }
 
diff --git a/alpro_amd/csrc/reduce_jobs.hip b/alpro_amd/csrc/reduce_jobs.hip
--- /dev/null
+++ b/alpro_amd/csrc/reduce_jobs.hip
@@ -0,0 +1,161 @@
+#include "common.hpp"
+#include "reduce_jobs.hpp"
+
+namespace alpro {
+namespace {
+
+struct ReduceTable {
+  int32_t njobs;
+  int32_t block0[ALPRO_REDUCE_MAX_BATCH + 1];
+  alpro_reduce_job_t job[ALPRO_REDUCE_MAX_BATCH];
+};
+static_assert(sizeof(alpro_reduce_job_t) == 88, "alpro_reduce_job_t is 88 bytes (alpro_amd/hip.py: ReduceJob)");
+static_assert(sizeof(ReduceTable) <= 4096, "the job table must fit the kernel argument segment");
+
+__device__ __forceinline__ int job_of_block(const ReduceTable& tab, int b) {
+  int j = 0;
+  while (j + 1 < tab.njobs && b >= tab.block0[j + 1]) ++j;
+  return j;
+}
+
+__global__ __launch_bounds__(256) void tn_reduce_jobs_kernel(const ReduceTable tab) {
+  __shared__ float red[8][32];
+  const int j = job_of_block(tab, (int)blockIdx.x);
+  const alpro_reduce_job_t& J = tab.job[j];
+  tn_reduce_block((int)blockIdx.x - tab.block0[j], red, J.part, J.part_cs, J.dst[0], J.ldc, J.dst[1], J.N, J.K, J.tiles, J.ranges, J.tn_cnt);
+}
+
+__global__ __launch_bounds__(1024) void colsum_reduce_jobs_kernel(const ReduceTable tab) {
+  __shared__ float4 red[128][8];
+  __shared__ float4 red2[8][8];
+  const int j = job_of_block(tab, (int)blockIdx.x);
+  const alpro_reduce_job_t& J = tab.job[j];
+  const int b = (int)blockIdx.x - tab.block0[j], k = b / (RJ_D / 32);
+  colsum_reduce_block(b - k * (RJ_D / 32), k, red, red2, J.part, J.nparts, J.nslots, J.dst[k]);
+}
+
+int job_blocks(const alpro_reduce_job_t& j) {
+  if (j.kind == ALPRO_REDUCE_TN) return (j.part ? j.tiles * 64 : 0) + (j.part_cs ? j.tn_cnt * (RJ_TW / 32) : 0);
+  return (RJ_D / 32) * (j.dst[2] ? 3 : 2);
+}
+
+bool job_ok(const alpro_reduce_job_t& j) {
+  if (j.kind == ALPRO_REDUCE_TN)
+    return (j.part || j.part_cs) && (!j.part || j.dst[0]) && (!j.part_cs || j.dst[1]) && j.N > 0 && j.K > 0 && j.tiles > 0 && j.ranges > 0 &&
+           j.tn_cnt > 0 && j.tiles % j.tn_cnt == 0 && j.tn_cnt == (j.N + RJ_TW - 1) / RJ_TW && j.tiles == j.tn_cnt * ((j.K + RJ_TW - 1) / RJ_TW) &&
+           (!j.part || (j.ldc >= j.K && j.ranges > 1));
+  if (j.kind == ALPRO_REDUCE_COLSUM)
+    return j.part && j.nparts > 0 && (j.nslots == 2 || j.nslots == 3) && (!j.dst[2] || j.nslots == 3) && (j.dst[0] || j.dst[1] || j.dst[2]);
+  return false;
+}
+
+struct Span { uintptr_t lo, hi; };
+int job_spans(const alpro_reduce_job_t& j, Span s[3]) {
+  int n = 0;
+  if (j.kind == ALPRO_REDUCE_TN) {
+    if (j.part) s[n++] = Span{(uintptr_t)j.dst[0], (uintptr_t)(j.dst[0] + ((int64_t)(j.N - 1) * j.ldc + j.K))};
+    if (j.part_cs) s[n++] = Span{(uintptr_t)j.dst[1], (uintptr_t)(j.dst[1] + j.N)};
+  } else {
+    for (int i = 0; i < 3; ++i)
+      if (j.dst[i]) s[n++] = Span{(uintptr_t)j.dst[i], (uintptr_t)(j.dst[i] + RJ_D)};
+  }
+  return n;
+}
+bool jobs_overlap(const alpro_reduce_job_t& a, const alpro_reduce_job_t& b) {
+  Span sa[3], sb[3];
+  const int na = job_spans(a, sa), nb = job_spans(b, sb);
+  for (int i = 0; i < na; ++i)
+    for (int k = 0; k < nb; ++k)
+      if (sa[i].lo < sb[k].hi && sb[k].lo < sa[i].hi) return true;
+  return false;
+}
+
+thread_local alpro_reduce_job_t* t_jobs = nullptr;
+thread_local int t_capacity = 0;
+thread_local int* t_njobs = nullptr;
+
+}
+
+int defer_reduce_job(const alpro_reduce_job_t& job) {
+  if (!t_jobs) return 0;
+  if (*t_njobs < 0 || *t_njobs >= t_capacity) {
+    set_error("alpro_reduce_defer: the job list is full (%d jobs): flush it with alpro_reduce_jobs", t_capacity);
+    return -1;
+  }
+  t_jobs[(*t_njobs)++] = job;
+  return 1;
+}
+
+int flush_deferred_overlapping(const float* lo, const float* hi, hipStream_t st) {
+  if (!t_jobs || *t_njobs <= 0) return ALPRO_OK;
+  bool hit = false;
+  for (int i = 0; i < *t_njobs && !hit; ++i) {
+    Span s[3];
+    const int n = job_spans(t_jobs[i], s);
+    for (int k = 0; k < n && !hit; ++k) hit = s[k].lo < (uintptr_t)hi && (uintptr_t)lo < s[k].hi;
+  }
+  if (!hit) return ALPRO_OK;
+  const int n = *t_njobs;
+  *t_njobs = 0;
+  return alpro_reduce_jobs(t_jobs, n, st);
+}
+
+}
+
+using namespace alpro;
+
+extern "C" int alpro_reduce_defer(alpro_reduce_job_t* jobs, int capacity, int* njobs) {
+  ALPRO_CHECK(!jobs || (capacity > 0 && njobs && *njobs >= 0 && *njobs <= capacity), "alpro_reduce_defer: a job list needs a capacity and a counter within it");
+  t_jobs = jobs;
+  t_capacity = jobs ? capacity : 0;
+  t_njobs = jobs ? njobs : nullptr;
+  return ALPRO_OK;
+}
+
+extern "C" int alpro_reduce_plan(const alpro_reduce_job_t* jobs, int njobs, int32_t* launch) {
+  if (!(njobs >= 0 && (njobs == 0 || (jobs && launch)))) { set_error("alpro_reduce_plan: bad args"); return -1; }
+  int open_idx[2][ALPRO_REDUCE_MAX_BATCH], open_n[2] = {0, 0}, next = 0;
+  auto close = [&](int kind) {
+    if (!open_n[kind]) return;
+    for (int i = 0; i < open_n[kind]; ++i) launch[open_idx[kind][i]] = next;
+    ++next;
+    open_n[kind] = 0;
+  };
+  for (int i = 0; i < njobs; ++i) {
+    if (!job_ok(jobs[i])) { set_error("alpro_reduce_plan: job %d is malformed (kind %d)", i, jobs[i].kind); return -1; }
+    const int kind = jobs[i].kind;
+    bool clash = false;
+    for (int k = 0; k < 2 && !clash; ++k)
+      for (int o = 0; o < open_n[k] && !clash; ++o) clash = jobs_overlap(jobs[i], jobs[open_idx[k][o]]);
+    if (clash) { close(0); close(1); }
+    if (open_n[kind] == ALPRO_REDUCE_MAX_BATCH) close(kind);
+    open_idx[kind][open_n[kind]++] = i;
+  }
+  close(0);
+  close(1);
+  return next;
+}
+
+extern "C" int alpro_reduce_jobs(const alpro_reduce_job_t* jobs, int njobs, void* stream) {
+  ALPRO_CHECK(njobs >= 0 && (njobs == 0 || jobs), "alpro_reduce_jobs: bad args");
+  if (njobs == 0) return ALPRO_OK;
+  int32_t stack_launch[256];
+  int32_t* launch = stack_launch;
+  if (njobs > 256) launch = new int32_t[njobs];
+  const int nl = alpro_reduce_plan(jobs, njobs, launch);
+  int rc = nl < 0 ? ALPRO_ERR_INVALID : ALPRO_OK;
+  for (int l = 0; l < nl; ++l) {
+    ReduceTable tab = {};
+    for (int i = 0; i < njobs && tab.njobs < ALPRO_REDUCE_MAX_BATCH; ++i)
+      if (launch[i] == l) {
+        tab.job[tab.njobs] = jobs[i];
+        tab.block0[tab.njobs + 1] = tab.block0[tab.njobs] + job_blocks(jobs[i]);
+        ++tab.njobs;
+      }
+    const unsigned grid = (unsigned)tab.block0[tab.njobs];
+    if (tab.job[0].kind == ALPRO_REDUCE_TN) hipLaunchKernelGGL(tn_reduce_jobs_kernel, dim3(grid), dim3(256), 0, (hipStream_t)stream, tab);
+    else hipLaunchKernelGGL(colsum_reduce_jobs_kernel, dim3(grid), dim3(1024), 0, (hipStream_t)stream, tab);
+  }
+  if (launch != stack_launch) delete[] launch;
+  return rc != ALPRO_OK ? rc : check_launch("alpro_reduce_jobs");
+}
diff --git a/alpro_amd/csrc/reduce_jobs.hpp b/alpro_amd/csrc/reduce_jobs.hpp
--- /dev/null
+++ b/alpro_amd/csrc/reduce_jobs.hpp
@@ -0,0 +1,78 @@
+#pragma once
+#include "common.hpp"
+
+namespace alpro {
+
+constexpr int RJ_TW = 256;
+constexpr int RJ_D = 768;
+
+__device__ __forceinline__ void tn_reduce_block(int block, float (*red)[32], const float* __restrict__ part, const float* __restrict__ part_cs,
+                                                float* __restrict__ C, int64_t ldc, float* __restrict__ colsum, int N, int K, int tiles,
+                                                int ranges, int tn_cnt) {
+  const int tile_blocks = part ? tiles * 64 : 0;
+  if (block >= tile_blocks) {
+    const int c = threadIdx.x & 31, p = threadIdx.x >> 5;
+    const int n = (block - tile_blocks) * 32 + c;
+    const int sets = ranges * (tiles / tn_cnt);
+    float t = 0.f;
+    for (int r = p; r < sets; r += 8) t += part_cs[(int64_t)r * (tn_cnt * RJ_TW) + n];
+    red[p][c] = t;
+    __syncthreads();
+    if (p == 0 && n < N) colsum[n] += ((red[0][c] + red[1][c]) + (red[2][c] + red[3][c])) + ((red[4][c] + red[5][c]) + (red[6][c] + red[7][c]));
+    return;
+  }
+  const int tile = block >> 6, f = ((block & 63) << 8) + threadIdx.x;
+  const int lane = f & 63, q = (f >> 6) & 3, j = (f >> 8) & 1, i = (f >> 9) & 3, wave = f >> 11;
+  const int n = (tile % tn_cnt) * RJ_TW + (wave >> 2) * 128 + i * 32 + 8 * q + 4 * (lane >> 5);
+  const int k = (tile / tn_cnt) * RJ_TW + (wave & 3) * 64 + j * 32 + (lane & 31);
+  const float* src = part + (int64_t)tile * (RJ_TW * RJ_TW) + f * 4;
+  const int64_t stride = (int64_t)tiles * (RJ_TW * RJ_TW);
+  f32x4 t = {0.f, 0.f, 0.f, 0.f};
+  int r = 0;
+  for (; r + 4 <= ranges; r += 4) {
+    const f32x4 a = __builtin_nontemporal_load((const f32x4*)(src + (r + 0) * stride)), b = __builtin_nontemporal_load((const f32x4*)(src + (r + 1) * stride));
+    const f32x4 c = __builtin_nontemporal_load((const f32x4*)(src + (r + 2) * stride)), d = __builtin_nontemporal_load((const f32x4*)(src + (r + 3) * stride));
+    t = (((t + a) + b) + c) + d;
+  }
+  for (; r < ranges; ++r) t = t + __builtin_nontemporal_load((const f32x4*)(src + r * stride));
+  if (k < K) {
+#pragma unroll
+    for (int c = 0; c < 4; ++c)
+      if (n + c < N) C[(int64_t)(n + c) * ldc + k] += t[c];
+  }
+}
+
+__device__ __forceinline__ void colsum_reduce_block(int cg, int k, float4 (*red)[8], float4 (*red2)[8], const float* __restrict__ part, int nparts,
+                                                    int nslots, float* __restrict__ dst) {
+  const int c4 = threadIdx.x & 7, sl = threadIdx.x >> 3;
+  if (!dst) return;
+  const int col = cg * 32 + c4 * 4;
+  float4 s = make_float4(0.f, 0.f, 0.f, 0.f);
+#pragma unroll 4
+  for (int p = sl; p < nparts; p += 128) {
+    const float4 v = *(const float4*)(part + ((int64_t)p * nslots + k) * RJ_D + col);
+    s.x += v.x; s.y += v.y; s.z += v.z; s.w += v.w;
+  }
+  red[sl][c4] = s;
+  __syncthreads();
+  if (sl < 8) {
+    float4 t = red[sl * 16][c4];
+#pragma unroll
+    for (int i = 1; i < 16; ++i) { const float4 v = red[sl * 16 + i][c4]; t.x += v.x; t.y += v.y; t.z += v.z; t.w += v.w; }
+    red2[sl][c4] = t;
+  }
+  __syncthreads();
+  if (sl == 0) {
+    float4 t = red2[0][c4];
+#pragma unroll
+    for (int i = 1; i < 8; ++i) { const float4 v = red2[i][c4]; t.x += v.x; t.y += v.y; t.z += v.z; t.w += v.w; }
+    float4* o = (float4*)(dst + col);
+    const float4 c = *o;
+    *o = make_float4(c.x + t.x, c.y + t.y, c.z + t.z, c.w + t.w);
+  }
+}
+
+int defer_reduce_job(const alpro_reduce_job_t& job);
+int flush_deferred_overlapping(const float* lo, const float* hi, hipStream_t st);
+
+}
diff --git a/alpro_amd/dist.py b/alpro_amd/dist.py
--- a/alpro_amd/dist.py
+++ b/alpro_amd/dist.py
@@ -120,6 +120,8 @@
     if not collectives_active() or not _GRAD_FINAL_HOOKS:
         return
     from alpro_amd import config as rt
+    if torch.cuda.is_available():
+        rt.flush_deferred_reduce(torch.device("cuda", torch.cuda.current_device()))
     rt.join_wgrad()
     rt.join_text_streams()
     live = []
diff --git a/alpro_amd/hip.py b/alpro_amd/hip.py
--- a/alpro_amd/hip.py
+++ b/alpro_amd/hip.py
@@ -1,3 +1,4 @@
+import contextlib
 import ctypes
 import os
 
@@ -26,6 +27,7 @@
            "alpro_hip_sched_workspace_bytes", "alpro_hip_set_sched_workspace", "alpro_hip_release_stream", "alpro_gemm_qkv_tattn", "alpro_add_layernorm_pre_mlp2", "alpro_adamw_step_lp",
            "alpro_gemm_rows_f32_relu_mask", "alpro_clip_pool", "alpro_adamw_step_groups", "alpro_attn_temporal_fwd_drop", "alpro_attn_temporal_bwd_drop",
            "alpro_vit_final_pool_mode", "alpro_vit_final_pool_mode_bwd", "alpro_augment_stage", "alpro_augment_stats", "alpro_resized_crop",
+           "alpro_reduce_defer", "alpro_reduce_jobs", "alpro_reduce_plan",
            "alpro_sim_topk", "alpro_sim_topk_workspace_bytes", "alpro_attn_probs", "alpro_attn_temporal_probs", "alpro_attn_probs_grad", "alpro_unpatchify"]
 
 
@@ -52,6 +54,16 @@
 class TransposeJob(ctypes.Structure):
     _fields_ = [("in_", ctypes.c_void_p), ("out", ctypes.c_void_p), ("ld_in", ctypes.c_int64), ("ld_out", ctypes.c_int64),
                 ("R", ctypes.c_int32), ("C", ctypes.c_int32), ("Rpad", ctypes.c_int32), ("tile0", ctypes.c_int32)]
+
+
+REDUCE_TN, REDUCE_COLSUM = 0, 1
+REDUCE_MAX_BATCH = 32
+
+
+class ReduceJob(ctypes.Structure):
+    _fields_ = [("part", ctypes.c_void_p), ("part_cs", ctypes.c_void_p), ("dst", ctypes.c_void_p * 3), ("ldc", ctypes.c_int64),
+                ("kind", ctypes.c_int32), ("N", ctypes.c_int32), ("K", ctypes.c_int32), ("tiles", ctypes.c_int32), ("ranges", ctypes.c_int32),
+                ("tn_cnt", ctypes.c_int32), ("nparts", ctypes.c_int32), ("nslots", ctypes.c_int32), ("reserved0", ctypes.c_int32)]
 
 
 ADAMW_MAX_SEGMENTS = 32
@@ -109,6 +121,9 @@
     lib.alpro_softmax_xent.argtypes = [vp, i64, vp, i32, vp, vp, i32, i64, vp, i32, i32, i32, vp]
     lib.alpro_gemm_tn_acc.argtypes = [vp, i64, vp, i64, vp, i64, i32, i32, i32, i32, vp, vp]
     lib.alpro_gemm_tn_acc_ws.argtypes = [vp, i64, vp, i64, vp, i64, i32, i32, i32, i32, vp, vp, ctypes.c_size_t, vp]
+    lib.alpro_reduce_defer.argtypes = [vp, i32, vp]
+    lib.alpro_reduce_jobs.argtypes = [vp, i32, vp]
+    lib.alpro_reduce_plan.argtypes = [vp, i32, vp]
     lib.alpro_gemm_tn_workspace_bytes.argtypes = [i32, i32, i32]
     lib.alpro_gemm_tn_workspace_bytes.restype = ctypes.c_size_t
     lib.alpro_gemm_tn_ranges.argtypes = [i32, i32, i32, i32]
@@ -473,7 +488,16 @@
     common = (_ptr(dy), _CODE[dy.dtype], D, _ptr(_dev(dy2, torch.float32)) if dy2 is not None else None, _ptr(x), D,
               _ptr(_dev(gamma, torch.float32)), eps, _ptr(dx), D, 1 if accumulate else 0, _ptr(dgamma), _ptr(dbeta), rows, D,
               map_mode, map_p0, map_p1, drop_p, drop_seed)
-    ws, wsb = _reduce_ws(dy.device)
+    cp = emit.get("colsum_pre") if emit is not None else None
+    if dgamma is None:
+        q, (ws, wsb) = None, _reduce_ws(dy.device)
+    else:
+        q, ws, wsb = _ln_reduce_ws(dy.device, rows, (dgamma, dbeta, cp), cls_rows=rows // (map_p1 + 1) if map_mode == MAP_FRAME_TOKENS else 0)
+    with (_deferring(q, (dgamma, dbeta, cp)) if q is not None else contextlib.nullcontext()):
+        return _layernorm_bwd_call(lib, common, emit, dy, D, ws, wsb, dx)
+
+
+def _layernorm_bwd_call(lib, common, emit, dy, D, ws, wsb, dx):
     if emit is None:
         _check(lib.alpro_layernorm_bwd(*common, ws, wsb, _stream()), "alpro_layernorm_bwd")
         return dx
@@ -508,12 +532,13 @@
     D = src.shape[-1]
     rows = rows if rows is not None else src.numel() // D
     out = torch.empty((rows, D), dtype=dtype, device=src.device)
-    ws, wsb = _reduce_ws(src.device) if (colsum is not None or colsum_pre is not None) else (None, 0)
-    _check(lib.alpro_gather_cast(_ptr(src), D, _ptr(out), _CODE[dtype], rows, D, map_mode, map_p0, map_p1,
-                                 _ptr(_dev(row_scale, torch.float32)) if row_scale is not None else None, row_scale_group, cls_scale, drop_p, drop_seed,
-                                 _ptr(_dev(colsum, torch.float32)) if colsum is not None else None,
-                                 _ptr(_dev(colsum_pre, torch.float32)) if colsum_pre is not None else None, ws, wsb, _stream()),
-           "alpro_gather_cast")
+    q, ws, wsb = _ln_reduce_ws(src.device, rows, (colsum, colsum_pre)) if (colsum is not None or colsum_pre is not None) else (None, None, 0)
+    with (_deferring(q, (colsum, colsum_pre)) if q is not None else contextlib.nullcontext()):
+        _check(lib.alpro_gather_cast(_ptr(src), D, _ptr(out), _CODE[dtype], rows, D, map_mode, map_p0, map_p1,
+                                     _ptr(_dev(row_scale, torch.float32)) if row_scale is not None else None, row_scale_group, cls_scale, drop_p, drop_seed,
+                                     _ptr(_dev(colsum, torch.float32)) if colsum is not None else None,
+                                     _ptr(_dev(colsum_pre, torch.float32)) if colsum_pre is not None else None, ws, wsb, _stream()),
+               "alpro_gather_cast")
     return out
 
 
@@ -540,6 +565,7 @@
 def scatter_add_rows(src, idx, dst, idx_mod=0, skip_idx=-1):
     lib = load()
     _dev(src, torch.float32); _dev(dst, torch.float32)
+    reduce_sync(dst)
     if idx is not None and _DETERMINISTIC[0]:
         idx = _dev(idx, torch.int64).view(-1)
         if src.shape[0] <= 8192 and dst.shape[0] < (1 << 19) and src.is_contiguous() and dst.is_contiguous():
@@ -872,10 +898,11 @@
         sc, group = emit.get("scale"), emit.get("group", 1)
         if sc is not None and (_dev(sc, torch.float32).numel() * group < rows or group <= 0):
             raise RuntimeError("vit_final_pool_mode_bwd: %d row scales for groups of %d rows do not cover %d rows" % (sc.numel(), group, rows))
-    ws, wsb = _reduce_ws(x.device)
-    _check(lib.alpro_vit_final_pool_mode_bwd(_ptr(dout), _ptr(x), _ptr(_dev(gamma, torch.float32)), eps, _ptr(dx), _ptr(dgamma), _ptr(dbeta), mode, rows, B, T, N, D,
-                                             _ptr(out), _CODE[out.dtype] if out is not None else F32, _ptr(sc), group, ws, wsb, _stream()),
-           "alpro_vit_final_pool_mode_bwd")
+    q, ws, wsb = _ln_reduce_ws(x.device, rows, (dgamma, dbeta))
+    with (_deferring(q, (dgamma, dbeta)) if q is not None else contextlib.nullcontext()):
+        _check(lib.alpro_vit_final_pool_mode_bwd(_ptr(dout), _ptr(x), _ptr(_dev(gamma, torch.float32)), eps, _ptr(dx), _ptr(dgamma), _ptr(dbeta), mode, rows, B, T, N, D,
+                                                 _ptr(out), _CODE[out.dtype] if out is not None else F32, _ptr(sc), group, ws, wsb, _stream()),
+               "alpro_vit_final_pool_mode_bwd")
     return dx if emit is None else (dx, out)
 
 
@@ -999,7 +1026,139 @@
     return _ptr(ws), _REDUCE_WS_BYTES
 
 
-def gemm_tn_acc(a, b, c, colsum=None, atomic=None):
+REDUCE_QUEUE_JOBS = 96
+_REDUCE_ARENA_MIN = 64 << 20
+_REDUCE_ARENA_MAX = 1 << 30
+_REDUCE_QUEUES = {}
+_reduce_scope = [0]
+_reduce_stats = {"flushes": 0, "jobs": 0}
+
+
+class _ReduceQueue:
+    def __init__(self, device, stream):
+        self.device, self.stream = device, stream
+        self.jobs = (ReduceJob * REDUCE_QUEUE_JOBS)()
+        self.n = ctypes.c_int(0)
+        self.spans = []
+        self.arena, self.off = None, 0
+
+    def flush(self):
+        if self.n.value:
+            _reduce_stats["flushes"] += 1
+            _reduce_stats["jobs"] += self.n.value
+            n, self.n.value = self.n.value, 0
+            _check(load().alpro_reduce_jobs(self.jobs, n, ctypes.c_void_p(self.stream.cuda_stream)), "alpro_reduce_jobs")
+        self.spans = []
+        self.off = 0
+
+    def take(self, nbytes):
+        nbytes = (int(nbytes) + 255) // 256 * 256
+        have = self.arena.numel() if self.arena is not None else 0
+        if self.off + nbytes > have or self.n.value >= REDUCE_QUEUE_JOBS - 1:
+            grow = self.off + nbytes > have and have < _REDUCE_ARENA_MAX
+            self.flush()
+            if grow or nbytes > have:
+                self.arena = None
+                self.arena = torch.empty(max(nbytes, min(max(2 * have, _REDUCE_ARENA_MIN), _REDUCE_ARENA_MAX)), dtype=torch.uint8, device=self.device)
+        ws = self.arena[self.off:self.off + nbytes]
+        self.off += nbytes
+        return ws
+
+
+def reduce_scope(enter):
+    _reduce_scope[0] += 1 if enter else -1
+
+
+def reduce_deferring():
+    if _reduce_scope[0] <= 0 or not (_DETERMINISTIC[0] and _DETERMINISTIC_WGRAD[0]):
+        return False
+    from alpro_amd import config as rt
+    return rt.defer_reduce()
+
+
+def _reduce_queue(device):
+    cur = torch.cuda.current_stream(device)
+    key = (device.index if device.index is not None else torch.cuda.current_device(), cur.cuda_stream)
+    q = _REDUCE_QUEUES.get(key)
+    if q is None:
+        q = _REDUCE_QUEUES[key] = _ReduceQueue(device, cur)
+    return q
+
+
+def _span(t):
+    lo = t.data_ptr()
+    if t.dim() == 2:
+        return lo, lo + ((t.shape[0] - 1) * t.stride(0) + t.shape[1]) * t.element_size()
+    return lo, lo + t.numel() * t.element_size()
+
+
+def reduce_sync(*tensors, but=None):
+    for q in _REDUCE_QUEUES.values():
+        if q is but or not q.n.value:
+            continue
+        spans = [_span(t) for t in tensors if t is not None]
+        if any(lo < h and l < hi for lo, hi in spans for l, h in q.spans):
+            q.flush()
+            cur = torch.cuda.current_stream(q.device)
+            if cur.cuda_stream != q.stream.cuda_stream:
+                cur.wait_stream(q.stream)
+
+
+class _deferring:
+
+    def __init__(self, q, dests):
+        self.q, self.dests = q, [d for d in dests if d is not None]
+
+    def __enter__(self):
+        reduce_sync(*self.dests, but=self.q)
+        self.n0 = self.q.n.value
+        _check(load().alpro_reduce_defer(self.q.jobs, REDUCE_QUEUE_JOBS, ctypes.byref(self.q.n)), "alpro_reduce_defer")
+
+    def __exit__(self, *a):
+        load().alpro_reduce_defer(None, 0, None)
+        if self.q.n.value:
+            self.q.spans.extend(_span(d) for d in self.dests)
+
+
+def flush_reduce(device=None, all_streams=False):
+    if not _REDUCE_QUEUES:
+        return
+    if not all_streams:
+        dev = device if device is not None else torch.device("cuda", torch.cuda.current_device())
+        q = _REDUCE_QUEUES.get((dev.index if dev.index is not None else torch.cuda.current_device(), torch.cuda.current_stream(dev).cuda_stream))
+        if q is not None:
+            q.flush()
+        return
+    for q in _REDUCE_QUEUES.values():
+        if q.n.value:
+            q.flush()
+            cur = torch.cuda.current_stream(q.device)
+            if cur.cuda_stream != q.stream.cuda_stream:
+                cur.wait_stream(q.stream)
+        else:
+            q.flush()
+
+
+def flush_reduce_of(device_index, stream):
+    q = _REDUCE_QUEUES.get((device_index, stream.cuda_stream))
+    if q is not None:
+        q.flush()
+
+
+def reduce_pending():
+    return sum(q.n.value for q in _REDUCE_QUEUES.values())
+
+
+def _ln_reduce_ws(device, rows, dests, cls_rows=0):
+    if not reduce_deferring():
+        return (None,) + _reduce_ws(device)
+    q = _reduce_queue(device)
+    nbytes = min((rows + 31) // 32, 8192) * 3 * 768 * 4 + cls_rows * 768 * 4
+    ws = q.take(nbytes)
+    return q, _ptr(ws), nbytes
+
+
+def gemm_tn_acc(a, b, c, colsum=None, atomic=None, defer=False):
     lib = load()
     _dev(a); _dev(b, a.dtype); _dev(c, torch.float32)
     assert a.shape[0] == b.shape[0] and tuple(c.shape) == (a.shape[1], b.shape[1])
@@ -1010,9 +1169,18 @@
     if atomic is None:
         atomic = not _DETERMINISTIC_WGRAD[0] and M > 65536 and ((N + 255) // 256) * ((K + 255) // 256) > 9
     if atomic:
+        reduce_sync(c, colsum)
         _check(lib.alpro_gemm_tn_acc(_ptr(a), a.stride(0), _ptr(b), b.stride(0), _ptr(c), c.stride(0), _CODE[a.dtype], M, N, K, _ptr(colsum), _stream()),
                "alpro_gemm_tn_acc")
         return c
+    if defer and reduce_deferring():
+        q = _reduce_queue(a.device)
+        ws = q.take(max(lib.alpro_gemm_tn_workspace_bytes(M, N, K), 256))
+        with _deferring(q, (c, colsum)):
+            _check(lib.alpro_gemm_tn_acc_ws(_ptr(a), a.stride(0), _ptr(b), b.stride(0), _ptr(c), c.stride(0), _CODE[a.dtype], M, N, K, _ptr(colsum),
+                                            _ptr(ws), ws.numel(), _stream()), "alpro_gemm_tn_acc_ws")
+        return c
+    reduce_sync(c, colsum)
     ws = _tn_workspace(a.device, lib.alpro_gemm_tn_workspace_bytes(M, N, K))
     _check(lib.alpro_gemm_tn_acc_ws(_ptr(a), a.stride(0), _ptr(b), b.stride(0), _ptr(c), c.stride(0), _CODE[a.dtype], M, N, K, _ptr(colsum),
                                     _ptr(ws), ws.numel(), _stream()), "alpro_gemm_tn_acc_ws")
@@ -1024,6 +1192,7 @@
     _dev(a); _dev(colsum, torch.float32)
     M, N = a.shape
     assert colsum.numel() >= N
+    reduce_sync(colsum)
     ws = _tn_workspace(a.device, lib.alpro_gemm_tn_workspace_bytes(M, N, K))
     _check(lib.alpro_colsum_tn(_ptr(a), a.stride(0), _CODE[a.dtype], M, N, K, _ptr(colsum), _ptr(ws), ws.numel(), _stream()), "alpro_colsum_tn")
     return colsum
diff --git a/alpro_amd/modeling/timesformer/vit.py b/alpro_amd/modeling/timesformer/vit.py
--- a/alpro_amd/modeling/timesformer/vit.py
+++ b/alpro_amd/modeling/timesformer/vit.py
@@ -504,7 +504,7 @@
         if dt != torch.float32 and not (t_fc or t_p):
             hip.colsum_tn(G, sv["a_t"].shape[1], db1)
         elif dt != torch.float32:
-            hip.gemm_tn_acc(G, sv["a_t"], dWe, colsum=cs)
+            hip.gemm_tn_acc(G, sv["a_t"], dWe, colsum=cs, defer=bool(sv.get("defer_product_rule")))
         elif t_fc or t_p:
             hip.gemm(hip.transpose(G, colsum=cs), hip.transpose(sv["a_t"]), out=dWe, out_dtype=torch.float32)
         else:
@@ -711,6 +711,7 @@
                                              b["ws"].device))
             self._bwd_tables[idx] = tb
         lo, hi = idx[0], idx[-1] + 1
+        hip.reduce_sync(b["ws"][lo:hi].reshape(-1), *[o[k] for o in ops for k in ("g_fc", "g_p", "g_bp")])
         hip.cast(b["ws"][lo:hi].reshape(-1), dt, out=b["ws_dt"][lo:hi].reshape(-1))
         hip.transpose_batch(*tb["t_dwe"], dt)
         tb["ga"].launch()
@@ -1070,6 +1071,7 @@
             if sv["defer_product_rule"]:
                 group_rule.insert(0, j)
             dtok, dz = blk.backward(sv, dtok, dz=dz, emit_for=self.saved[j - 1 - nfro] if j > nfro else None)
+            rt.flush_deferred_reduce(dtok.device)
             done = nb - j
             if done % 4 == 0 or j == nfro:
                 if banked:
diff --git a/alpro_amd/modeling/train.py b/alpro_amd/modeling/train.py
--- a/alpro_amd/modeling/train.py
+++ b/alpro_amd/modeling/train.py
@@ -38,6 +38,8 @@
     if p.grad is None or (p.grad.numel() > 1 and not any(p.grad.stride())):
         p.grad = g.detach().clone().reshape(p.shape).contiguous()
     else:
+        if p.grad.is_cuda:
+            hip.reduce_sync(p.grad)
         p.grad.add_(g.reshape(p.shape))
 
 
@@ -144,11 +146,11 @@
         from alpro_amd import config as rt
         side = rt.wgrad_side_stream(dy_t.device)
         if side is None:
-            hip.gemm_tn_acc(dy_t, x_t, gw2, colsum=gb)
+            hip.gemm_tn_acc(dy_t, x_t, gw2, colsum=gb, defer=True)
             return
         side.wait_stream(torch.cuda.current_stream(dy_t.device))
         with torch.cuda.stream(side):
-            hip.gemm_tn_acc(dy_t, x_t, gw2, colsum=gb)
+            hip.gemm_tn_acc(dy_t, x_t, gw2, colsum=gb, defer=True)
         dy_t.record_stream(side)
         x_t.record_stream(side)
         return
@@ -204,11 +206,15 @@
         from alpro_amd import config as rt
         rt.check_backward_precision(getattr(ctx.run, "dt", None) or ctx.dt)
         rt.wgrad_scope(True)
+        hip.reduce_scope(True)
         try:
             with torch.no_grad():
                 g = ctx.run.backward(*[None if x is None else x.contiguous() for x in grads])
         finally:
+            hip.reduce_scope(False)
             rt.wgrad_scope(False)
+            if any(x is not None and x.is_cuda for x in grads):
+                rt.flush_deferred_reduce(next(x.device for x in grads if x is not None and x.is_cuda))
             rt.join_wgrad()
             _LIVE_ANCHORS.discard(ctx)
         if grads and any(x is not None and x.is_cuda for x in grads):
diff --git a/alpro_amd/modeling/xbert.py b/alpro_amd/modeling/xbert.py
--- a/alpro_amd/modeling/xbert.py
+++ b/alpro_amd/modeling/xbert.py
@@ -235,7 +235,7 @@
                 tr.grad_buffer(lin.bias, zero=True)
             gw, gb = tr.fused_grad_view([l.weight for l in lins]), tr.fused_grad_view([l.bias for l in lins])
         if gw is not None and gb is not None:
-            hip.gemm_tn_acc(dqkv, sv["h_t"], gw, colsum=gb)
+            hip.gemm_tn_acc(dqkv, sv["h_t"], gw, colsum=gb, defer=True)
         else:
             for i, lin in enumerate(lins):
                 tr.wgrad(dqkv[:, i * Hd:(i + 1) * Hd], sv["h_t"], lin.weight, lin.bias)
@@ -583,6 +583,7 @@
         d32, d_t = (dout.reshape(B * L, -1) if self.out_rows is None else dout.reshape(self.out_rows.numel(), -1)).contiguous(), None
         for i in range(hi - 1, lo - 1, -1):
             d32, d_t = m.encoder.layer[i].backward(self.saved.pop(), d32, d_t)
+            rt.flush_deferred_reduce(d32.device)
         if self.prefix:
             return None
         if self.parts is not None:
diff --git a/alpro_amd/optim.py b/alpro_amd/optim.py
--- a/alpro_amd/optim.py
+++ b/alpro_amd/optim.py
@@ -372,6 +372,7 @@
                     timer="device events on the compute stream" if log[0]["events"] is not None else "host clock (CPU tensors)")
 
     def synchronize(self, average=False):
+        hip.flush_reduce(all_streams=True)
         if not self.allreduce or not dist.collectives_active():
             self._note_synced("avg" if average else None)
             return 0
@@ -415,6 +416,7 @@
             (loss * sc.scale.reshape(())).backward()
 
     def step(self, closure=None):
+        hip.flush_reduce(all_streams=True)
         if self._pre_synced is not None and not (self._sync_is_current() and not self._inflight) and self.allreduce and dist.collectives_active():
             self.synchronize(average=self._pre_synced == "avg")
         pre = self._pre_synced
diff --git a/include/alpro_hip.h b/include/alpro_hip.h
--- a/include/alpro_hip.h
+++ b/include/alpro_hip.h
@@ -210,6 +210,22 @@
 int alpro_colsum_acc(const void* A, int64_t lda, float* out, int dtype, int M, int N, void* stream);
 int alpro_colsum_tn(const void* A, int64_t lda, int dtype, int M, int N, int K, float* colsum, void* workspace, size_t workspace_bytes, void* stream);
 
+enum { ALPRO_REDUCE_TN = 0, ALPRO_REDUCE_COLSUM = 1 };
+enum { ALPRO_REDUCE_MAX_BATCH = 32 };
+typedef struct alpro_reduce_job {
+  const float* part;
+  const float* part_cs;
+  float* dst[3];
+  int64_t ldc;
+  int32_t kind;
+  int32_t N, K, tiles, ranges, tn_cnt;
+  int32_t nparts, nslots;
+  int32_t reserved0;
+} alpro_reduce_job_t;
+int alpro_reduce_defer(alpro_reduce_job_t* jobs, int capacity, int* njobs);
+int alpro_reduce_jobs(const alpro_reduce_job_t* jobs, int njobs, void* stream);
+int alpro_reduce_plan(const alpro_reduce_job_t* jobs, int njobs, int32_t* launch);
+
 int alpro_softmax_xent(const float* logits, int64_t ld, const int64_t* labels, int ignore_index, float* loss_rows,
                        void* dlogits, int dtype, int64_t ldd, const float* grad_scale, int M, int V, int Vpad,
                        void* stream);
```

Result: no change. 436.4 (-0.2%).
